# kewei/gnss-sdr-rs

Hardware: AMD Instinct MI355X
Metric: acq PRN×Doppler cells/s + tracking ch×Msps at 1/2/4/8 GPU; % HBM roofline (higher is better)
Workload: dtype f32

## Files before the change

gnss-sdr-rs_amd/_lib.py:

```python
import ctypes as C
import os

_HERE = os.path.dirname(os.path.abspath(__file__))
_LIB_PATH = os.environ.get("GM_LIB_PATH") or os.path.join(_HERE, "lib", "libgnss_mi355x.so")


class GmError(RuntimeError):
    def __init__(self, status, where, detail=""):
        self.status = status
        super().__init__(f"{where}: gm_status {status} ({detail})")


class c32(C.Structure):
    _fields_ = [("re", C.c_float), ("im", C.c_float)]


class AcqResult(C.Structure):
    _fields_ = [("prn", C.c_uint8), ("code_phase_samples", C.c_uint64), ("code_phase_chips", C.c_float),
                ("carrier_freq", C.c_float), ("fs", C.c_float), ("mag_relative", C.c_float),
                ("sample_global_index", C.c_uint64), ("doppler_bin", C.c_int32)]

    def as_dict(self):
        return {k: getattr(self, k) for k, _ in self._fields_}


class AcqCfg(C.Structure):
    _fields_ = [("fs", C.c_float), ("f_if", C.c_float), ("fft_size", C.c_uint32), ("n_integrations", C.c_uint32),
                ("n_bins", C.c_uint32), ("doppler_hz", C.c_void_p), ("tables", C.c_void_p),
                ("table_freq", C.c_void_p), ("n_prn", C.c_uint32), ("prn_ids", C.c_void_p), ("codes", C.c_void_p),
                ("code_len", C.c_uint32), ("code_rate", C.c_float), ("threshold", C.c_float),
                ("decision_mode", C.c_int32), ("strict_sum_order", C.c_int32), ("reference_products", C.c_int32),
                ("any_length", C.c_int32), ("coherent_periods", C.c_uint32)]


class AcqPlan(C.Structure):
    _fields_ = [("form", C.c_int32), ("base", C.c_uint32), ("q", C.c_uint32), ("transform_len", C.c_uint32)]


ACQ_FORM_LDS, ACQ_FORM_COMPOSITE, ACQ_FORM_LONG, ACQ_FORM_LONG_PADDED = 0, 1, 2, 3


class TrkState(C.Structure):
    _fields_ = [("prn", C.c_uint8), ("active", C.c_uint8), ("reserved", C.c_uint8 * 2), ("lost_counter", C.c_uint32),
                ("next_sample_index", C.c_uint64), ("num_samples_per_code", C.c_uint64),
                ("carrier_freq", C.c_float), ("carrier_phase", C.c_float), ("carrier_error", C.c_float),
                ("carrier_nco", C.c_float), ("code_phase", C.c_float), ("code_error", C.c_float),
                ("code_nco", C.c_float), ("code_rate", C.c_float), ("i_prompt", C.c_float), ("q_prompt", C.c_float)]


class TrkOut(C.Structure):
    _fields_ = [(k, C.c_float) for k in ("ip", "qp", "ie", "qe", "il", "ql", "ive", "qve", "ivl", "qvl")]


class NavStatus(C.Structure):
    _fields_ = [("flag_bit_sync", C.c_uint8), ("flag_frame_sync", C.c_uint8), ("sync_sw", C.c_uint8), ("bit", C.c_int8),
                ("polarity", C.c_int8), ("frame_sync_ind", C.c_uint32), ("n_frame_bits", C.c_uint64), ("i_p", C.c_float),
                ("sf_cnt", C.c_uint64), ("sf_start_biti", C.c_uint64), ("tow_expected_ind", C.c_uint64)]


class TrkCfg(C.Structure):
    _fields_ = [("fs", C.c_float), ("n_channels", C.c_uint32), ("n_arms", C.c_uint32),
                ("early_late_space", C.c_float), ("very_early_late_space", C.c_float),
                ("code_index_mode", C.c_int32), ("boc11", C.c_int32), ("codes", C.c_void_p),
                ("n_codes", C.c_uint32), ("code_len", C.c_uint32), ("nominal_code_rate", C.c_float),
                ("pll_bw", C.c_float), ("pll_zeta", C.c_float), ("pll_gain", C.c_float), ("dll_bw", C.c_float),
                ("dll_zeta", C.c_float), ("dll_gain", C.c_float), ("pll_dt", C.c_float), ("dll_dt", C.c_float),
                ("lock_threshold", C.c_float), ("max_lost_epochs", C.c_uint32), ("strict_libm", C.c_int32), ("strict_sum_order", C.c_int32),
                ("share_device", C.c_int32)]


FMT_C32, FMT_I8_IQ, FMT_I8_REAL = 0, 1, 2
CODE_INDEX_FAITHFUL, CODE_INDEX_FIXED = 0, 1

_vp, _f, _u64, _u32, _sz, _i = C.c_void_p, C.c_float, C.c_uint64, C.c_uint32, C.c_size_t, C.c_int
SIGNATURES = {
    "gm_abi_version": (_i, []),
    "gm_init": (_i, [_i]),
    "gm_device_count": (_i, [C.POINTER(_i)]),
    "gm_last_error": (C.c_char_p, []),
    "gm_status_string": (C.c_char_p, [_i]),
    "gm_ca_code_row": (_i, [_i, _vp]),
    "gm_b1i_code": (_i, [C.c_uint32, _vp, C.c_uint32]),
    "gm_generate_ca_code_samples": (_i, [C.c_uint8, _f, _f, _vp, _sz, C.POINTER(_sz)]),
    "gm_doppler_table_new": (_i, [_f, _f, _f, _sz, C.POINTER(_f), _vp]),
    "gm_apply_doppler_shift": (_i, [_vp, _vp, _vp, _sz]),
    "gm_fft_c2c_f32": (_i, [_sz, _i, _vp, _sz]),
    "gm_fft_power_spectrum_f32": (_i, [_sz, _vp, _vp]),
    "gm_rfft_f32": (_i, [_sz, _vp, _vp]),
    "gm_fft_supported_sizes": (_i, [_vp, _i]),
    "gm_acq_plan_info": (_i, [C.c_uint32, C.c_int32, C.POINTER(AcqPlan)]),
    "gm_acq_create": (_i, [C.POINTER(AcqCfg), C.POINTER(_vp)]),
    "gm_acq_destroy": (_i, [_vp]),
    "gm_acq_search": (_i, [_vp, _vp, _sz, _i, _u64, _u64, _vp, _vp]),
    "gm_acq_search_c32": (_i, [_vp, _vp, _sz, _u64, _u64, _vp, _vp]),
    "gm_acq_search_i8": (_i, [_vp, _vp, _sz, _u64, _u64, _vp, _vp]),
    "gm_acq_search_ring": (_i, [_vp, _vp, _u64, _vp, _vp, C.POINTER(_u64)]),
    "gm_acq_search_dev": (_i, [_vp, _vp, _i, _vp]),
    "gm_acq_set_prn_mask": (_i, [_vp, _u64]),
    "gm_acq_decide_dev": (_i, [_vp, _vp, _u32, _vp, _u64]),
    "gm_acq_finer_doppler": (_i, [_vp, _vp, _vp, _u32, _vp, _vp, _vp, _vp]),
    "gm_comm_get_unique_id": (_i, [_vp]),
    "gm_comm_init": (_i, [_i, _i, _vp, _vp]),
    "gm_comm_destroy": (_i, [_vp]),
    "gm_comm_info": (_i, [_vp, _vp, _vp]),
    "gm_acq_allgather_metrics": (_i, [_vp, _vp, _vp, _vp]),
    "gm_acq_allgather_metrics_async": (_i, [_vp, _vp, _vp, _vp]),
    "gm_comm_wait": (_i, [_vp, _vp]),
    "gm_comm_allgather_words": (_i, [_vp, _vp, _vp, _sz, _vp]),
    "gm_grid_assemble_dev": (_i, [_vp, _u32, _u32, _u32, _vp, _u32, _vp, _vp]),
    "gm_acq_decide_planes_dev": (_i, [_vp, _vp, _vp, _u32, _u32, _vp, _vp, _u32, _f, _f, _f, _i, _u64, _vp, _vp, _vp]),
    "gm_acq_fetch_results": (_i, [_vp, _u32, _vp, _vp]),
    "gm_acq_decide_host": (_i, [_vp, _vp, _vp, _vp, _u32, _u32, _vp, _u32, _f, _f, _f, _u64, _vp, _vp]),
    "gm_acq_synchronize": (_i, [_vp]),
    "gm_acq_set_deferred_decision": (_i, [_vp, _i]),
    "gm_acq_prepare_dev": (_i, [_vp, _vp, _i, _vp, C.POINTER(C.c_uint64)]),
    "gm_acq_search_prepared_dev": (_i, [_vp, C.c_uint64, _vp]),
    "gm_acq_drop_prepared": (_i, [_vp]),
    "gm_acq_set_stream": (_i, [_vp, _vp]),
    "gm_acq_metrics": (_i, [_vp, _vp, _vp, _vp]),
    "gm_acq_code_fft": (_i, [_vp, _u32, _vp]),
    "gm_acq_tables": (_i, [_vp, _vp, _vp]),
    "gm_acq_coherent_phasors": (_i, [_vp, _vp]),
    "gm_acq_edge_dwell_periods": (_i, [_u32, _u32, _u32, _vp, _vp, C.POINTER(_u64)]),
    "gm_acq_set_edge_search": (_i, [_vp, _u32, _vp, _vp]),
    "gm_acq_edge_metrics": (_i, [_vp, _vp, _vp, _vp]),
    "gm_acq_edge_choice": (_i, [_vp, _vp]),
    "gm_acq_result_offsets": (_i, [_vp, _vp, _vp, _u32, _vp]),
    "gm_acq_enable_timing": (_i, [_vp, _i]),
    "gm_acq_last_timing": (_i, [_vp, C.POINTER(_f), C.POINTER(_f), C.POINTER(_f)]),
    "gm_acq_timing_summary": (_i, [_vp, C.POINTER(_u32), C.POINTER(_f), C.POINTER(_f)]),
    "gm_acq_debug_stamps": (_i, [_vp, _vp]),
    "gm_acq_manager_mode_for": (_i, [_sz]),
    "gm_acq_manager_pacing_and_list": (_i, [_i, _u32, C.POINTER(_u64), C.POINTER(_u32)]),
    "gm_ring_create": (_i, [_sz, C.POINTER(_vp)]),
    "gm_ring_destroy": (_i, [_vp]),
    "gm_ring_write_samples": (_i, [_vp, _vp, _sz]),
    "gm_ring_get_head": (_i, [_vp, C.POINTER(_u64)]),
    "gm_ring_copy_to_slice": (_i, [_vp, _u64, _vp, _sz]),
    "gm_ring_write_samples_async": (_i, [_vp, _vp, _sz]),
    "gm_ring_flush": (_i, [_vp]),
    "gm_ring_get_enqueued_head": (_i, [_vp, C.POINTER(_u64)]),
    "gm_ring_wait_head": (_i, [_vp, _u64, _u32, _vp]),
    "gm_nav_sync_create": (_i, [_i, _vp]),
    "gm_nav_sync_destroy": (_i, [_vp]),
    "gm_nav_sync_update": (_i, [_vp, _f, _f, _u64, _u64, _vp]),
    "gm_nav_sync_update_many": (_i, [_vp, _f, _vp, _sz, _sz, _u64, _u64, _vp, _vp, _vp]),
    "gm_nav_sync_frame_bits": (_i, [_vp, _vp, _sz, _vp]),
    "gm_nav_sync_histogram": (_i, [_vp, _vp]),
    "gm_nav_parity_check": (_i, [_vp, _vp, _vp]),
    "gm_frontend_create": (_i, [_f, _f, _f, _vp]),
    "gm_frontend_destroy": (_i, [_vp]),
    "gm_frontend_lut": (_i, [_vp, _vp, _vp, _vp]),
    "gm_frontend_get_state": (_i, [_vp, _vp, _vp, _vp]),
    "gm_frontend_set_state": (_i, [_vp, _f, _vp, _vp]),
    "gm_frontend_process_block": (_i, [_vp, _vp, _sz]),
    "gm_frontend_process_dev": (_i, [_vp, _vp, _i, _vp, _sz, _vp]),
    "gm_frontend_process_dev_batch": (_i, [_vp, _u32, _vp, _i, _vp, _sz, _vp]),
    "gm_frontend_synchronize": (_i, [_vp]),
    "gm_frontend_write_ring": (_i, [_vp, _vp, _vp, _sz, _i]),
    "gm_frontend_debug_repairs": (_i, [_vp, C.POINTER(_u32)]),
    "gm_trk_create": (_i, [C.POINTER(TrkCfg), C.POINTER(_vp)]),
    "gm_trk_destroy": (_i, [_vp]),
    "gm_trk_start": (_i, [_vp, _u32, C.POINTER(AcqResult)]),
    "gm_trk_reset": (_i, [_vp, _u32]),
    "gm_trk_get_state": (_i, [_vp, _u32, C.POINTER(TrkState)]),
    "gm_trk_set_state": (_i, [_vp, _u32, C.POINTER(TrkState)]),
    "gm_trk_get_ca_chip": (_i, [_vp, _u32, _f, C.POINTER(_f)]),
    "gm_loop_filter_new": (_i, [_f, _f, _f, C.POINTER(_f), C.POINTER(_f)]),
    "gm_loop_filter_update": (_f, [_f, _f, _f, _f, _f]),
    "gm_trk_correlate": (_i, [_vp, _u32, _vp, _sz, C.POINTER(TrkOut)]),
    "gm_trk_do_work": (_i, [_vp, _u32, _vp, _sz, C.POINTER(TrkOut), C.POINTER(C.c_uint8), C.POINTER(C.c_uint8)]),
    "gm_trk_update_all": (_i, [_vp, _vp, _u32, _vp, _vp, _vp, C.POINTER(_u32)]),
    "gm_trk_update_all_dev": (_i, [_vp, _vp, _u32]),
    "gm_trk_update_all_async": (_i, [_vp, _vp, _u32, C.POINTER(C.c_uint64)]),
    "gm_trk_collect": (_i, [_vp, C.c_uint64, _i, _vp, _vp, _vp, _vp, C.POINTER(_u32), C.POINTER(_i)]),
    "gm_trk_get_states": (_i, [_vp, _vp]),
    "gm_trk_set_states": (_i, [_vp, _vp, _vp]),
    "gm_trk_synchronize": (_i, [_vp]),
    "gm_trk_set_stream": (_i, [_vp, _vp]),
    "gm_trk_debug_stamps": (_i, [_vp, _u32, _vp]),
    "gm_trk_enable_timing": (_i, [_vp, _i]),
    "gm_trk_last_timing": (_i, [_vp, C.POINTER(_f), C.POINTER(_u32)]),
}

_lib = None


def library_path():
    return _LIB_PATH


def lib():
    global _lib
    if _lib is not None:
        return _lib
    if not os.path.exists(_LIB_PATH):
        raise ImportError(f"{_LIB_PATH} is missing: run `python __graft_entry__.py build` (hipcc, gfx950). "
                          "There is no CPU fallback for the HIP path.")
    L = C.CDLL(_LIB_PATH)
    for name, (res, args) in SIGNATURES.items():
        fn = getattr(L, name)
        fn.restype, fn.argtypes = res, args
    _lib = L
    return L


def check(status, where):
    if status != 0:
        L = lib()
        raise GmError(status, where, (L.gm_status_string(status) or b"").decode() + "; " +
                      (L.gm_last_error() or b"").decode())


_initialised = None


def init(device=0):
    global _initialised
    if _initialised != device:
        check(lib().gm_init(device), "gm_init")
        _initialised = device
```

gnss-sdr-rs_amd/build.py:

```python
import os
import subprocess
import sys
from concurrent.futures import ThreadPoolExecutor

HERE = os.path.dirname(os.path.abspath(__file__))
CSRC = os.path.join(HERE, "csrc")
LIBDIR = os.path.join(HERE, "lib")
LIB = os.path.join(LIBDIR, "libgnss_mi355x.so")
SOURCES = ["acq_kernels.hip", "acq_composite.hip", "acq_long.hip", "acq_coherent.hip", "acq_edge.hip", "trk_kernels.hip", "fe_kernels.hip", "nav_host.hip", "gm_api.hip"]
HEADERS = ["fft_core.h", "fft_plans.h", "acq_corr_plans.h", "gm_internal.h", "gm_libm.h", "acq_device.h", "acq_corr_ws31.h", "ws31_core.h", "acq_comp_ws.h", os.path.join("..", "..", "include", "gnss_mi355x.h")]
FLAGS = ["--offload-arch=gfx950", "-O3", "-std=c++17", "-ffp-contract=off", "-fno-slp-vectorize", "-fhip-fp32-correctly-rounded-divide-sqrt", "-fPIC",
         "-Wall", "-Wno-unused-function"]


def _stale(target, deps):
    if not os.path.exists(target):
        return True
    t = os.path.getmtime(target)
    return any(os.path.getmtime(d) > t for d in deps)


def build(force=False, verbose=False):
    global LIB
    extra = os.environ.get("GM_EXTRA_FLAGS", "").split()
    suffix = os.environ.get("GM_LIB_SUFFIX", "")
    if suffix:
        LIB = os.path.join(LIBDIR, "libgnss_mi355x%s.so" % suffix)
    os.makedirs(LIBDIR, exist_ok=True)
    objdir = os.path.join(HERE, "build" + suffix)
    os.makedirs(objdir, exist_ok=True)
    hdrs = [os.path.join(CSRC, h) for h in HEADERS]
    jobs = []
    for src in SOURCES:
        s = os.path.join(CSRC, src)
        o = os.path.join(objdir, src + ".o")
        if force or _stale(o, [s] + hdrs):
            jobs.append(["hipcc", *FLAGS, *extra, "-c", s, "-o", o])
    def run(cmd):
        if verbose:
            print(" ".join(cmd), flush=True)
        r = subprocess.run(cmd, stdout=subprocess.PIPE, stderr=subprocess.STDOUT, text=True)
        if r.returncode:
            raise RuntimeError("hipcc failed:\n" + " ".join(cmd) + "\n" + r.stdout)
        return r.stdout
    with ThreadPoolExecutor(max_workers=6) as ex:
        list(ex.map(run, jobs))
    objs = [os.path.join(objdir, s + ".o") for s in SOURCES]
    if force or jobs or _stale(LIB, objs):
        run(["hipcc", "--offload-arch=gfx950", "-shared", "-fPIC", "-o", LIB, *objs,
             "-Wl,--version-script=" + os.path.join(CSRC, "exports.map")])
    build_synth(force)
    build_receiver_harness(force)
    return LIB


def build_receiver_harness(force=False):
    src = os.path.join(HERE, "host", "receiver_harness.cpp")
    lib = os.path.join(LIBDIR, "libgm_receiver.so")
    deps = [src, os.path.join(HERE, "host", "gnss_sdr.hpp"), os.path.join(HERE, "..", "include", "gnss_mi355x.h")]
    product = os.path.join(LIBDIR, "libgnss_mi355x.so")
    if force or _stale(lib, deps) or (os.path.exists(product) and os.path.getmtime(product) > os.path.getmtime(lib)):
        r = subprocess.run(["g++", "-O2", "-std=c++17", "-fPIC", "-shared", "-ffp-contract=off", "-Wall", "-o", lib, src,
                            "-L", LIBDIR, "-lgnss_mi355x", "-Wl,-rpath,$ORIGIN", "-Wl,-rpath,/opt/rocm/lib", "-pthread"],
                           stdout=subprocess.PIPE, stderr=subprocess.STDOUT, text=True)
        if r.returncode:
            raise RuntimeError("g++ failed:\n" + r.stdout)
    return lib


def build_synth(force=False):
    src = os.path.join(HERE, "synthgen", "synth_xoshiro.cpp")
    lib = os.path.join(LIBDIR, "libgm_synth.so")
    if force or _stale(lib, [src]):
        r = subprocess.run(["g++", "-O2", "-std=c++17", "-fPIC", "-shared", "-fopenmp", "-ffp-contract=off", "-fno-builtin", "-o", lib, src],
                           stdout=subprocess.PIPE, stderr=subprocess.STDOUT, text=True)
        if r.returncode:
            raise RuntimeError("g++ failed:\n" + r.stdout)
    return lib


if __name__ == "__main__":
    print(build(force="--force" in sys.argv, verbose=True))
```

gnss-sdr-rs_amd/csrc/acq_kernels.hip:

```cpp
#include "acq_device.h"

namespace gm {

template <bool WG>
__device__ __forceinline__ void decide_body(const DecideArgs& a, int p, int lane, float* dsm) {
    const int D = a.n_bins;
    float* smax = dsm;
    float* ssum = dsm + D;
    uint32_t* sarg = reinterpret_cast<uint32_t*>(dsm + 2 * D);
    for (int d = lane; d < D; d += 64) {
        const size_t o = size_t(p) * D + d;
        smax[d] = a.mmax[o]; ssum[d] = a.msum[o]; sarg[d] = a.margmax[o];
    }
    if constexpr (WG) __syncthreads();
    else { __builtin_amdgcn_fence(__ATOMIC_RELEASE, "workgroup"); __builtin_amdgcn_wave_barrier(); __builtin_amdgcn_fence(__ATOMIC_ACQUIRE, "workgroup"); }
    const bool searched = (p >= 64) || ((a.mask_lo >> p) & 1ull);
    float gmax = 0.0f, bsum = 0.0f;
    uint32_t bphase = 0;
    int bbin = -1;
    bool pass = false;
    float carry_v = 0.0f;
    int carry_b = -1;
    for (int d0 = 0; d0 < D; d0 += 64) {
        const int d = d0 + lane;
        if (d0 > 0) { gmax = 0.0f; bsum = 0.0f; bphase = 0; bbin = -1; }
#ifdef GM_DECIDE_SERIAL_SCAN
        if (d < D && searched) {
            for (int q = 0; q <= d; ++q) {
                const float lm = smax[q];
                if (lm > gmax) { gmax = lm; bphase = sarg[q]; bsum = ssum[q]; bbin = q; }
            }
        }
#else
        {
            const float own = (d < D) ? smax[d] : 0.0f;
            gmax = own > 0.0f ? own : 0.0f;
            bbin = own > 0.0f ? d : -1;
#pragma unroll
            for (int off = 1; off < 64; off <<= 1) {
                const float ev = __shfl_up(gmax, off, 64);
                const int eb = __shfl_up(bbin, off, 64);
                if (lane >= off && !(gmax > ev)) { gmax = ev; bbin = eb; }
            }
            if (d0 > 0 && !(gmax > carry_v)) { gmax = carry_v; bbin = carry_b; }
            carry_v = __shfl(gmax, 63, 64); carry_b = __shfl(bbin, 63, 64);
            bphase = bbin >= 0 ? sarg[bbin] : 0u;
            bsum = bbin >= 0 ? ssum[bbin] : 0.0f;
        }
#endif
        if (d < D && searched) {
            if (!a.best_bin_mode || d + 1 == D) {
                const float avg = __fdiv_rn(bsum - gmax, float(a.fft_size - 1));
                pass = __fdiv_rn(gmax, avg) > a.threshold;
            }
        }
        const unsigned long long votes = __ballot(pass);
        if (votes) {
            if (lane == __ffsll((long long)votes) - 1) {
                gm_acq_result r;
                r.prn = a.prn_ids[p];
                r.code_phase_samples = bphase;
                r.code_phase_chips = __fdiv_rn(float(bphase) * a.code_rate, a.fs);
                r.carrier_freq = a.table_freq[bbin]; r.fs = a.fs; r.mag_relative = gmax;
                r.sample_global_index = a.local_tail + bphase; r.doppler_bin = bbin;
                a.results[p] = r;
                a.found[p] = 1;
            }
            return;
        }
    }
    if (lane == 0) {
        gm_acq_result r;
        r.prn = a.prn_ids[p]; r.code_phase_samples = 0; r.code_phase_chips = 0.f; r.carrier_freq = 0.f;
        r.fs = 0.f; r.mag_relative = 0.f; r.sample_global_index = 0; r.doppler_bin = -1;
        a.results[p] = r;
        a.found[p] = 0;
    }
}
__global__ __launch_bounds__(64) void decide_kernel(DecideArgs a) {
    extern __shared__ float dsm[];
    decide_body<true>(a, blockIdx.x, threadIdx.x, dsm);
}

template <class PLX>
__global__ __launch_bounds__(MixPlanOf<PLX>::type::T) void acq_mix_fft_kernel(const void* __restrict__ samples, int fmt,
                                                            const cf* __restrict__ tables,
                                                            const cf* __restrict__ tw_fwd,
                                                            cf* __restrict__ spectra, int n_int,
                                                            uint32_t* __restrict__ clear_tickets,
                                                            const uint16_t* __restrict__ order, int n_items, DecideArgs dec) {
    using PL = typename MixPlanOf<PLX>::type;
    using CP = typename CorrPlanOf<PLX>::type;
    static_assert(PL::N == PLX::N, "the mix plan keeps the size");
    constexpr bool PERMUTED = CorrMode<CP>::PERMUTED;
    constexpr int STAGE = PERMUTED ? PL::N + PL::N / 32 + 1 : 0;
    constexpr int LDS_N = PL::LDS_ELEMS + PL::TW_TOTAL > STAGE ? PL::LDS_ELEMS + PL::TW_TOTAL : STAGE;
    __shared__ cf lds[LDS_N];
    if (int(blockIdx.x) >= n_items) {
        static_assert(LDS_N * 8 >= 3 * 64 * 4, "room for the decision's staging");
        if (threadIdx.x < 64) decide_body<false>(dec, int(blockIdx.x) - n_items, threadIdx.x, reinterpret_cast<float*>(lds));
        return;
    }
    cf* tw = lds + PL::LDS_ELEMS;
    const int tid = threadIdx.x;
    const int d = blockIdx.x / n_int, m = blockIdx.x % n_int;
    if (clear_tickets && blockIdx.x == 0)
        for (int i = tid; i < GM_CORR_SPLIT_MAX_ITEMS; i += PL::T) clear_tickets[i] = 0u;
    load_twiddles<PL>(tw, tw_fwd, tid);
    const size_t sbase = size_t(m) * PL::N;
    const cf* tab = tables + size_t(d) * PL::N;
    cf* dst = spectra + size_t(blockIdx.x) * PL::N;
    constexpr int NB0 = PL::NB(0);
    auto in = [&](int it, int r) {
        const int idx = (tid + it * PL::T) + r * NB0;
        const cf s = load_sample(samples, fmt, sbase + idx);
        const cf t = tab[idx];
        return cf_make(s.x * t.x - s.y * t.y, s.x * t.y + s.y * t.x);
    };
    if constexpr (!PERMUTED) {
        constexpr int NBL = PL::NB(PL::NP - 1);
        lds_transform<PL, false>(in, [&](int it, int r, cf val) { dst[PairLayout<CP>::pos((tid + it * PL::T) + r * NBL)] = val; }, lds, tw, tid);
    } else {
        constexpr int NBL = PL::NB(PL::NP - 1);
        {
            cf v0[PL::IT0][PL::R0];
            Fft<PL, false>::pass0_stage1(v0, in, tid);
            __syncthreads();
            Fft<PL, false>::pass0_stage2(v0, lds, tid);
        }
        __syncthreads();
        MiddlePasses<PL, false, 1>::run(lds, tw, tid);
        cf vl[PL::ITL][PL::RL];
        Fft<PL, false>::last_stage1(vl, lds, tw, tid);
        __syncthreads();
        Fft<PL, false>::last_stage2(vl, [&](int it, int r, cf val) {
            const int k = (tid + it * PL::T) + r * NBL;
            lds[k + (k >> 5)] = val; }, tid);
        __syncthreads();
        static_assert(PL::N % 2 == 0, "N must be even");
        for (int g = tid; g < PL::N / 2; g += PL::T) {
            const uint32_t o = reinterpret_cast<const uint32_t*>(order)[g];
            const int k0 = int(o & 0xffffu), k1 = int(o >> 16);
            const cf v0 = lds[k0 + (k0 >> 5)], v1 = lds[k1 + (k1 >> 5)];
            reinterpret_cast<float4*>(dst)[g] = make_float4(v0.x, v0.y, v1.x, v1.y);
        }
    }
}

__device__ long long* g_corr_stamps = nullptr;
__device__ __forceinline__ void corr_stamp(long long* base, int m, int wave, int phase) {
    if (base) {
        unsigned long long t;
        __builtin_amdgcn_sched_barrier(0);
        asm volatile("s_memtime %0\n\ts_waitcnt lgkmcnt(0)" : "=s"(t) :: "memory");
        __builtin_amdgcn_sched_barrier(0);
        base[(size_t(m) * 8 + wave) * 8 + phase] = (long long)t;
    }
}
#ifdef GM_DIAG_STAMPS
static bool g_corr_stamps_armed = false;
bool corr_stamps_built() { return true; }
void set_corr_stamps(long long* d_ptr) {
    (void)hipMemcpyToSymbol(HIP_SYMBOL(g_corr_stamps), &d_ptr, sizeof(d_ptr));
    g_corr_stamps_armed = d_ptr != nullptr;
}
#else
static constexpr bool g_corr_stamps_armed = false;
bool corr_stamps_built() { return false; }
void set_corr_stamps(long long*) {}
#endif

template <class PLX, bool KEEP_CODE, bool STAMPS, bool REF_MUL>
__global__ __launch_bounds__(CorrPlanOf<PLX>::type::T, CorrPlanOf<PLX>::type::WAVES_PER_EU) void acq_corr_kernel(
    const cf* __restrict__ spectra, const cf* __restrict__ code_fft, const cf* __restrict__ tw_inv,
    float* __restrict__ mmax, uint32_t* __restrict__ margmax, float* __restrict__ msum,
    const uint32_t* __restrict__ worker_list, int n_workers, int n_bins, int n_int, int map_mode,
    int split_from, int split_k, int split_items, float* __restrict__ split_scratch, uint32_t* __restrict__ split_counter,
    int strict_sum) {
    const int xcd = blockIdx.x & 7, wslot = blockIdx.x >> 3;
    int slot = wslot, part = 0, parts = 1;
    if (wslot >= split_from) {
        const int h = wslot - split_from;
        slot = split_from + h / split_k;
        part = h % split_k;
        parts = split_k;
    }
    int d, p;
    if (map_mode == 0) {
        const int items = n_bins * n_workers, share = (items + 7) >> 3;
        const int item = xcd * share + slot;
        if (slot >= share || item >= items) return;
        d = item / n_workers;
        p = int(worker_list[item - d * n_workers]);
    } else if (map_mode >= 16) {
        const int cb = map_mode >> 4, rows_max = map_mode & 15;
        const int items = n_bins * n_workers, share = (items + 7) >> 3;
        const int it_lo = xcd * share, it_hi = it_lo + share < items ? it_lo + share : items;
        const int d_lo = it_lo / n_workers, per_blk = rows_max * cb;
        const int blk = slot / per_blk, rem = slot - blk * per_blk, dr = rem / cb, w = blk * cb + (rem - dr * cb);
        const int item = (d_lo + dr) * n_workers + w;
        if (w >= n_workers || item < it_lo || item >= it_hi) return;
        d = d_lo + dr;
        p = int(worker_list[w]);
    } else if (map_mode == 1) {
        d = xcd + 8 * (slot / n_workers);
        if (d >= n_bins) return;
        p = int(worker_list[slot % n_workers]);
    } else {
        const int q = n_bins >> 3, whole = q * n_workers;
        if (slot < whole) {
            d = xcd + 8 * (slot / n_workers);
            p = int(worker_list[slot % n_workers]);
        } else {
            const int left = (n_bins - 8 * q) * n_workers, each = (left + 7) >> 3;
            const int j = slot - whole, item = xcd * each + j;
            if (j >= each || item >= left) return;
            d = 8 * q + item / n_workers;
            p = int(worker_list[item % n_workers]);
        }
    }

    using PL = typename CorrPlanOf<PLX>::type;
    constexpr bool PFA = CorrMode<PL>::PFA, HYB = CorrMode<PL>::HYBRID;
    __shared__ cf lds[PL::LDS_ELEMS + ((PFA || HYB) ? 0 : PL::TW_TOTAL)];
    cf* tw = lds + PL::LDS_ELEMS;
    const int tid = threadIdx.x;
    if constexpr (!PFA && !HYB) load_twiddles<PL>(tw, tw_inv, tid);
    constexpr int NB0 = PL::NB(0), NBL = PL::NB(PL::NP - 1);
    auto last_active = [&](int it) { if constexpr (HYB) return PL::last_active(tid); else return tid + it * PL::T < NBL; };
    auto out_index = [&](int it, int r) {
        if constexpr (HYB) return PL::out_index(tid, r);
        else if constexpr (PFA) return Pfa<PL>::out_index(tid + it * PL::T, r);
        else return (tid + it * PL::T) + r * NBL;
    };

    const __amdgpu_buffer_rsrc_t xrs = make_rsrc(spectra + size_t(d) * n_int * PL::N, unsigned(n_int) * PL::N * 8u);
    const __amdgpu_buffer_rsrc_t crs = make_rsrc(code_fft + size_t(p) * PL::N, PL::N * 8u);

    using PLd = PairLoad<PL>;
    constexpr bool CODE_PAIRED = CorrLayout<PL>::CODE_PAIRED;
    cf cc[KEEP_CODE ? PL::IT0 : 1][KEEP_CODE ? PL::R0 : 1];
    if constexpr (KEEP_CODE) {
#pragma unroll
        for (int it = 0; it < PL::IT0; ++it) {
            const int b = tid + it * PL::T;
            if (b < NB0) {
                PLd q;
                if constexpr (CODE_PAIRED) q.load(crs, b, 0);
#pragma unroll
                for (int r = 0; r < PL::R0; ++r) {
                    const cf c = CODE_PAIRED ? q.get(r) : buf_load_cf(crs, b * 8, r * NB0 * 8);
                    cc[it][r] = cf_make(c.x, -c.y);
                }
            }
        }
    }
    float acc[PL::ITL][PL::RL];
#pragma unroll
    for (int it = 0; it < PL::ITL; ++it)
#pragma unroll
        for (int r = 0; r < PL::RL; ++r) acc[it][r] = 0.0f;

    long long* stbase = nullptr;
    if constexpr (STAMPS) stbase = (blockIdx.x == 0 && (tid & 63) == 0 && PL::T / 64 <= 8) ? g_corr_stamps : nullptr;
    const int wv = tid >> 6;
    const int m_per = n_int / parts, m_begin = part * m_per, m_end = m_begin + m_per;
    constexpr bool CAN_SPLIT = !STAMPS;
    constexpr int RL4 = (PL::RL + 3) / 4;
    auto acc_or_zero = [&](int it, int r) { return r < PL::RL ? acc[it][r < PL::RL ? r : 0] : 0.0f; };
#ifndef GM_CORR_PREFETCH_PAIRS
#define GM_CORR_PREFETCH_PAIRS 4
#endif
    constexpr int NPF = (HYB && CODE_PAIRED && !STAMPS && !KEEP_CODE) ? (GM_CORR_PREFETCH_PAIRS < PLd::NPAIR ? GM_CORR_PREFETCH_PAIRS : PLd::NPAIR) : 0;
    PLd xq[PL::IT0];
    auto load_x_ahead = [&](int m_) {
#pragma unroll
        for (int it = 0; it < PL::IT0; ++it) xq[it].template load_range<0, NPF, false>(xrs, tid + it * PL::T, m_ * PL::N);
    };
    if constexpr (NPF > 0) load_x_ahead(m_begin);
    for (int m = m_begin; m < m_end; ++m) {
        PLd cq[(KEEP_CODE || !CODE_PAIRED) ? 1 : PL::IT0];
#pragma unroll
        for (int it = 0; it < PL::IT0; ++it) {
            const int b = tid + it * PL::T;
            if constexpr (CODE_PAIRED) xq[it].template load_range<NPF, PLd::NPAIR, true>(xrs, b, m * PL::N);
            if constexpr (!KEEP_CODE && CODE_PAIRED) cq[it].load(crs, b, 0);
        }
        auto in = [&](int it, int r) {
            const cf a = CODE_PAIRED ? xq[it].get(r) : buf_load_cf(xrs, (tid + it * PL::T) * 8, (m * PL::N + r * NB0) * 8);
            cf c;
            if constexpr (KEEP_CODE) c = cc[it][r];
            else if constexpr (CODE_PAIRED) { const cf g = cq[it].get(r); c = cf_make(g.x, -g.y); }
            else { const cf g = buf_load_cf(crs, (tid + it * PL::T) * 8, r * NB0 * 8); c = cf_make(g.x, -g.y); }
            if constexpr (REF_MUL) return cf_make(a.x * c.x - a.y * c.y, a.x * c.y + a.y * c.x);
            else return cf_make(__builtin_fmaf(a.x, c.x, -(a.y * c.y)), __builtin_fmaf(a.x, c.y, a.y * c.x));
        };
        auto out = [&](int it, int r, cf v) {
            if constexpr (REF_MUL) acc[it][r] = acc[it][r] + (v.x * v.x + v.y * v.y);
            else acc[it][r] = acc[it][r] + __builtin_fmaf(v.y, v.y, v.x * v.x);
        };
        if constexpr (NPF > 0) {
            lds_transform<PL, true, PFA>(in, out, lds, tw, tid, [&](int k) {
                if (k == 1) {
                    __builtin_amdgcn_sched_barrier(0);
                    load_x_ahead(m + 1 < m_end ? m + 1 : n_int);
                    __builtin_amdgcn_sched_barrier(0);
                }
            });
        } else if constexpr (!STAMPS) {
            lds_transform<PL, true, PFA>(in, out, lds, tw, tid);
        } else {
            auto st = [&](int k) { corr_stamp(stbase, m, wv, k); };
            st(0);
            {
                cf v0[PL::IT0][PL::R0];
                Fft<PL, true, PFA>::pass0_stage1(v0, in, tid);
                st(1);
                __syncthreads();
                st(2);
                Fft<PL, true, PFA>::pass0_stage2(v0, lds, tid);
            }
            st(3);
            __syncthreads();
            MiddlePasses<PL, true, 1, PFA>::run(lds, tw, tid, st);
            cf vl[PL::ITL][PL::RL];
            Fft<PL, true, PFA>::last_stage1(vl, lds, tw, tid);
            Fft<PL, true, PFA>::last_stage2(vl, out, tid);
        }
    }

    if constexpr (CAN_SPLIT) {
        if (parts > 1) {
            constexpr int SLAB = PL::ITL * RL4 * 4 * PL::T;
            const size_t item_plane0 = (size_t(xcd) * split_items + (slot - split_from)) * size_t(n_int);
            const __amdgpu_buffer_rsrc_t srs = make_rsrc(split_scratch + item_plane0 * SLAB, unsigned(n_int) * SLAB * 4u);
            const int voff = tid * 16 + part * SLAB * 4;
#pragma unroll
            for (int it = 0; it < PL::ITL; ++it)
#pragma unroll
                for (int r4 = 0; r4 < RL4; ++r4) {
                    u32x4 v;
                    v.x = __float_as_uint(acc_or_zero(it, 4 * r4 + 0)); v.y = __float_as_uint(acc_or_zero(it, 4 * r4 + 1));
                    v.z = __float_as_uint(acc_or_zero(it, 4 * r4 + 2)); v.w = __float_as_uint(acc_or_zero(it, 4 * r4 + 3));
                    __builtin_amdgcn_raw_buffer_store_b128(v, srs, voff + (it * RL4 + r4) * PL::T * 16, 0, 16);
                    asm volatile("s_nop 1" ::: "memory");
                }
            asm volatile("s_waitcnt vmcnt(0)" ::: "memory");
            __syncthreads();
            __shared__ int s_last;
            if (tid == 0) {
                uint32_t* cnt = split_counter + size_t(xcd) * split_items + (slot - split_from);
                const uint32_t old = __hip_atomic_fetch_add(cnt, 1u, __ATOMIC_RELAXED, __HIP_MEMORY_SCOPE_AGENT);
                s_last = (old == uint32_t(parts - 1)) ? 1 : 0;
            }
            __syncthreads();
            if (!s_last) return;
#pragma unroll
            for (int it = 0; it < PL::ITL; ++it)
#pragma unroll
                for (int r = 0; r < PL::RL; ++r) acc[it][r] = 0.0f;
            for (int q = 0; q < n_int; ++q) {
#pragma unroll
                for (int it = 0; it < PL::ITL; ++it)
#pragma unroll
                    for (int r4 = 0; r4 < RL4; ++r4) {
                        const u32x4 v = __builtin_amdgcn_raw_buffer_load_b128(srs, tid * 16, (q * SLAB + (it * RL4 + r4) * PL::T * 4) * 4, 16);
                        if (4 * r4 + 0 < PL::RL) acc[it][4 * r4 + 0] += __uint_as_float(v.x);
                        if (4 * r4 + 1 < PL::RL) acc[it][4 * r4 + 1 < PL::RL ? 4 * r4 + 1 : 0] += __uint_as_float(v.y);
                        if (4 * r4 + 2 < PL::RL) acc[it][4 * r4 + 2 < PL::RL ? 4 * r4 + 2 : 0] += __uint_as_float(v.z);
                        if (4 * r4 + 3 < PL::RL) acc[it][4 * r4 + 3 < PL::RL ? 4 * r4 + 3 : 0] += __uint_as_float(v.w);
                    }
            }
        }
    }

    float strict_total = 0.0f;
    if (strict_sum) {
        __syncthreads();
        float* pl = reinterpret_cast<float*>(lds);
#pragma unroll
        for (int it = 0; it < PL::ITL; ++it) {
            if (last_active(it)) {
#pragma unroll
                for (int r = 0; r < PL::RL; ++r) pl[out_index(it, r)] = acc[it][r];
            }
        }
        __syncthreads();
        if (tid < 64) {
            float ls = 0.0f;
            if (tid < 8) {
                constexpr int CHUNKS = PL::N / 8;
#pragma unroll 8
                for (int c = 0; c < CHUNKS; ++c) ls = ls + pl[c * 8 + tid];
            }
            float t = -0.0f;
#pragma unroll
            for (int l = 0; l < 8; ++l) t = t + __uint_as_float(__builtin_amdgcn_readlane(__float_as_uint(ls), l));
            strict_total = t;
        }
    }

    float bv = 0.0f, sum = 0.0f;
    uint32_t bi = 0xffffffffu;
    if constexpr (!PFA) {
#pragma unroll
        for (int it = 0; it < PL::ITL; ++it) {
            if (last_active(it)) {
#pragma unroll
                for (int r = 0; r < PL::RL; ++r) {
                    take_better(bv, bi, acc[it][r], uint32_t(out_index(it, r)));
                    sum += acc[it][r];
                }
            }
        }
    } else {
        int bs = -1, ties = 0;
#pragma unroll
        for (int it = 0; it < PL::ITL; ++it) {
            if (tid + it * PL::T < NBL) {
#pragma unroll
                for (int r = 0; r < PL::RL; ++r) {
                    const float v = acc[it][r];
                    if (v > bv) { bv = v; bs = it * PL::RL + r; }
                    sum += v;
                }
            }
        }
#pragma unroll
        for (int it = 0; it < PL::ITL; ++it) {
            if (tid + it * PL::T < NBL) {
#pragma unroll
                for (int r = 0; r < PL::RL; ++r) ties += acc[it][r] == bv ? 1 : 0;
            }
        }
        if (ties == 1 && bs >= 0) {
            bi = uint32_t(Pfa<PL>::out_index(tid + (bs / PL::RL) * PL::T, bs % PL::RL));
        } else if (ties >= 1) {
#pragma unroll
            for (int it = 0; it < PL::ITL; ++it) {
                const int b = tid + it * PL::T;
                if (b < NBL) {
#pragma unroll
                    for (int r = 0; r < PL::RL; ++r)
                        if (acc[it][r] == bv) {
                            const uint32_t i = uint32_t(Pfa<PL>::out_index(b, r));
                            bi = i < bi ? i : bi;
                        }
                }
            }
        }
    }
#pragma unroll
    for (int off = 32; off >= 1; off >>= 1) {
        const float ov = __shfl_xor(bv, off, 64);
        const uint32_t oi = uint32_t(__shfl_xor(int(bi), off, 64));
        const float os = __shfl_xor(sum, off, 64);
        take_better(bv, bi, ov, oi);
        sum += os;
    }
    __syncthreads();
    float* sv = reinterpret_cast<float*>(lds);
    uint32_t* si = reinterpret_cast<uint32_t*>(lds) + 64;
    float* ss = reinterpret_cast<float*>(lds) + 128;
    const int wave = tid >> 6, lane = tid & 63;
    constexpr int NW = PL::T / 64;
    if (lane == 0) { sv[wave] = bv; si[wave] = bi; ss[wave] = sum; }
    __syncthreads();
    if (tid == 0) {
        float fv = sv[0], fs = ss[0];
        uint32_t fi = si[0];
        for (int w = 1; w < NW; ++w) { take_better(fv, fi, sv[w], si[w]); fs += ss[w]; }
        if (fi == 0xffffffffu) fi = 0;
        const size_t o = size_t(p) * n_bins + d;
        mmax[o] = fv; margmax[o] = fi; msum[o] = strict_sum ? strict_total : fs;
    }
}

}
#include "acq_corr_ws31.h"
namespace gm {

template <class PL>
__global__ __launch_bounds__(PL::T) void acq_code_fft_kernel(const int8_t* __restrict__ code_samples,
                                                             const cf* __restrict__ tw_fwd,
                                                             cf* __restrict__ code_fft) {
    __shared__ cf lds[PL::LDS_ELEMS + PL::TW_TOTAL];
    cf* tw = lds + PL::LDS_ELEMS;
    const int tid = threadIdx.x;
    load_twiddles<PL>(tw, tw_fwd, tid);
    const int8_t* src = code_samples + size_t(blockIdx.x) * PL::N;
    cf* dst = code_fft + size_t(blockIdx.x) * PL::N;
    constexpr int NB0 = PL::NB(0), NBL = PL::NB(PL::NP - 1);
    lds_transform<PL, false>([&](int it, int r) { return cf_make(float(src[(tid + it * PL::T) + r * NB0]), 0.0f); },
                             [&](int it, int r, cf val) { dst[(tid + it * PL::T) + r * NBL] = val; }, lds, tw, tid);
}

template <class PL, bool INV>
__global__ __launch_bounds__(PL::T) void fft_batch_kernel(cf* __restrict__ data, const cf* __restrict__ tw_g) {
    __shared__ cf lds[PL::LDS_ELEMS + PL::TW_TOTAL];
    cf* tw = lds + PL::LDS_ELEMS;
    const int tid = threadIdx.x;
    load_twiddles<PL>(tw, tw_g, tid);
    cf* x = data + size_t(blockIdx.x) * PL::N;
    constexpr int NB0 = PL::NB(0), NBL = PL::NB(PL::NP - 1);
    lds_transform<PL, INV>([&](int it, int r) { return x[(tid + it * PL::T) + r * NB0]; },
                           [&](int it, int r, cf val) { x[(tid + it * PL::T) + r * NBL] = val; }, lds, tw, tid);
}

template <class PL, bool INV>
__global__ __launch_bounds__(PL::T) void big_cols_kernel(const cf* __restrict__ x, cf* __restrict__ B, const cf* __restrict__ tw_g, uint32_t N2) {
    __shared__ cf lds[PL::LDS_ELEMS + PL::TW_TOTAL];
    cf* tw = lds + PL::LDS_ELEMS;
    const int tid = threadIdx.x;
    const uint32_t n2 = blockIdx.x, L = uint32_t(PL::N) * N2;
    load_twiddles<PL>(tw, tw_g, tid);
    cf* dst = B + size_t(n2) * PL::N;
    constexpr int NB0 = PL::NB(0), NBL = PL::NB(PL::NP - 1);
    const float inv_l = 2.0f / float(L);
    lds_transform<PL, INV>(
        [&](int it, int r) { return x[size_t(N2) * uint32_t((tid + it * PL::T) + r * NB0) + n2]; },
        [&](int it, int r, cf v) {
            const uint32_t k1 = uint32_t((tid + it * PL::T) + r * NBL);
            const uint32_t t = (n2 * k1) & (L - 1u);
            float sn, cs;
            sincospif(float(t) * inv_l, &sn, &cs);
            if (INV) sn = -sn;
            dst[k1] = cf_make(__builtin_fmaf(v.x, cs, v.y * sn), __builtin_fmaf(v.y, cs, -(v.x * sn)));
        },
        lds, tw, tid);
}
template <class PL, bool INV>
__global__ __launch_bounds__(PL::T) void big_rows_kernel(const cf* __restrict__ B, cf* __restrict__ X, const cf* __restrict__ tw_g, uint32_t N1) {
    __shared__ cf lds[PL::LDS_ELEMS + PL::TW_TOTAL];
    cf* tw = lds + PL::LDS_ELEMS;
    const int tid = threadIdx.x;
    const uint32_t k1 = blockIdx.x;
    load_twiddles<PL>(tw, tw_g, tid);
    constexpr int NB0 = PL::NB(0), NBL = PL::NB(PL::NP - 1);
    lds_transform<PL, INV>(
        [&](int it, int r) { return B[size_t(uint32_t((tid + it * PL::T) + r * NB0)) * N1 + k1]; },
        [&](int it, int r, cf v) { X[size_t(N1) * uint32_t((tid + it * PL::T) + r * NBL) + k1] = v; },
        lds, tw, tid);
}

template <class PL>
__global__ __launch_bounds__(PL::T) void fine_cols_kernel(FineArgs a) {
    __shared__ cf lds[PL::LDS_ELEMS + PL::TW_TOTAL];
    cf* tw = lds + PL::LDS_ELEMS;
    const int tid = threadIdx.x;
    const uint32_t n2 = blockIdx.x, sat = blockIdx.y;
    load_twiddles<PL>(tw, a.tw1, tid);
    const uint32_t cp = a.sat_code_phase[sat];
    const int8_t* chips = a.chips + size_t(a.sat_worker[sat]) * a.code_len;
    const float mre = a.mean[0], mim = a.mean[1];
    cf* dst = a.B + (size_t(sat) * a.N2 + n2) * PL::N;
    constexpr int NB0 = PL::NB(0), NBL = PL::NB(PL::NP - 1);
    const float inv_n = 2.0f / float(a.N1 * a.N2);
    lds_transform<PL, false>(
        [&](int it, int r) {
            const uint32_t n1 = uint32_t((tid + it * PL::T) + r * NB0);
            const uint32_t n = a.N2 * n1 + n2;
            if (n >= a.size_use) return cf_make(0.0f, 0.0f);
            const cf s = load_sample(a.samples, a.fmt, size_t(cp) + n);
            const uint32_t ind = uint32_t(floorf((float(n) * a.code_rate) / a.fs)) % a.code_len;
            const float c = float(chips[ind]);
            return cf_make((s.x - mre) * c, (s.y - mim) * c);
        },
        [&](int it, int r, cf v) {
            const uint32_t k1 = uint32_t((tid + it * PL::T) + r * NBL);
            const uint32_t t = (n2 * k1) & (a.N1 * a.N2 - 1u);
            float sn, cs;
            sincospif(float(t) * inv_n, &sn, &cs);
            dst[k1] = cf_make(__builtin_fmaf(v.x, cs, v.y * sn), __builtin_fmaf(v.y, cs, -(v.x * sn)));
        },
        lds, tw, tid);
}

template <class PL> struct FineRows {
    static constexpr int PER = PL::IT0 * PL::R0;
    static constexpr int RT = PL::T >= 1024 ? 1 : (PER <= 8 ? 8 : (PER <= 16 ? 4 : (PER <= 32 ? 2 : 1)));
};

template <class PL>
__global__ __launch_bounds__(PL::T) void fine_rows_kernel(FineArgs a) {
    constexpr int RT = FineRows<PL>::RT;
    __shared__ cf lds[PL::LDS_ELEMS + PL::TW_TOTAL];
    __shared__ float s_p[PL::T / 64];
    __shared__ uint32_t s_k[PL::T / 64];
    cf* tw = lds + PL::LDS_ELEMS;
    const int tid = threadIdx.x;
    const uint32_t k1_0 = blockIdx.x * RT, sat = blockIdx.y;
    load_twiddles<PL>(tw, a.tw2, tid);
    const cf* src = a.B + size_t(sat) * a.N2 * a.N1 + k1_0;
    constexpr int NB0 = PL::NB(0), NBL = PL::NB(PL::NP - 1);
    cf tile[RT][PL::IT0][PL::R0];
#pragma unroll
    for (int it = 0; it < PL::IT0; ++it) {
        const int b = tid + it * PL::T;
        if (b < NB0) {
#pragma unroll
            for (int r = 0; r < PL::R0; ++r) {
                const cf* p = src + size_t(b + r * NB0) * a.N1;
#pragma unroll
                for (int j = 0; j < RT; ++j) tile[j][it][r] = p[j];
            }
        }
    }
    float best = -1.0f;
    uint32_t bestk = 0xFFFFFFFFu;
#pragma unroll
    for (int j = 0; j < RT; ++j) {
        lds_transform<PL, false>(
            [&](int it, int r) { return tile[j][it][r]; },
            [&](int it, int r, cf v) {
                const uint32_t k = (k1_0 + j) + a.N1 * uint32_t((tid + it * PL::T) + r * NBL);
                const float p = __builtin_fmaf(v.x, v.x, v.y * v.y);
                if (p > best || (p == best && k < bestk)) { best = p; bestk = k; }
            },
            lds, tw, tid);
    }
    for (int off = 32; off > 0; off >>= 1) {
        const float op = __shfl_xor(best, off);
        const uint32_t ok = __shfl_xor(bestk, off);
        if (op > best || (op == best && ok < bestk)) { best = op; bestk = ok; }
    }
    if ((tid & 63) == 0) { s_p[tid >> 6] = best; s_k[tid >> 6] = bestk; }
    __syncthreads();
    if (tid == 0) {
        for (int w = 1; w < PL::T / 64; ++w)
            if (s_p[w] > best || (s_p[w] == best && s_k[w] < bestk)) { best = s_p[w]; bestk = s_k[w]; }
        a.rowmax[size_t(sat) * (a.N1 / RT) + blockIdx.x] = best;
        a.rowarg[size_t(sat) * (a.N1 / RT) + blockIdx.x] = bestk;
    }
}

__global__ __launch_bounds__(256) void fine_final_kernel(const float* __restrict__ rowmax, const uint32_t* __restrict__ rowarg,
                                                         uint32_t n_rows, float* __restrict__ peak_pow,
                                                         uint32_t* __restrict__ peak_idx) {
    __shared__ float s_p[4];
    __shared__ uint32_t s_k[4];
    const int tid = threadIdx.x;
    const uint32_t sat = blockIdx.x;
    float best = -1.0f;
    uint32_t bestk = 0xFFFFFFFFu;
    for (uint32_t i = tid; i < n_rows; i += 256) {
        const float p = rowmax[size_t(sat) * n_rows + i];
        const uint32_t k = rowarg[size_t(sat) * n_rows + i];
        if (p > best || (p == best && k < bestk)) { best = p; bestk = k; }
    }
    for (int off = 32; off > 0; off >>= 1) {
        const float op = __shfl_xor(best, off);
        const uint32_t ok = __shfl_xor(bestk, off);
        if (op > best || (op == best && ok < bestk)) { best = op; bestk = ok; }
    }
    if ((tid & 63) == 0) { s_p[tid >> 6] = best; s_k[tid >> 6] = bestk; }
    __syncthreads();
    if (tid == 0) {
        for (int w = 1; w < 4; ++w)
            if (s_p[w] > best || (s_p[w] == best && s_k[w] < bestk)) { best = s_p[w]; bestk = s_k[w]; }
        peak_pow[sat] = best;
        peak_idx[sat] = bestk;
    }
}
void launch_fine_final(hipStream_t st, const float* rowmax, const uint32_t* rowarg, uint32_t n_rows, int n_sats,
                       float* peak_pow, uint32_t* peak_idx) {
    hipLaunchKernelGGL(fine_final_kernel, dim3(n_sats), dim3(256), 0, st, rowmax, rowarg, n_rows, peak_pow, peak_idx);
}

__global__ __launch_bounds__(1024) void fine_mean_kernel(const void* __restrict__ samples, int fmt, uint32_t n, float* __restrict__ mean) {
    __shared__ float s_re[16], s_im[16];
    const int tid = threadIdx.x;
    float re = 0.0f, im = 0.0f;
    for (uint32_t i = tid; i < n; i += 1024) {
        const cf v = load_sample(samples, fmt, i);
        re += v.x; im += v.y;
    }
    for (int off = 32; off > 0; off >>= 1) { re += __shfl_xor(re, off); im += __shfl_xor(im, off); }
    if ((tid & 63) == 0) { s_re[tid >> 6] = re; s_im[tid >> 6] = im; }
    __syncthreads();
    if (tid == 0) {
        for (int w = 1; w < 16; ++w) { re += s_re[w]; im += s_im[w]; }
        mean[0] = re / float(n);
        mean[1] = im / float(n);
    }
}
void launch_fine_mean(hipStream_t st, const void* samples, int fmt, uint32_t n, float* d_mean) {
    hipLaunchKernelGGL(fine_mean_kernel, dim3(1), dim3(1024), 0, st, samples, fmt, n, d_mean);
}

template <class PL> struct Launch {
    static void fill_tw(cf* tw, bool inverse) {
        fill_twiddles<PL>(tw, inverse, [](double a) { return ::cos(a); }, [](double a) { return ::sin(a); });
    }
    using CP = typename CorrPlanOf<PL>::type;
    static constexpr bool CORR_TW = !CorrMode<CP>::PFA && !CorrMode<CP>::HYBRID;
    static constexpr int corr_tw_total() { if constexpr (CORR_TW) return CP::TW_TOTAL; else return 0; }
    static void fill_tw_corr(cf* tw) {
        if constexpr (CORR_TW) fill_twiddles<CP>(tw, true, [](double a) { return ::cos(a); }, [](double a) { return ::sin(a); });
    }
    static_assert(CP::T == PL::T && CP::N == PL::N, "the correlation plan keeps the size and the workgroup");
    using MP = typename MixPlanOf<PL>::type;
    static void fill_tw_mix(cf* tw, bool inverse) {
        fill_twiddles<MP>(tw, inverse, [](double a) { return ::cos(a); }, [](double a) { return ::sin(a); });
    }
    static void mix_fft(hipStream_t st, const void* samples, int fmt, const cf* tables, const cf* tw_fwd,
                        cf* spectra, int n_bins, int n_int, uint32_t* clear_tickets, const uint16_t* order, const DecideArgs* dec) {
        const int n_items = n_bins * n_int, n_dec = dec ? dec->n_prn : 0;
        DecideArgs none{};
        hipLaunchKernelGGL(acq_mix_fft_kernel<PL>, dim3(n_items + n_dec), dim3(MP::T), 0, st, samples, fmt,
                           tables, tw_fwd, spectra, n_int, clear_tickets, order, n_items, dec ? *dec : none);
    }
    static int fill_order(uint16_t* order) { return fill_order_table<CP>(order); }
    static constexpr bool WS31 = Ws31<CP>::USE && CorrMode<CP>::PFA;
    static constexpr int slab() {
        constexpr int generic = CP::ITL * ((CP::RL + 3) / 4) * 4 * CP::T;
        if constexpr (WS31) return ws31_split_slab<CP>() > generic ? ws31_split_slab<CP>() : generic;
        else return generic;
    }
    static constexpr int SPLIT_SLAB = slab();
    static void corr(hipStream_t st, const cf* spectra, const cf* code_fft, const cf* tw_inv, float* mmax,
                     uint32_t* margmax, float* msum, const uint32_t* worker_list, int n_workers, int n_bins,
                     int n_int, float* split_scratch, int split_planes, uint32_t* split_counter, int strict_sum, int tickets_cleared,
                     int ref_mul) {
        if (n_workers <= 0) return;
        static const int forced = diag_int("GM_CORR_MAP", -1);
        const int per_xcd_bins = ((n_bins + 7) / 8) * n_workers, per_xcd_even = (n_bins * n_workers + 7) / 8;
        const int slots = 32 * CP::WG_PER_CU;
        const int q = n_bins / 8, left = (n_bins - 8 * q) * n_workers;
        const int per_xcd_mixed = q * n_workers + (left + 7) / 8;
        int map_mode = ((per_xcd_bins + slots - 1) / slots > (per_xcd_even + slots - 1) / slots) ? 0 : 1;
        if (map_mode == 1 && per_xcd_mixed < per_xcd_bins) map_mode = 2;
        if (forced >= 0) map_mode = forced;
        static const int cb_env = diag_int("GM_CORR_CB", -1);
        int cb = cb_env >= 0 ? cb_env : 0;
        int share = map_mode == 0 ? per_xcd_even : (map_mode == 1 ? per_xcd_bins : per_xcd_mixed);
        if (cb > 0) {
            const int rows_max = (per_xcd_even + n_workers - 2) / n_workers + 1;
            if (rows_max <= 15 && cb <= 1000) {
                map_mode = (cb << 4) | rows_max;
                share = ((n_workers + cb - 1) / cb) * rows_max * cb;
            }
        }
        static const int split_env = diag_int("GM_CORR_SPLIT", -1);
        static const int items_env = diag_int("GM_CORR_SPLIT_ITEMS", -1);
        int split_from = share, split_k = 1, split_items = 0;
        if (SPLIT_SLAB && split_scratch && split_counter && split_env != 0 && !g_corr_stamps_armed && !strict_sum &&
            (share > slots || share <= GM_CORR_SPLIT_MAX_ITEMS / 8)) {
            const bool all = share <= slots;
            if (n_int >= 2 && n_int <= GM_CORR_SPLIT_MAX_K && (!all || share * n_int <= split_planes / 8)) split_k = n_int;
            if (CP::WG_PER_CU == 1 && !all && split_env < 0) split_k = 1;
            if (split_env == 1) split_k = 1;
            if (split_k > 1) {
                split_items = items_env > 0 ? items_env : (all ? share : (slots + split_k - 1) / split_k);
                if (split_items > share) split_items = share;
                if (split_items > GM_CORR_SPLIT_MAX_ITEMS / 8) split_items = GM_CORR_SPLIT_MAX_ITEMS / 8;
                if (split_items * n_int > split_planes / 8) split_items = split_planes / 8 / n_int;
                if (split_items <= 0) { split_items = 0; split_k = 1; }
                split_from = share - split_items;
            }
        }
        const int grid = 8 * (split_from + split_items * split_k);
        if (split_k > 1 && !tickets_cleared) (void)hipMemsetAsync(split_counter, 0, size_t(GM_CORR_SPLIT_MAX_ITEMS) * sizeof(uint32_t), st);
        if constexpr (WS31) {
            if (!g_corr_stamps_armed) {
                if (ref_mul)
                    hipLaunchKernelGGL((acq_corr_ws31_kernel<CP, true>), dim3(grid), dim3(1024), 0, st, spectra, code_fft, mmax, margmax, msum,
                                       worker_list, n_workers, n_bins, n_int, map_mode, split_from, split_k, split_items, split_scratch, split_counter, strict_sum);
                else
                    hipLaunchKernelGGL((acq_corr_ws31_kernel<CP, false>), dim3(grid), dim3(1024), 0, st, spectra, code_fft, mmax, margmax, msum,
                                       worker_list, n_workers, n_bins, n_int, map_mode, split_from, split_k, split_items, split_scratch, split_counter, strict_sum);
                return;
            }
        }
#ifdef GM_DIAG_STAMPS
        if (g_corr_stamps_armed) {
            hipLaunchKernelGGL((acq_corr_kernel<PL, CP::KEEP_CODE, true, false>), dim3(grid), dim3(PL::T), 0, st,
                               spectra, code_fft, tw_inv, mmax, margmax, msum, worker_list, n_workers, n_bins, n_int, map_mode,
                               split_from, split_k, split_items, split_scratch, split_counter, strict_sum);
            return;
        }
#endif
#ifdef GM_DIAG_STAMPS
        constexpr bool GENERIC = true;
#else
        constexpr bool GENERIC = !WS31;
#endif
        if constexpr (GENERIC) {
            if (ref_mul)
                hipLaunchKernelGGL((acq_corr_kernel<PL, CP::KEEP_CODE, false, true>), dim3(grid), dim3(PL::T), 0, st,
                                   spectra, code_fft, tw_inv, mmax, margmax, msum, worker_list, n_workers, n_bins, n_int, map_mode,
                                   split_from, split_k, split_items, split_scratch, split_counter, strict_sum);
            else
                hipLaunchKernelGGL((acq_corr_kernel<PL, CP::KEEP_CODE, false, false>), dim3(grid), dim3(PL::T), 0, st,
                                   spectra, code_fft, tw_inv, mmax, margmax, msum, worker_list, n_workers, n_bins, n_int, map_mode,
                                   split_from, split_k, split_items, split_scratch, split_counter, strict_sum);
        }
    }
    static void code_fft(hipStream_t st, const int8_t* code_samples, const cf* tw_fwd, cf* out, int n_codes) {
        hipLaunchKernelGGL(acq_code_fft_kernel<PL>, dim3(n_codes), dim3(PL::T), 0, st, code_samples, tw_fwd, out);
    }
    static void pair_codes(hipStream_t st, const cf* nat, cf* paired, int n_codes) {
        hipLaunchKernelGGL(relayout_kernel<CP>, dim3(n_codes * 4 < 1024 ? n_codes * 4 : 1024), dim3(256), 0, st, nat, paired, n_codes);
    }
    static void fft_batch(hipStream_t st, cf* data, const cf* tw, int inverse, int batch) {
        if (inverse) hipLaunchKernelGGL((fft_batch_kernel<PL, true>), dim3(batch), dim3(PL::T), 0, st, data, tw);
        else hipLaunchKernelGGL((fft_batch_kernel<PL, false>), dim3(batch), dim3(PL::T), 0, st, data, tw);
    }
    static constexpr bool POW2 = (PL::N & (PL::N - 1)) == 0;
    static void big_cols(hipStream_t st, const cf* x, cf* B, const cf* tw, uint32_t n2, int inverse) {
        if constexpr (POW2) {
            if (inverse) hipLaunchKernelGGL((big_cols_kernel<PL, true>), dim3(n2), dim3(PL::T), 0, st, x, B, tw, n2);
            else hipLaunchKernelGGL((big_cols_kernel<PL, false>), dim3(n2), dim3(PL::T), 0, st, x, B, tw, n2);
        }
    }
    static void big_rows(hipStream_t st, const cf* B, cf* X, const cf* tw, uint32_t n1, int inverse) {
        if constexpr (POW2) {
            if (inverse) hipLaunchKernelGGL((big_rows_kernel<PL, true>), dim3(n1), dim3(PL::T), 0, st, B, X, tw, n1);
            else hipLaunchKernelGGL((big_rows_kernel<PL, false>), dim3(n1), dim3(PL::T), 0, st, B, X, tw, n1);
        }
    }
    static void fine_cols(hipStream_t st, const FineArgs& a, int n_sats) {
        if constexpr (POW2) hipLaunchKernelGGL(fine_cols_kernel<PL>, dim3(a.N2, n_sats), dim3(PL::T), 0, st, a);
    }
    static void fine_rows(hipStream_t st, const FineArgs& a, int n_sats) {
        if constexpr (POW2) hipLaunchKernelGGL(fine_rows_kernel<PL>, dim3(a.N1 / FineRows<PL>::RT, n_sats), dim3(PL::T), 0, st, a);
    }
    static constexpr PlanOps ops() {
        return PlanOps{PL::N, PL::T, PL::TW_TOTAL, int(sizeof(cf)) * (CP::LDS_ELEMS + corr_tw_total()), SPLIT_SLAB,
                       CorrLayout<CP>::RELAYOUT ? 1 : 0,
                       &fill_tw, &fill_order, &mix_fft, &corr, &code_fft, &pair_codes, &fft_batch,
                       POW2 ? &fine_cols : nullptr, POW2 ? &fine_rows : nullptr, FineRows<PL>::RT,
                       POW2 ? &big_cols : nullptr, POW2 ? &big_rows : nullptr, MP::TW_TOTAL, &fill_tw_mix, corr_tw_total(), &fill_tw_corr,
                       &launch_mix_fft_coh<PL>};
    }
};

#define GM_PLAN_ENTRY(PL) Launch<PL>::ops(),
static const PlanOps g_plans[] = {GM_FOR_EACH_PLAN(GM_PLAN_ENTRY)};

const PlanOps* find_plan(int n) {
    for (const PlanOps& p : g_plans)
        if (p.n == n) return &p;
    return nullptr;
}
int list_plans(uint32_t* sizes, int cap) {
    int k = 0;
    for (const PlanOps& p : g_plans) {
        if (k < cap && sizes) sizes[k] = uint32_t(p.n);
        ++k;
    }
    return k;
}

__global__ void apply_doppler_kernel(const cf* __restrict__ s, const cf* __restrict__ t, cf* __restrict__ out,
                                     size_t n4) {
    for (size_t i = size_t(blockIdx.x) * blockDim.x + threadIdx.x; i < n4; i += size_t(gridDim.x) * blockDim.x) {
        const cf a = s[i], b = t[i];
        out[i] = cf_make(a.x * b.x - a.y * b.y, a.x * b.y + a.y * b.x);
    }
}
void launch_apply_doppler(hipStream_t st, const cf* s, const cf* t, cf* out, size_t n) {
    const size_t n4 = (n / 4) * 4;
    if (!n4) return;
    const int blocks = int((n4 + 255) / 256 < 2048 ? (n4 + 255) / 256 : 2048);
    hipLaunchKernelGGL(apply_doppler_kernel, dim3(blocks), dim3(256), 0, st, s, t, out, n4);
}

__global__ void power_kernel(const cf* __restrict__ x, float* __restrict__ p, size_t n) {
    for (size_t i = size_t(blockIdx.x) * blockDim.x + threadIdx.x; i < n; i += size_t(gridDim.x) * blockDim.x) {
        const cf v = x[i];
        p[i] = v.x * v.x + v.y * v.y;
    }
}
void launch_power(hipStream_t st, const cf* x, float* p, size_t n) {
    if (!n) return;
    const int blocks = int((n + 255) / 256 < 2048 ? (n + 255) / 256 : 2048);
    hipLaunchKernelGGL(power_kernel, dim3(blocks), dim3(256), 0, st, x, p, n);
}

void launch_decide(hipStream_t st, const DecideArgs& a) {
    if (a.n_prn <= 0) return;
    hipLaunchKernelGGL(decide_kernel, dim3(a.n_prn), dim3(64), size_t(a.n_bins) * 12, st, a);
}

}
```

gnss-sdr-rs_amd/csrc/gm_api.hip:

```cpp
#include <dlfcn.h>
#include <math.h>
#include <stdio.h>
#include <stdlib.h>
#include <string.h>

#include <algorithm>
#include <atomic>
#include <chrono>
#include <condition_variable>
#include <mutex>
#include <string>
#include <vector>

#include "gm_internal.h"

using gm::cf;

extern char** environ;
namespace gm {
static const char* env_lookup(const char* name) {
    const size_t n = strlen(name);
    for (char** e = environ; e && *e; ++e)
        if (!strncmp(*e, name, n) && (*e)[n] == '=') return *e + n + 1;
    return nullptr;
}
int diag_int(const char* name, int dflt) {
    static const bool on = [] { const char* v = env_lookup("GM_DIAGNOSTICS"); return v && !strcmp(v, "1"); }();
    if (!on) return dflt;
    const char* v = env_lookup(name);
    return (v && *v) ? atoi(v) : dflt;
}
}

namespace {

thread_local std::string g_last_error;
int g_device = -1;

int set_err(int code, const char* what) {
    g_last_error = what ? what : "";
    return code;
}
int hip_fail(hipError_t e, const char* where) {
    char buf[256];
    snprintf(buf, sizeof(buf), "%s: %s", where, hipGetErrorString(e));
    g_last_error = buf;
    return GM_ERR_HIP;
}
#define HIPC(expr)                                         \
    do {                                                   \
        hipError_t _e = (expr);                            \
        if (_e != hipSuccess) return hip_fail(_e, #expr);  \
    } while (0)

int ensure_device(int dev) {
    if (dev < 0) return set_err(GM_ERR_NO_DEVICE, "gm_init() has not selected a HIP device");
    HIPC(hipSetDevice(dev));
    return GM_OK;
}

#define PI_F 3.14159265358979323846f
const float CA_RATE = 1.023e6f, CA_LEN = 1023.0f;

const uint16_t kG2Delay[32] = {5,   6,   7,   8,   17,  18,  139, 140, 141, 251, 252, 254, 255, 256, 257, 258,
                               469, 470, 471, 472, 473, 474, 509, 512, 513, 514, 515, 516, 859, 860, 861, 862};
struct CaTable {
    int8_t rows[32][1023];
    CaTable() {
        uint8_t g1[1023], g2[1023];
        uint16_t r1 = 0x3ff, r2 = 0x3ff;
        for (int i = 0; i < 1023; ++i) {
            g1[i] = (r1 >> 9) & 1;
            g2[i] = (r2 >> 9) & 1;
            const uint16_t f1 = ((r1 >> 2) ^ (r1 >> 9)) & 1;
            const uint16_t f2 = ((r2 >> 1) ^ (r2 >> 2) ^ (r2 >> 5) ^ (r2 >> 7) ^ (r2 >> 8) ^ (r2 >> 9)) & 1;
            r1 = uint16_t(((r1 << 1) | f1) & 0x3ff);
            r2 = uint16_t(((r2 << 1) | f2) & 0x3ff);
        }
        for (int p = 0; p < 32; ++p)
            for (int i = 0; i < 1023; ++i)
                rows[p][i] = (g1[i] ^ g2[(i + 1023 - kG2Delay[p]) % 1023]) ? 1 : -1;
    }
};
const CaTable& ca_table() {
    static const CaTable t;
    return t;
}

const uint8_t kB1iPhase[37][2] = {{1, 3}, {1, 4}, {1, 5}, {1, 6}, {1, 8}, {1, 9}, {1, 10}, {1, 11}, {2, 7}, {3, 4}, {3, 5}, {3, 6},
                                  {3, 8}, {3, 9}, {3, 10}, {3, 11}, {4, 5}, {4, 6}, {4, 8}, {4, 9}, {4, 10}, {4, 11}, {5, 6}, {5, 8},
                                  {5, 9}, {5, 10}, {5, 11}, {6, 8}, {6, 9}, {6, 10}, {6, 11}, {8, 9}, {8, 10}, {8, 11}, {9, 10},
                                  {9, 11}, {10, 11}};
int b1i_code(uint32_t prn, int8_t* out, uint32_t n_chips) {
    if (prn < 1 || prn > 37 || n_chips > 2047) return GM_ERR_OUT_OF_RANGE;
    uint8_t g1[11], g2[11];
    for (int k = 0; k < 11; ++k) g1[k] = g2[k] = uint8_t(k & 1);
    const int a = kB1iPhase[prn - 1][0] - 1, b = kB1iPhase[prn - 1][1] - 1;
    for (uint32_t i = 0; i < n_chips; ++i) {
        const uint8_t chip = g1[10] ^ g2[a] ^ g2[b];
        out[i] = chip ? -1 : 1;
        const uint8_t f1 = g1[0] ^ g1[6] ^ g1[7] ^ g1[8] ^ g1[9] ^ g1[10];
        const uint8_t f2 = g2[0] ^ g2[1] ^ g2[2] ^ g2[3] ^ g2[4] ^ g2[7] ^ g2[8] ^ g2[10];
        for (int k = 10; k > 0; --k) { g1[k] = g1[k - 1]; g2[k] = g2[k - 1]; }
        g1[0] = f1; g2[0] = f2;
    }
    return GM_OK;
}

size_t num_samples_per_code(float code_rate, float fs, float len) {
    const float v = roundf(fs / (code_rate / len));
    return v > 0.0f ? size_t(v) : 0;
}

int resample_code(const int8_t* chips, size_t code_len, bool wrap, float code_rate, float fs, size_t n, int8_t* out) {
    for (size_t i = 0; i < n; ++i) {
        const float f = floorf((float(i) * code_rate) / fs);
        size_t ind = f > 0.0f ? size_t(f) : 0;
        if (ind >= code_len) {
            if (!wrap) return GM_ERR_OUT_OF_RANGE;
            ind %= code_len;
        }
        out[i] = chips[ind];
    }
    return GM_OK;
}

void loop_filter_new(float bw, float zeta, float gain, float* tau1, float* tau2) {
    const float w = bw * 8.0f * zeta / (4.0f * (zeta * zeta) + 1.0f);
    *tau1 = gain / (w * w);
    *tau2 = (2.0f * zeta) / w;
}

struct Timing {
    static constexpr int CAP = 512;
    std::vector<hipEvent_t> ev;
    bool on = false;
    int stride = 1;
    int calls = 0;
    bool this_call = false;
    int count = 0;
    bool decide_valid = false;
};

}

struct gm_ring {
    int device = -1;
    cf* d_buf = nullptr;
    size_t size = 0, mask = 0;
    std::atomic<uint64_t> head{0};
    std::mutex notifier;
    std::condition_variable condvar;
    static constexpr int SLOTS = 4;
    static constexpr size_t SLOT_SAMPLES_MAX = size_t(1) << 19;
    size_t slot_samples = 0;
    cf* staging[SLOTS] = {nullptr, nullptr, nullptr, nullptr};
    hipEvent_t slot_done[SLOTS] = {nullptr, nullptr, nullptr, nullptr};
    bool slot_used[SLOTS] = {false, false, false, false};
    hipStream_t copy_stream = nullptr;
    hipStream_t fe_stream = nullptr;
    hipEvent_t h2d_done[SLOTS] = {nullptr, nullptr, nullptr, nullptr};
    hipStream_t last_enq_stream = nullptr;
    uint64_t write_pos = 0;
    uint64_t slot_seq = 0;
    struct Pending { int slot; uint64_t new_head; };
    std::mutex pend_mu;
    std::vector<Pending> pending;
    std::mutex enq_mu;
    hipEvent_t ev_enq = nullptr;
    uint64_t enqueued = 0;
    bool ev_enq_armed = false;
};

static hipError_t wait_event_polling(hipEvent_t ev) {
    const auto t0 = std::chrono::steady_clock::now();
    for (;;) {
        const hipError_t q = hipEventQuery(ev);
        if (q != hipErrorNotReady) return q;
        (void)hipGetLastError();
        if (std::chrono::steady_clock::now() - t0 > std::chrono::milliseconds(2)) return hipEventSynchronize(ev);
    }
}

static void ring_publish(gm_ring* r, uint64_t new_head) {
    uint64_t cur = r->head.load(std::memory_order_relaxed);
    bool moved = false;
    while (int64_t(new_head - cur) > 0) {
        if (r->head.compare_exchange_weak(cur, new_head, std::memory_order_release, std::memory_order_relaxed)) { moved = true; break; }
    }
    if (!moved) return;
    std::lock_guard<std::mutex> g(r->notifier);
    r->condvar.notify_all();
}
static void ring_refresh_head(gm_ring* r, bool all = false) {
    if (!r->copy_stream) return;
    uint64_t newest = 0;
    bool any = false;
    {
        std::lock_guard<std::mutex> g(r->pend_mu);
        size_t done = 0;
        while (done < r->pending.size()) {
            if (!all) {
                const hipError_t q = hipEventQuery(r->slot_done[r->pending[done].slot]);
                if (q != hipSuccess) { (void)hipGetLastError(); break; }
            }
            newest = r->pending[done].new_head; any = true; ++done;
        }
        if (done) r->pending.erase(r->pending.begin(), r->pending.begin() + done);
    }
    if (any) ring_publish(r, newest);
}
static int ring_async_init(gm_ring* r) {
    if (r->copy_stream) return GM_OK;
    {
        int least = 0, greatest = 0;
        HIPC(hipDeviceGetStreamPriorityRange(&least, &greatest));
        const int pr = gm::diag_int("GM_RING_COPY_PRIORITY", 99);
        HIPC(hipStreamCreateWithPriority(&r->copy_stream, hipStreamNonBlocking, pr == 99 ? least : pr));
    }
    for (int i = 0; i < gm_ring::SLOTS; ++i) {
        HIPC(hipHostMalloc(reinterpret_cast<void**>(&r->staging[i]), r->slot_samples * 8, hipHostMallocDefault));
        HIPC(hipEventCreateWithFlags(&r->slot_done[i], hipEventDisableTiming));
    }
    r->write_pos = r->head.load(std::memory_order_relaxed);
    return GM_OK;
}
static int ring_enqueue_publish(gm_ring* r, int slot, hipStream_t st) {
    {
        std::lock_guard<std::mutex> g(r->pend_mu);
        r->pending.push_back(gm_ring::Pending{slot, r->write_pos});
    }
    {
        std::lock_guard<std::mutex> g(r->enq_mu);
        if (!r->ev_enq) HIPC(hipEventCreateWithFlags(&r->ev_enq, hipEventDisableTiming));
        if (r->ev_enq_armed && r->last_enq_stream != st) HIPC(hipStreamWaitEvent(st, r->ev_enq, 0));
        r->last_enq_stream = st;
        HIPC(hipEventRecord(r->ev_enq, st));
        r->enqueued = r->write_pos;
        r->ev_enq_armed = true;
    }
    return GM_OK;
}
static int ring_reclaim_slot(gm_ring* r, int slot) {
    if (!r->slot_used[slot]) return GM_OK;
    HIPC(wait_event_polling(r->slot_done[slot]));
    ring_refresh_head(r);
    return GM_OK;
}

struct gm_acq {
    int device = -1;
    gm_acq_cfg cfg{};
    const gm::PlanOps* plan = nullptr;
    hipStream_t stream = nullptr;
    bool own_stream = false;
    uint32_t N = 0, D = 0, M = 0, P = 0;
    uint32_t K = 1;
    cf* d_rho = nullptr;
    struct Edge {
        uint32_t H = 0;
        std::vector<uint32_t> offsets;
        uint32_t o_max = 0, neg = 0;
        uint32_t* d_offsets = nullptr;
        cf* d_spectra = nullptr;
        cf* d_tmp = nullptr;
        uint32_t* d_full = nullptr;
        uint32_t* d_choice = nullptr;
        float* d_long_part = nullptr;
        float* d_planes = nullptr;
        gm::EdgeLaunch fwd = nullptr;
    } edge;
    float code_rate = CA_RATE;
    std::vector<float> table_freq;
    std::vector<uint8_t> prn_ids, dev_prn_ids;
    cf* d_tw_mix = nullptr;
    cf *d_tables = nullptr, *d_tw_fwd = nullptr, *d_tw_inv = nullptr, *d_code_fft = nullptr, *d_spectra = nullptr;
    cf* d_code_fft_paired = nullptr;
    uint16_t* d_order = nullptr;
    float* d_table_freq = nullptr;
    int8_t* d_code_samples = nullptr;
    void* d_samples = nullptr;
    size_t samples_cap = 0;
    uint32_t* d_metrics = nullptr;
    uint32_t* d_worker_list = nullptr;
    std::vector<uint32_t> worker_list;
    uint64_t mask = ~0ull;
    uint32_t n_workers = 0;
    gm_acq_result* d_results = nullptr;
    uint8_t *d_found = nullptr, *d_prn_ids = nullptr;
    uint32_t results_cap = 0;
    const void* last_metrics = nullptr;
    Timing tm;
    float* d_split_scratch = nullptr;
    int split_planes = 0;
    uint32_t* d_split_counter = nullptr;
    uint32_t Q = 1, Nb = 0;
    const gm::CompOps* comp = nullptr;
    cf* d_comp_tmp = nullptr;
    cf* d_comp_twn = nullptr;
    float* d_planes = nullptr;
    cf* d_code_comb = nullptr;
    const gm::LongOps* lng = nullptr;
    uint32_t L = 0, long_lim = 0, long_slab = 0;
    float long_scale = 1.0f;
    cf* d_long_code = nullptr;
    cf* d_long_z = nullptr;
    float* d_long_part = nullptr;
    struct Ahead {
        cf* d_spectra_alt = nullptr;
        hipStream_t side = nullptr;
        hipEvent_t ev_s = nullptr, ev_f = nullptr, ev_in = nullptr;
        bool valid = false;
        uint64_t token = 0, next_token = 1;
        const void* samples = nullptr;
        int fmt = 0;
        bool comp_wait = false;
    } ahead;
    bool defer_decisions = false;
    bool dec_deferred = false;
    gm::DecideArgs dec_args{};
    bool comp_post_folded = false;
    std::vector<int8_t> chips;
    uint32_t code_len = 1023;
    const void* last_samples = nullptr;
    int last_fmt = GM_FMT_C32;
    struct Fine {
        const gm::PlanOps *p1 = nullptr, *p2 = nullptr;
        uint32_t size_use = 0, sats_cap = 0;
        int8_t* d_chips = nullptr;
        cf *d_tw1 = nullptr, *d_tw2 = nullptr, *d_B = nullptr;
        float *d_mean = nullptr, *d_rowmax = nullptr, *d_peak_pow = nullptr;
        uint32_t *d_rowarg = nullptr, *d_sat_worker = nullptr, *d_sat_cp = nullptr, *d_peak_idx = nullptr;
    } fine;
};

static bool acq_fused(const gm_acq* a) { return a->Q == 1 && !a->lng; }

static size_t acq_dwell_periods(const gm_acq* a) { return size_t(a->K) * a->M + (a->edge.H ? a->edge.o_max : 0u); }
static void acq_edge_free(gm_acq::Edge& e) {
    hipFree(e.d_offsets); hipFree(e.d_spectra); hipFree(e.d_tmp); hipFree(e.d_full); hipFree(e.d_choice); hipFree(e.d_long_part);
    hipFree(e.d_planes);
    e = gm_acq::Edge{};
}

static int acq_set_mask(gm_acq* a, uint64_t mask) {
    std::vector<uint32_t> wl;
    for (uint32_t i = 0; i < a->P; ++i)
        if (i >= 64 || ((mask >> i) & 1ull)) wl.push_back(i);
    a->mask = mask;
    if (wl != a->worker_list || a->n_workers != wl.size()) {
        a->worker_list = wl;
        a->n_workers = uint32_t(wl.size());
        if (!wl.empty())
            HIPC(hipMemcpyAsync(a->d_worker_list, a->worker_list.data(), wl.size() * sizeof(uint32_t),
                                hipMemcpyHostToDevice, a->stream));
        HIPC(hipStreamSynchronize(a->stream));
    }
    return GM_OK;
}

static int acq_flush_decision(gm_acq* a) {
    if (a->dec_deferred) {
        a->dec_deferred = false;
        gm::launch_decide(a->stream, a->dec_args);
        HIPC(hipGetLastError());
    }
    return GM_OK;
}

static int acq_reserve_results(gm_acq* a, uint32_t n) {
    if (n <= a->results_cap) return GM_OK;
    if (int rc = acq_flush_decision(a)) return rc;
    void* blk = nullptr;
    uint8_t* ids = nullptr;
    HIPC(hipHostMalloc(&blk, (sizeof(gm_acq_result) + 1) * size_t(n), hipHostMallocDefault));
    if (hipError_t e = hipMalloc(&ids, n); e != hipSuccess) { hipHostFree(blk); return hip_fail(e, "hipMalloc(prn ids)"); }
    if (a->d_results) {
        if (hipError_t e = hipStreamSynchronize(a->stream); e != hipSuccess) { hipHostFree(blk); hipFree(ids); return hip_fail(e, "hipStreamSynchronize"); }
        hipHostFree(a->d_results);
        hipFree(a->d_prn_ids);
    }
    a->dev_prn_ids.clear();
    a->d_results = static_cast<gm_acq_result*>(blk);
    a->d_found = reinterpret_cast<uint8_t*>(a->d_results + n);
    a->d_prn_ids = ids;
    a->results_cap = n;
    return GM_OK;
}

extern "C" {

int gm_abi_version(void) { return GM_ABI_VERSION; }

int gm_device_count(int* count) {
    if (!count) return set_err(GM_ERR_INVALID_ARG, "count is null");
    int n = 0;
    hipError_t e = hipGetDeviceCount(&n);
    if (e != hipSuccess) { *count = 0; return hip_fail(e, "hipGetDeviceCount"); }
    *count = n;
    return GM_OK;
}

int gm_init(int device) {
    int n = 0;
    hipError_t e = hipGetDeviceCount(&n);
    if (e != hipSuccess || n <= 0) return set_err(GM_ERR_NO_DEVICE, "no HIP device visible");
    if (device < 0 || device >= n) return set_err(GM_ERR_INVALID_ARG, "device index out of range");
    HIPC(hipSetDevice(device));
    g_device = device;
    return GM_OK;
}

const char* gm_last_error(void) { return g_last_error.c_str(); }

const char* gm_status_string(int s) {
    switch (s) {
        case GM_OK: return "ok";
        case GM_ERR_INVALID_ARG: return "invalid argument";
        case GM_ERR_UNSUPPORTED_N: return "no FFT plan for this fft_size";
        case GM_ERR_NO_DEVICE: return "no HIP device";
        case GM_ERR_HIP: return "HIP runtime error";
        case GM_ERR_OUT_OF_RANGE: return "index out of range";
        case GM_ERR_ALIGNMENT: return "fft_size must be a multiple of 8";
        case GM_ERR_NOMEM: return "out of memory";
        default: return "unknown status";
    }
}

int gm_b1i_code(uint32_t prn, int8_t* out_chips, uint32_t n_chips) {
    if (!out_chips) return set_err(GM_ERR_INVALID_ARG, "null out");
    if (int rc = b1i_code(prn, out_chips, n_chips)) return set_err(rc, "B1I PRN 1..37, at most 2047 chips");
    return GM_OK;
}

int gm_ca_code_row(int row, int8_t out[1023]) {
    if (row < 0 || row > 31 || !out) return set_err(GM_ERR_OUT_OF_RANGE, "row must be 0..31");
    memcpy(out, ca_table().rows[row], 1023);
    return GM_OK;
}

int gm_generate_ca_code_samples(uint8_t prn, float code_rate, float fs, int8_t* out, size_t cap, size_t* n_out) {
    if (prn < 1 || prn > 32) return set_err(GM_ERR_OUT_OF_RANGE, "prn must be 1..=32");
    const size_t n = num_samples_per_code(code_rate, fs, CA_LEN);
    if (n_out) *n_out = n;
    std::vector<int8_t> tmp(n);
    const int rc = resample_code(ca_table().rows[prn - 1], 1023, false, code_rate, fs, n, tmp.data());
    if (rc) return set_err(rc, "chip index reached 1023 (the reference panics)");
    if (out) memcpy(out, tmp.data(), n < cap ? n : cap);
// ... 30 lines not shown
}

int gm_fft_supported_sizes(uint32_t* sizes, int cap) { return gm::list_plans(sizes, cap); }

static bool pow2_split(size_t n, const gm::PlanOps** p1, const gm::PlanOps** p2) {
    if (n < 2 || (n & (n - 1)) || n > (size_t(1) << 28)) return false;
    for (size_t n2 = 256; n2 * n2 <= n || n2 <= 16384; n2 *= 2) {
        if (n % n2) continue;
        const size_t n1 = n / n2;
        if (n1 < n2) break;
        const gm::PlanOps *a = n1 <= 16384 ? gm::find_plan(int(n1)) : nullptr, *b = gm::find_plan(int(n2));
        if (a && b && a->big_cols && b->big_rows) { *p1 = a; *p2 = b; return true; }
    }
    return false;
}
static int fft_run_big(size_t n, int dir, cf* d_data, size_t batch, hipStream_t st) {
    const gm::PlanOps *p1 = nullptr, *p2 = nullptr;
    if (!pow2_split(n, &p1, &p2)) return set_err(GM_ERR_UNSUPPORTED_N, "no in-LDS FFT plan for this length");
    std::vector<cf> t1(size_t(p1->tw_total) + 1), t2(size_t(p2->tw_total) + 1);
    p1->fill_tw(t1.data(), dir != 0);
    p2->fill_tw(t2.data(), dir != 0);
    cf *d_t1 = nullptr, *d_t2 = nullptr, *d_b = nullptr;
    auto done = [&](int code) { hipFree(d_t1); hipFree(d_t2); hipFree(d_b); return code; };
    if (hipMalloc(&d_t1, t1.size() * 8) != hipSuccess || hipMalloc(&d_t2, t2.size() * 8) != hipSuccess || hipMalloc(&d_b, n * 8) != hipSuccess)
        return done(set_err(GM_ERR_NOMEM, "hipMalloc (long FFT)"));
    if (hipMemcpy(d_t1, t1.data(), t1.size() * 8, hipMemcpyHostToDevice) != hipSuccess ||
        hipMemcpy(d_t2, t2.data(), t2.size() * 8, hipMemcpyHostToDevice) != hipSuccess) return done(set_err(GM_ERR_HIP, "hipMemcpy"));
    for (size_t it = 0; it < batch; ++it) {
        cf* x = d_data + it * n;
        p1->big_cols(st, x, d_b, d_t1, uint32_t(p2->n), dir != 0);
        p2->big_rows(st, d_b, x, d_t2, uint32_t(p1->n), dir != 0);
    }
    if (hipGetLastError() != hipSuccess || hipStreamSynchronize(st) != hipSuccess) return done(set_err(GM_ERR_HIP, "long FFT kernels"));
    return done(GM_OK);
}

static int fft_run(size_t n, int dir, cf* d_data, size_t batch, hipStream_t st) {
    const gm::PlanOps* pl = gm::find_plan(int(n));
    if (!pl) return fft_run_big(n, dir, d_data, batch, st);
    std::vector<cf> tw(size_t(pl->tw_total) + 1);
    pl->fill_tw(tw.data(), dir != 0);
    cf* d_tw = nullptr;
    HIPC(hipMalloc(&d_tw, tw.size() * sizeof(cf)));
    HIPC(hipMemcpy(d_tw, tw.data(), tw.size() * sizeof(cf), hipMemcpyHostToDevice));
    pl->fft_batch(st, d_data, d_tw, dir != 0, int(batch));
    HIPC(hipGetLastError());
    HIPC(hipStreamSynchronize(st));
    hipFree(d_tw);
    return GM_OK;
}

static int fft_bluestein(size_t n, int dir, gm_c32* inout, size_t batch) {
    size_t L = 256;
    while (L < 2 * n - 1) L *= 2;
    {
        const gm::PlanOps *p1 = nullptr, *p2 = nullptr;
        while (L <= (size_t(1) << 24) && !gm::find_plan(int(L)) && !pow2_split(L, &p1, &p2)) L *= 2;
        if (L > (size_t(1) << 24))
            return set_err(GM_ERR_UNSUPPORTED_N, "length above 2^23: no FFT plan (Bluestein needs a power of two >= 2N - 1, at most 2^24)");
    }
    std::vector<cf> c(n), b(L, gm::cf_make(0.f, 0.f));
    for (size_t i = 0; i < n; ++i) {
        const double a = M_PI * double((uint64_t(i) * i) % (2 * n)) / double(n);
        c[i] = gm::cf_make(float(cos(a)), float(-sin(a)));
    }
    b[0] = gm::cf_make(1.f, 0.f);
    for (size_t i = 1; i < n; ++i) b[i] = b[L - i] = gm::cf_make(c[i].x, -c[i].y);
    cf *d_b = nullptr, *d_a = nullptr, *d_y = nullptr;
    int rc = GM_OK;
    auto done = [&](int code) { hipFree(d_b); hipFree(d_a); hipFree(d_y); return code; };
    if (hipMalloc(&d_b, L * 8) != hipSuccess || hipMalloc(&d_a, L * 8) != hipSuccess || hipMalloc(&d_y, L * 8) != hipSuccess)
        return done(set_err(GM_ERR_HIP, "hipMalloc"));
    if (hipMemcpy(d_b, b.data(), L * 8, hipMemcpyHostToDevice) != hipSuccess) return done(set_err(GM_ERR_HIP, "hipMemcpy"));
    if ((rc = fft_run(L, 0, d_b, 1, nullptr))) return done(rc);
    std::vector<cf> a(L), y(L);
    const float inv_l = 1.0f / float(L);
    for (size_t it = 0; it < batch; ++it) {
        gm_c32* x = inout + it * n;
        for (size_t i = 0; i < L; ++i) a[i] = gm::cf_make(0.f, 0.f);
        for (size_t i = 0; i < n; ++i) {
            const cf xi = gm::cf_make(x[i].re, dir ? -x[i].im : x[i].im);
            a[i] = gm::cf_make(xi.x * c[i].x - xi.y * c[i].y, xi.x * c[i].y + xi.y * c[i].x);
        }
        if (hipMemcpy(d_a, a.data(), L * 8, hipMemcpyHostToDevice) != hipSuccess) return done(set_err(GM_ERR_HIP, "hipMemcpy"));
        if ((rc = fft_run(L, 0, d_a, 1, nullptr))) return done(rc);
        gm::launch_apply_doppler(nullptr, d_a, d_b, d_y, L);
        if (hipGetLastError() != hipSuccess) return done(set_err(GM_ERR_HIP, "product kernel"));
        if ((rc = fft_run(L, 1, d_y, 1, nullptr))) return done(rc);
        if (hipMemcpy(y.data(), d_y, L * 8, hipMemcpyDeviceToHost) != hipSuccess) return done(set_err(GM_ERR_HIP, "hipMemcpy"));
        for (size_t k = 0; k < n; ++k) {
            const float yr = y[k].x * inv_l, yi = y[k].y * inv_l;
            const float re = yr * c[k].x - yi * c[k].y, im = yr * c[k].y + yi * c[k].x;
            x[k].re = re; x[k].im = dir ? -im : im;
        }
    }
    return done(GM_OK);
}

int gm_fft_c2c_f32(size_t n, int dir, gm_c32* inout, size_t batch) {
    if (!inout || !n || !batch) return set_err(GM_ERR_INVALID_ARG, "null or empty");
    if (int rc = ensure_device(g_device)) return rc;
    {
        const gm::PlanOps *p1 = nullptr, *p2 = nullptr;
        if (!gm::find_plan(int(n)) && !pow2_split(n, &p1, &p2)) return fft_bluestein(n, dir, inout, batch);
    }
    cf* d = nullptr;
    HIPC(hipMalloc(&d, n * batch * 8));
    HIPC(hipMemcpy(d, inout, n * batch * 8, hipMemcpyHostToDevice));
    const int rc = fft_run(n, dir, d, batch, nullptr);
    if (!rc) HIPC(hipMemcpy(inout, d, n * batch * 8, hipMemcpyDeviceToHost));
    hipFree(d);
    return rc;
}

int gm_fft_power_spectrum_f32(size_t n, gm_c32* inout, float* power) {
    if (!inout || !power || !n) return set_err(GM_ERR_INVALID_ARG, "null or empty");
    if (int rc = ensure_device(g_device)) return rc;
    const gm::PlanOps *pp1 = nullptr, *pp2 = nullptr;
    if (!gm::find_plan(int(n)) && !pow2_split(n, &pp1, &pp2)) {
        if (int rc = fft_bluestein(n, 0, inout, 1)) return rc;
        for (size_t i = 0; i < n; ++i) power[i] = inout[i].re * inout[i].re + inout[i].im * inout[i].im;
        return GM_OK;
    }
    cf* d = nullptr; float* dp = nullptr;
    HIPC(hipMalloc(&d, n * 8)); HIPC(hipMalloc(&dp, n * 4));
    HIPC(hipMemcpy(d, inout, n * 8, hipMemcpyHostToDevice));
    int rc = fft_run(n, 0, d, 1, nullptr);
    if (!rc) {
        gm::launch_power(nullptr, d, dp, n);
        HIPC(hipGetLastError());
        HIPC(hipMemcpy(inout, d, n * 8, hipMemcpyDeviceToHost));
        HIPC(hipMemcpy(power, dp, n * 4, hipMemcpyDeviceToHost));
    }
    hipFree(d); hipFree(dp);
    return rc;
}

int gm_rfft_f32(size_t n, const float* in, gm_c32* out) {
    if (!in || !out || !n) return set_err(GM_ERR_INVALID_ARG, "null or empty");
    std::vector<gm_c32> buf(n);
    for (size_t i = 0; i < n; ++i) { buf[i].re = in[i]; buf[i].im = 0.0f; }
    const int rc = gm_fft_c2c_f32(n, 0, buf.data(), 1);
    if (!rc) memcpy(out, buf.data(), (n / 2 + 1) * sizeof(gm_c32));
    return rc;
}

int gm_acq_destroy(gm_acq* a) {
    if (!a) return GM_OK;
    if (a->device >= 0) hipSetDevice(a->device);
    acq_edge_free(a->edge);
    hipFree(a->d_planes);
    if (a->d_long_code != a->d_code_fft) hipFree(a->d_long_code);
    hipFree(a->d_long_z); hipFree(a->d_long_part);
    hipFree(a->d_comp_tmp); hipFree(a->d_comp_twn); hipFree(a->d_code_comb); hipFree(a->d_split_scratch); hipFree(a->d_split_counter);
    hipFree(a->fine.d_chips); hipFree(a->fine.d_tw1); hipFree(a->fine.d_tw2); hipFree(a->fine.d_B); hipFree(a->fine.d_mean);
    hipFree(a->fine.d_rowmax); hipFree(a->fine.d_rowarg); hipFree(a->fine.d_sat_worker); hipFree(a->fine.d_sat_cp);
    hipFree(a->fine.d_peak_pow); hipFree(a->fine.d_peak_idx);
    if (a->device >= 0) hipSetDevice(a->device);
    hipFree(a->d_tw_mix);
    hipFree(a->d_tables); hipFree(a->d_tw_fwd); hipFree(a->d_tw_inv); hipFree(a->d_code_fft); hipFree(a->d_code_fft_paired); hipFree(a->d_order);
    hipFree(a->d_spectra); hipFree(a->d_rho); hipFree(a->d_table_freq); hipFree(a->d_code_samples); hipFree(a->d_samples);
    hipFree(a->d_metrics); hipFree(a->d_worker_list); if (a->d_results) hipHostFree(a->d_results);
    hipFree(a->d_prn_ids);
    for (auto& e : a->tm.ev) if (e) hipEventDestroy(e);
    if (a->ahead.side) { hipStreamSynchronize(a->ahead.side); hipStreamDestroy(a->ahead.side); }
    if (a->ahead.ev_s) hipEventDestroy(a->ahead.ev_s);
    if (a->ahead.ev_f) hipEventDestroy(a->ahead.ev_f);
    if (a->ahead.ev_in) hipEventDestroy(a->ahead.ev_in);
    hipFree(a->ahead.d_spectra_alt);
    if (a->own_stream && a->stream) hipStreamDestroy(a->stream);
    delete a;
    return GM_OK;
}

static int acq_choose(uint32_t n, int32_t any_length, gm_acq_plan* info, const gm::PlanOps** pl, const gm::CompOps** comp,
                      const gm::LongOps** lng) {
    gm_acq_plan o{GM_ACQ_FORM_LDS, n, 1, n};
    const gm::PlanOps* p = nullptr;
    const gm::CompOps* c = nullptr;
    const gm::LongOps* l = nullptr;
    if (!n) return GM_ERR_INVALID_ARG;
    if (n % 8) return GM_ERR_ALIGNMENT;
    if ((p = gm::find_plan(int(n)))) {
    } else if ((c = gm::find_comp(n))) {
        p = gm::find_plan(c->nb);
        o = gm_acq_plan{GM_ACQ_FORM_COMPOSITE, uint32_t(c->nb), uint32_t(c->q), n};
    } else if (any_length && n >= 1024 && n <= 262144) {
        int nl = 0;
        const gm::LongOps* bases = gm::long_bases(&nl);
        for (int i = 0; i < nl && !l; ++i)
            if (n % uint32_t(bases[i].nb) == 0 && n / uint32_t(bases[i].nb) <= 32) {
                l = &bases[i];
                o = gm_acq_plan{GM_ACQ_FORM_LONG, uint32_t(l->nb), n / uint32_t(l->nb), n};
            }
        if (!l) {
            uint64_t best = 0;
            for (int i = 0; i < nl; ++i) {
                const uint64_t nb = uint64_t(bases[i].nb), q = (2 * uint64_t(n) + nb - 1) / nb;
                if (q <= 32 && (!best || q * nb < best)) { best = q * nb; l = &bases[i]; }
            }
            if (l) o = gm_acq_plan{GM_ACQ_FORM_LONG_PADDED, uint32_t(l->nb), uint32_t(best / uint64_t(l->nb)), uint32_t(best)};
        }
        if (l) p = gm::find_plan(l->nb);
    }
    if (!p) return GM_ERR_UNSUPPORTED_N;
    if (info) *info = o;
    if (pl) *pl = p;
    if (comp) *comp = c;
    if (lng) *lng = l;
    return GM_OK;
}

int gm_acq_plan_info(uint32_t fft_size, int32_t any_length, gm_acq_plan* out) {
    const int rc = acq_choose(fft_size, any_length, out, nullptr, nullptr, nullptr);
    if (rc == GM_ERR_ALIGNMENT) return set_err(rc, "fft_size % 8 != 0");
    if (rc == GM_ERR_UNSUPPORTED_N) return set_err(rc, "no acquisition path for this fft_size (gm_acq_cfg.any_length: multiples of 8 in [1024, 262144])");
    if (rc) return set_err(rc, "fft_size is required");
    return GM_OK;
}

int gm_acq_create(const gm_acq_cfg* cfg, gm_acq** out) {
    if (!cfg || !out) return set_err(GM_ERR_INVALID_ARG, "null cfg/out");
    *out = nullptr;
    if (!cfg->fft_size || !cfg->n_integrations || !cfg->n_bins || !cfg->n_prn || !cfg->prn_ids)
        return set_err(GM_ERR_INVALID_ARG, "fft_size, n_integrations, n_bins, n_prn, prn_ids are required");
    if (!cfg->tables && !cfg->doppler_hz) return set_err(GM_ERR_INVALID_ARG, "doppler_hz or tables required");
    if (cfg->tables && !cfg->table_freq) return set_err(GM_ERR_INVALID_ARG, "table_freq required with tables");
    if (cfg->fft_size % 8) return set_err(GM_ERR_ALIGNMENT, "fft_size % 8 != 0");
    if (cfg->coherent_periods > uint32_t(gm::GM_COHERENT_MAX)) return set_err(GM_ERR_INVALID_ARG, "coherent_periods > 32");
    const gm::PlanOps* pl = nullptr;
    const gm::CompOps* comp = nullptr;
    const gm::LongOps* lng = nullptr;
    gm_acq_plan form{};
    if (acq_choose(cfg->fft_size, cfg->any_length, &form, &pl, &comp, &lng) != GM_OK) pl = nullptr;
    uint32_t comp_q = comp ? uint32_t(comp->q) : 1;
    if (pl && !comp && !lng && !cfg->strict_sum_order && !cfg->reference_products && gm::diag_int("GM_COMP_BASE", 0) > 0) {
        const gm::CompOps* c = gm::find_comp(cfg->fft_size);
        if (c && c->nb == gm::diag_int("GM_COMP_BASE", 0)) { comp = c; pl = gm::find_plan(c->nb); comp_q = uint32_t(c->q); }
    }
    if (!pl) return set_err(GM_ERR_UNSUPPORTED_N, cfg->any_length ? "no acquisition path for this fft_size (any_length: multiples of 8 in [1024, 262144])"
                                                                 : "no in-LDS FFT plan for this fft_size, nor Q x {16384, 16368, 16000, 8192, 8184, 8000, 6000, 5000, 4000} with Q in {2,3,4,5,6,8}");
    if (cfg->reference_products && (comp_q > 1 || lng))
        return set_err(GM_ERR_INVALID_ARG, "reference_products needs an fft_size with an in-LDS plan (gm_fft_supported_sizes)");
    if (int rc = ensure_device(g_device)) return rc;

    gm_acq* a = new gm_acq();
    a->device = g_device;
    a->cfg = *cfg;
    a->plan = pl;
    a->N = cfg->fft_size; a->D = cfg->n_bins; a->M = cfg->n_integrations; a->P = cfg->n_prn;
    a->K = cfg->coherent_periods > 1 ? cfg->coherent_periods : 1;
    a->Q = lng ? form.q : comp_q; a->Nb = uint32_t(pl->n); a->comp = comp;
    a->lng = lng;
    if (lng) {
        a->L = form.transform_len;
        a->long_lim = form.form == GM_ACQ_FORM_LONG_PADDED ? 2 * cfg->fft_size : cfg->fft_size;
        const double r = double(cfg->fft_size) / double(a->L);
        a->long_scale = float(r * r);
    }
    if (cfg->threshold == 0.0f) a->cfg.threshold = 7.0f;
    a->code_rate = cfg->codes ? (cfg->code_rate > 0 ? cfg->code_rate : CA_RATE) : CA_RATE;
    a->prn_ids.assign(cfg->prn_ids, cfg->prn_ids + a->P);
    const size_t N = a->N, D = a->D, M = a->M, P = a->P, K = a->K;
    int rc = GM_OK;
    auto fail = [&](int code) { gm_acq_destroy(a); return code; };

    std::vector<gm_c32> tables(D * N);
    a->table_freq.resize(D);
    if (cfg->tables) {
        memcpy(tables.data(), cfg->tables, D * N * sizeof(gm_c32));
        memcpy(a->table_freq.data(), cfg->table_freq, D * sizeof(float));
    } else {
        for (size_t d = 0; d < D; ++d)
            gm_doppler_table_new(cfg->f_if, cfg->doppler_hz[d], cfg->fs, N, &a->table_freq[d], &tables[d * N]);
    }
    std::vector<gm_c32> rho(D * K);
    for (size_t d = 0; d < D; ++d)
        for (size_t k = 0; k < K; ++k) {
            const double cyc = double(a->table_freq[d]) * double(k * N) / double(cfg->fs);
            const double ang = 2.0 * 3.14159265358979323846 * (cyc - ::floor(cyc));
            rho[d * K + k] = gm_c32{float(::cos(ang)), float(0.0 - ::sin(ang))};
        }
    std::vector<int8_t> code_samples(P * N);
    a->code_len = cfg->codes ? cfg->code_len : 1023u;
    a->chips.resize(P * size_t(a->code_len));
    for (size_t p = 0; p < P; ++p) {
        if (cfg->codes) {
            if (!cfg->code_len) return fail(set_err(GM_ERR_INVALID_ARG, "code_len required with codes"));
            memcpy(&a->chips[p * a->code_len], cfg->codes + p * cfg->code_len, cfg->code_len);
            rc = resample_code(cfg->codes + p * cfg->code_len, cfg->code_len, true, a->code_rate, cfg->fs, N,
                               &code_samples[p * N]);
        } else {
            const uint8_t prn = a->prn_ids[p];
            if (prn < 1 || prn > 32) return fail(set_err(GM_ERR_OUT_OF_RANGE, "prn must be 1..=32"));
            if (num_samples_per_code(CA_RATE, cfg->fs, CA_LEN) != N)
                return fail(set_err(GM_ERR_INVALID_ARG, "fft_size != round(fs / 1 kHz)"));
            memcpy(&a->chips[p * 1023], ca_table().rows[prn - 1], 1023);
            rc = resample_code(ca_table().rows[prn - 1], 1023, false, CA_RATE, cfg->fs, N, &code_samples[p * N]);
        }
        if (rc) return fail(set_err(rc, "code resampling index out of range"));
    }
    const bool twi_corr = acq_fused(a);
    std::vector<cf> twf(size_t(pl->tw_total) + 1), twi(size_t(twi_corr ? pl->tw_total_corr : pl->tw_total) + 1);
    pl->fill_tw(twf.data(), false);
    if (twi_corr) pl->fill_tw_corr(twi.data());
    else pl->fill_tw(twi.data(), true);
    std::vector<cf> twm(size_t(pl->tw_total_mix) + 1);
    pl->fill_tw_mix(twm.data(), false);

#define HIPA(expr)                                                     \
    do {                                                               \
        hipError_t _e = (expr);                                        \
        if (_e != hipSuccess) return fail(hip_fail(_e, #expr));        \
    } while (0)
    HIPA(hipStreamCreateWithFlags(&a->stream, hipStreamNonBlocking));
    a->own_stream = true;
    HIPA(hipMalloc(&a->d_tables, D * N * 8));
    HIPA(hipMalloc(&a->d_table_freq, D * 4));
    HIPA(hipMalloc(&a->d_tw_fwd, twf.size() * 8));
    HIPA(hipMalloc(&a->d_tw_inv, twi.size() * 8));
    HIPA(hipMalloc(&a->d_tw_mix, twm.size() * 8));
    HIPA(hipMalloc(&a->d_code_samples, P * N));
    HIPA(hipMalloc(&a->d_code_fft, P * N * 8));
    HIPA(hipMalloc(&a->d_spectra, D * M * (a->lng ? size_t(a->L) : N) * 8));
    a->samples_cap = K * M * N * 8;
    HIPA(hipMalloc(&a->d_samples, a->samples_cap));
    HIPA(hipMalloc(&a->d_metrics, 3 * P * D * 4));
    HIPA(hipMemsetAsync(a->d_metrics, 0, 3 * P * D * 4, a->stream));
    HIPA(hipMalloc(&a->d_worker_list, P * 4));
    HIPA(hipMalloc(&a->d_rho, D * K * 8));
    HIPA(hipMemcpy(a->d_rho, rho.data(), D * K * 8, hipMemcpyHostToDevice));
    if (acq_fused(a) && pl->split_slab && M >= 2) {
        size_t planes = size_t(8) * ((P * D + 7) / 8) * M;
        const size_t tail = size_t(8) * (64 + M);
        if (planes < tail) planes = tail;
        if (planes > size_t(gm::GM_CORR_SPLIT_MAX_SLABS)) planes = size_t(gm::GM_CORR_SPLIT_MAX_SLABS);
        a->split_planes = int(planes);
        HIPA(hipMalloc(&a->d_split_scratch, planes * pl->split_slab * sizeof(float)));
        HIPA(hipMalloc(&a->d_split_counter, gm::GM_CORR_SPLIT_MAX_ITEMS * sizeof(uint32_t)));
        HIPA(hipMemsetAsync(a->d_split_counter, 0, gm::GM_CORR_SPLIT_MAX_ITEMS * sizeof(uint32_t), a->stream));
    }
    HIPA(hipMemcpy(a->d_tables, tables.data(), D * N * 8, hipMemcpyHostToDevice));
    HIPA(hipMemcpy(a->d_table_freq, a->table_freq.data(), D * 4, hipMemcpyHostToDevice));
    HIPA(hipMemcpy(a->d_tw_fwd, twf.data(), twf.size() * 8, hipMemcpyHostToDevice));
    HIPA(hipMemcpy(a->d_tw_inv, twi.data(), twi.size() * 8, hipMemcpyHostToDevice));
    HIPA(hipMemcpy(a->d_tw_mix, twm.data(), twm.size() * 8, hipMemcpyHostToDevice));
    HIPA(hipMemcpy(a->d_code_samples, code_samples.data(), P * N, hipMemcpyHostToDevice));
    if ((rc = acq_reserve_results(a, uint32_t(P)))) return fail(rc);
    HIPA(hipMemcpy(a->d_prn_ids, a->prn_ids.data(), P, hipMemcpyHostToDevice));
    a->dev_prn_ids = a->prn_ids;
    int (*fill_order)(uint16_t*) = a->lng ? nullptr : (a->Q == 1 ? pl->fill_order : comp->fill_order);
    if (const int n_order = fill_order ? fill_order(nullptr) : 0) {
        std::vector<uint16_t> order(static_cast<size_t>(n_order), 0);
        fill_order(order.data());
        HIPA(hipMalloc(&a->d_order, order.size() * sizeof(uint16_t)));
        HIPA(hipMemcpy(a->d_order, order.data(), order.size() * sizeof(uint16_t), hipMemcpyHostToDevice));
    }
    if (a->lng) {
        const size_t L = a->L;
        if (L == N) a->d_long_code = a->d_code_fft;
        else HIPA(hipMalloc(&a->d_long_code, P * L * 8));
        a->lng->fwd_sub(a->stream, nullptr, GM_FMT_C32, nullptr, a->d_code_samples, a->d_tw_fwd, a->d_long_code, uint32_t(P), a->Q,
                        uint32_t(N), uint32_t(N), 1);
        gm::launch_long_fwd_post(a->stream, a->d_long_code, uint32_t(P), a->Q, a->Nb);
        size_t slab = (size_t(128) << 20) / (M * L * 8);
        if (slab < 1) slab = 1;
        if (slab > P * D) slab = P * D;
        if (slab * M > 65535) slab = 65535 / M;
        a->long_slab = uint32_t(slab);
        HIPA(hipMalloc(&a->d_long_z, slab * M * L * 8));
        HIPA(hipMalloc(&a->d_long_part, 3 * P * D * a->Q * 4));
        if (cfg->strict_sum_order) HIPA(hipMalloc(&a->d_planes, P * D * N * sizeof(float)));
        if (L != N) {
            std::vector<gm_c32> cb(P * N);
            for (size_t i = 0; i < P * N; ++i) { cb[i].re = float(code_samples[i]); cb[i].im = 0.0f; }
            HIPA(hipStreamSynchronize(a->stream));
            if ((rc = gm_fft_c2c_f32(N, 0, cb.data(), P))) return fail(rc);
            HIPA(hipMemcpy(a->d_code_fft, cb.data(), P * N * 8, hipMemcpyHostToDevice));
        }
    } else if (a->Q == 1) {
        pl->code_fft(a->stream, a->d_code_samples, a->d_tw_fwd, a->d_code_fft, int(P));
        HIPA(hipMalloc(&a->d_code_fft_paired, P * N * 8));
        pl->pair_codes(a->stream, a->d_code_fft, a->d_code_fft_paired, int(P));
    } else {
        const size_t tmp_items = D * M > P ? D * M : P;
        HIPA(hipMalloc(&a->d_comp_tmp, tmp_items * N * 8));
        if (cfg->strict_sum_order) HIPA(hipMalloc(&a->d_planes, P * D * N * sizeof(float)));
        HIPA(hipMalloc(&a->d_comp_twn, N * 8));
        HIPA(hipMalloc(&a->d_code_fft_paired, P * N * 8));
        std::vector<gm::cf> twn(N);
        comp->fill_twn(twn.data());
        HIPA(hipMemcpy(a->d_comp_twn, twn.data(), N * 8, hipMemcpyHostToDevice));
        comp->fwd_sub(a->stream, nullptr, GM_FMT_C32, nullptr, a->d_code_samples, a->d_tw_mix, a->d_comp_tmp, uint32_t(P), 1, nullptr);
        comp->fwd_post(a->stream, a->d_comp_tmp, a->d_code_fft, uint32_t(P), 0, nullptr);
        comp->relayout(a->stream, a->d_code_fft, a->d_code_fft_paired, int(P * a->Q));
        HIPA(hipMalloc(&a->d_code_comb, P * a->Q * N * 8));
        comp->comb(a->stream, a->d_code_fft_paired, a->d_comp_twn, a->d_code_comb, uint32_t(P));
        if (a->d_order) {
            gm::cf* comb2 = nullptr;
            HIPA(hipMalloc(&comb2, P * a->Q * N * 8));
            comp->fold_post(a->stream, a->d_code_comb, a->d_order, comb2, uint32_t(P));
            HIPA(hipStreamSynchronize(a->stream));
            hipFree(a->d_code_comb);
            a->d_code_comb = comb2;
            a->comp_post_folded = true;
        }
    }
    HIPA(hipGetLastError());
    HIPA(hipStreamSynchronize(a->stream));
    a->worker_list.clear();
    a->n_workers = 0xffffffffu;
    if ((rc = acq_set_mask(a, ~0ull))) return fail(rc);
#undef HIPA
    *out = a;
    return GM_OK;
}

int gm_acq_set_stream(gm_acq* a, void* s) {
    if (!a) return set_err(GM_ERR_INVALID_ARG, "null handle");
    if (a->dec_deferred) { if (int rc = ensure_device(a->device)) return rc; if (int rc = acq_flush_decision(a)) return rc; }
    if (a->own_stream && a->stream) { hipStreamSynchronize(a->stream); hipStreamDestroy(a->stream); }
    a->stream = reinterpret_cast<hipStream_t>(s);
    a->own_stream = false;
    return GM_OK;
}

int gm_acq_set_prn_mask(gm_acq* a, uint64_t mask) {
    if (!a) return set_err(GM_ERR_INVALID_ARG, "null handle");
    if (int rc = ensure_device(a->device)) return rc;
    return acq_set_mask(a, mask);
}

static gm::CohArgs acq_coh_args(const gm_acq* a, const void* d_samples, int fmt, const cf* tw_fwd, cf* out, uint32_t* clear_tickets) {
    gm::CohArgs c{};
    c.samples = d_samples; c.fmt = fmt; c.rho = a->d_rho; c.K = a->K; c.tables = a->d_tables; c.tw_fwd = tw_fwd; c.out = out;
    c.n_bins = a->D; c.n_int = a->M; c.Q = a->Q; c.N = a->N; c.lim = a->long_lim; c.clear_tickets = clear_tickets;
    c.order = a->lng ? nullptr : a->d_order;
    return c;
}

static int acq_search_common(gm_acq* a, const void* d_samples, int fmt, void* d_metrics, bool prepared) {
    uint32_t* const met_out = d_metrics ? static_cast<uint32_t*>(d_metrics) : a->d_metrics;
    const gm_acq::Edge& eg = a->edge;
    const bool edge = eg.H > 0;
    const uint32_t Dv = edge ? eg.H * a->D : a->D;
    uint32_t* met = edge ? eg.d_full : met_out;
    float* const planes = edge ? eg.d_planes : a->d_planes;
    const size_t PD = size_t(a->P) * Dv;
    const bool t = a->tm.on && (a->tm.calls++ % a->tm.stride == 0);
    a->tm.this_call = t;
    if (t) { if (int rc = acq_flush_decision(a)) return rc; }
    hipEvent_t* ev = t ? &a->tm.ev[size_t(a->tm.count % Timing::CAP) * 4] : nullptr;
    if (t) HIPC(hipEventRecord(ev[0], a->stream));
    gm_acq::Ahead& ah = a->ahead;
    bool tickets_cleared = a->d_split_counter != nullptr;
    if (prepared) {
        if (int rc = acq_flush_decision(a)) return rc;
        ah.valid = false;
        std::swap(a->d_spectra, ah.d_spectra_alt);
        HIPC(hipStreamWaitEvent(a->stream, ah.ev_f, 0));
        tickets_cleared = false;
    } else if (edge) {
        gm::EdgeArgs c{};
        c.samples = d_samples; c.fmt = fmt; c.rho = a->d_rho; c.K = a->K; c.offsets = eg.d_offsets; c.H = eg.H; c.neg = eg.neg;
        c.tables = a->d_tables; c.n_bins = a->D; c.n_int = a->M; c.Q = a->Q; c.N = a->N; c.lim = a->long_lim;
        c.order = a->lng ? nullptr : a->d_order;
        const uint32_t items = Dv * a->M;
        cf* const spectra = eg.d_spectra;
        if (a->lng) {
            c.tw_fwd = a->d_tw_fwd; c.out = spectra;
            eg.fwd(a->stream, c);
            for (uint32_t i0 = 0; i0 < items; i0 += 65535u)
                gm::launch_long_fwd_post(a->stream, spectra + size_t(i0) * a->L, items - i0 < 65535u ? items - i0 : 65535u, a->Q, a->Nb);
        } else if (a->Q == 1) {
            c.tw_fwd = a->d_tw_mix; c.out = spectra; c.clear_tickets = a->d_split_counter;
            eg.fwd(a->stream, c);
            a->dec_deferred = false;
        } else {
            c.tw_fwd = a->d_tw_mix; c.out = a->comp_post_folded ? spectra : eg.d_tmp;
            eg.fwd(a->stream, c);
            if (!a->comp_post_folded)
                for (uint32_t i0 = 0; i0 < items; i0 += 65535u)
                    a->comp->fwd_post(a->stream, eg.d_tmp + size_t(i0) * a->N, spectra + size_t(i0) * a->N,
                                      items - i0 < 65535u ? items - i0 : 65535u, 1, a->d_order);
        }
    } else if (a->lng) {
        if (a->K > 1)
            a->lng->fwd_sub_coh(a->stream, acq_coh_args(a, d_samples, fmt, a->d_tw_fwd, a->d_spectra, nullptr));
        else
            a->lng->fwd_sub(a->stream, d_samples, fmt, a->d_tables, nullptr, a->d_tw_fwd, a->d_spectra, a->D * a->M, a->Q, a->N, a->long_lim, a->M);
        gm::launch_long_fwd_post(a->stream, a->d_spectra, a->D * a->M, a->Q, a->Nb);
    } else if (a->Q == 1) {
        if (a->K > 1)
            a->plan->mix_fft_coh(a->stream, acq_coh_args(a, d_samples, fmt, a->d_tw_mix, a->d_spectra, a->d_split_counter));
        else
            a->plan->mix_fft(a->stream, d_samples, fmt, a->d_tables, a->d_tw_mix, a->d_spectra, int(a->D), int(a->M), a->d_split_counter, a->d_order,
                             a->dec_deferred ? &a->dec_args : nullptr);
        a->dec_deferred = false;
    } else {
        cf* sub = a->comp_post_folded ? a->d_spectra : a->d_comp_tmp;
        if (a->K > 1)
            a->comp->fwd_sub_coh(a->stream, acq_coh_args(a, d_samples, fmt, a->d_tw_mix, sub, nullptr));
        else
            a->comp->fwd_sub(a->stream, d_samples, fmt, a->d_tables, nullptr, a->d_tw_mix, sub, a->D * a->M, a->M, a->d_order);
        if (!a->comp_post_folded) {
            a->comp->fwd_post(a->stream, a->d_comp_tmp, a->d_spectra, a->D * a->M, 1, a->d_order);
        }
    }
    if (t) HIPC(hipEventRecord(ev[1], a->stream));
    if (ah.side) HIPC(hipEventRecord(ah.ev_s, a->stream));
    cf* const spectra = edge ? eg.d_spectra : a->d_spectra;
    if (a->lng) {
        if (a->n_workers) {
            const size_t part = size_t(a->P) * Dv * a->Q;
            float* const lp = edge ? eg.d_long_part : a->d_long_part;
            gm::LongCorrArgs la{};
            la.spectra = spectra; la.code_fft = a->d_long_code; la.tw_inv = a->d_tw_inv; la.Z = a->d_long_z;
            la.pmax = lp; la.parg = reinterpret_cast<uint32_t*>(lp + part); la.psum = lp + 2 * part;
            la.mmax = reinterpret_cast<float*>(met); la.margmax = met + PD; la.msum = reinterpret_cast<float*>(met + 2 * PD);
            la.planes = planes; la.worker_list = a->d_worker_list;
            la.n_workers = a->n_workers; la.n_bins = Dv; la.n_int = a->M; la.Q = a->Q; la.Nb = a->Nb; la.N = a->N;
            la.slab_items = a->long_slab; la.scale = a->long_scale;
            gm::launch_long_corr(a->stream, a->lng, la);
            if (planes)
                gm::launch_plane_strict_sum(a->stream, planes, reinterpret_cast<float*>(met + 2 * PD), a->d_worker_list, int(a->n_workers), int(Dv), uint32_t(a->N));
        }
    } else if (a->Q == 1) {
        a->plan->corr(a->stream, spectra, a->plan->code_paired ? a->d_code_fft_paired : a->d_code_fft, a->d_tw_inv, reinterpret_cast<float*>(met), met + PD,
                      reinterpret_cast<float*>(met + 2 * PD), a->d_worker_list, int(a->n_workers), int(Dv), int(a->M),
                      a->d_split_scratch, a->split_planes, a->d_split_counter, a->cfg.strict_sum_order ? 1 : 0, tickets_cleared ? 1 : 0,
                      a->cfg.reference_products ? 1 : 0);
    } else if (a->n_workers) {
        a->comp->corr(a->stream, spectra, a->d_code_comb, a->d_comp_twn, a->d_tw_inv, reinterpret_cast<float*>(met),
                      met + PD, reinterpret_cast<float*>(met + 2 * PD), a->d_worker_list, int(a->n_workers), int(Dv), int(a->M), planes);
        if (planes)
            gm::launch_plane_strict_sum(a->stream, planes, reinterpret_cast<float*>(met + 2 * PD), a->d_worker_list, int(a->n_workers), int(Dv), uint32_t(a->N));
    }
    if (edge) {
        gm::launch_edge_reduce(a->stream, eg.d_full, met_out, eg.d_choice, a->d_worker_list, a->n_workers, a->P, eg.H, a->D);
        met = met_out;
    }
    if (t) { HIPC(hipEventRecord(ev[2], a->stream)); a->tm.count++; a->tm.decide_valid = false; }
    HIPC(hipGetLastError());
    a->last_metrics = met;
    a->last_samples = d_samples; a->last_fmt = fmt;
    return GM_OK;
}

int gm_acq_search_dev(gm_acq* a, const void* d_samples, int fmt, void* d_metrics) {
    if (!a || !d_samples) return set_err(GM_ERR_INVALID_ARG, "null handle/samples");
    if (fmt < GM_FMT_C32 || fmt > GM_FMT_I8_REAL) return set_err(GM_ERR_INVALID_ARG, "bad sample format");
    if (int rc = ensure_device(a->device)) return rc;
    return acq_search_common(a, d_samples, fmt, d_metrics, false);
}

int gm_acq_search_prepared_dev(gm_acq* a, uint64_t token, void* d_metrics) {
    if (!a) return set_err(GM_ERR_INVALID_ARG, "null handle");
    gm_acq::Ahead& ah = a->ahead;
    if (!token || !ah.valid || ah.token != token)
        return set_err(GM_ERR_INVALID_ARG, "no such preparation (token stale, consumed, replaced or dropped)");
    if (int rc = ensure_device(a->device)) return rc;
    if (!acq_fused(a) || a->edge.H) {
        ah.valid = false;
        if (ah.comp_wait) { HIPC(hipStreamWaitEvent(a->stream, ah.ev_in, 0)); ah.comp_wait = false; }
        return acq_search_common(a, ah.samples, ah.fmt, d_metrics, false);
    }
    return acq_search_common(a, ah.samples, ah.fmt, d_metrics, true);
}

int gm_acq_drop_prepared(gm_acq* a) {
    if (!a) return set_err(GM_ERR_INVALID_ARG, "null handle");
    a->ahead.valid = false;
    return GM_OK;
}

int gm_acq_prepare_dev(gm_acq* a, const void* d_samples, int fmt, void* ready_stream, uint64_t* token) {
    if (!a || !d_samples || !token) return set_err(GM_ERR_INVALID_ARG, "null handle/samples/token");
    if (fmt < GM_FMT_C32 || fmt > GM_FMT_I8_REAL) return set_err(GM_ERR_INVALID_ARG, "bad sample format");
    *token = 0;
    gm_acq::Ahead& ah = a->ahead;
    if (int rc = ensure_device(a->device)) return rc;
    if (!acq_fused(a) || a->edge.H) {
        ah.valid = false; ah.comp_wait = false;
        if (ready_stream) {
            if (!ah.ev_in) HIPC(hipEventCreateWithFlags(&ah.ev_in, hipEventDisableTiming));
            HIPC(hipEventRecord(ah.ev_in, reinterpret_cast<hipStream_t>(ready_stream)));
            ah.comp_wait = true;
        }
        ah.valid = true; ah.samples = d_samples; ah.fmt = fmt; ah.token = *token = ah.next_token++;
        return GM_OK;
    }
    if (!ah.side) {
        cf* buf = nullptr; hipStream_t side = nullptr; hipEvent_t e[3] = {nullptr, nullptr, nullptr};
        int least = 0, greatest = 0;
        hipError_t er = hipMalloc(&buf, size_t(a->D) * a->M * a->N * 8);
        if (er == hipSuccess) er = hipDeviceGetStreamPriorityRange(&least, &greatest);
        if (er == hipSuccess) er = hipStreamCreateWithPriority(&side, hipStreamNonBlocking, gm::diag_int("GM_PREPARE_PRIORITY", least));
        for (int i = 0; i < 3 && er == hipSuccess; ++i) er = hipEventCreateWithFlags(&e[i], hipEventDisableTiming);
        if (er == hipSuccess) er = hipEventRecord(e[0], a->stream);
        if (er != hipSuccess) {
            for (hipEvent_t x : e) if (x) (void)hipEventDestroy(x);
            if (side) (void)hipStreamDestroy(side);
            if (buf) (void)hipFree(buf);
            return set_err(GM_ERR_HIP, hipGetErrorString(er));
        }
        ah.d_spectra_alt = buf; ah.side = side; ah.ev_s = e[0]; ah.ev_f = e[1]; ah.ev_in = e[2];
    }
    HIPC(hipStreamWaitEvent(ah.side, ah.ev_s, 0));
    if (ready_stream) {
        HIPC(hipEventRecord(ah.ev_in, reinterpret_cast<hipStream_t>(ready_stream)));
        HIPC(hipStreamWaitEvent(ah.side, ah.ev_in, 0));
    }
    ah.valid = false;
    if (a->K > 1)
        a->plan->mix_fft_coh(ah.side, acq_coh_args(a, d_samples, fmt, a->d_tw_mix, ah.d_spectra_alt, nullptr));
    else
        a->plan->mix_fft(ah.side, d_samples, fmt, a->d_tables, a->d_tw_mix, ah.d_spectra_alt, int(a->D), int(a->M), nullptr, a->d_order, nullptr);
    HIPC(hipEventRecord(ah.ev_f, ah.side));
    HIPC(hipGetLastError());
    ah.valid = true; ah.samples = d_samples; ah.fmt = fmt; ah.token = *token = ah.next_token++;
    return GM_OK;
}

int gm_acq_decide_dev(gm_acq* a, const void* d_metrics, uint32_t n_prn, const uint8_t* prn_ids, uint64_t local_tail) {
    if (!a || !n_prn) return set_err(GM_ERR_INVALID_ARG, "null handle / n_prn == 0");
    if (int rc = ensure_device(a->device)) return rc;
    if (int rc = acq_flush_decision(a)) return rc;
    if (int rc = acq_reserve_results(a, n_prn)) return rc;
    const uint32_t* met = d_metrics ? static_cast<const uint32_t*>(d_metrics) : a->d_metrics;
    const uint8_t* ids = prn_ids ? prn_ids : (n_prn == a->P ? a->prn_ids.data() : nullptr);
    if (!ids) return set_err(GM_ERR_INVALID_ARG, "prn_ids required when n_prn differs from the handle's");
    if (a->dev_prn_ids.size() != n_prn || memcmp(a->dev_prn_ids.data(), ids, n_prn) != 0) {
        a->dev_prn_ids.assign(ids, ids + n_prn);
        HIPC(hipMemcpyAsync(a->d_prn_ids, a->dev_prn_ids.data(), n_prn, hipMemcpyHostToDevice, a->stream));
        HIPC(hipStreamSynchronize(a->stream));
    }
    const size_t PD = size_t(n_prn) * a->D;
    gm::DecideArgs da;
    da.mmax = reinterpret_cast<const float*>(met);
    da.margmax = met + PD;
    da.msum = reinterpret_cast<const float*>(met + 2 * PD);
    da.table_freq = a->d_table_freq;
    da.prn_ids = a->d_prn_ids;
    da.mask_lo = (d_metrics && n_prn != a->P) ? ~0ull : a->mask;
    da.n_prn = int(n_prn); da.n_bins = int(a->D); da.fft_size = int(a->N);
    da.fs = a->cfg.fs; da.threshold = a->cfg.threshold; da.code_rate = a->code_rate;
    da.best_bin_mode = a->cfg.decision_mode == GM_DECIDE_BEST_BIN ? 1 : 0;
    da.local_tail = local_tail;
    da.results = a->d_results; da.found = a->d_found;
    if (a->defer_decisions && acq_fused(a) && a->K == 1 && !(a->tm.on && a->tm.this_call) && met == a->last_metrics && a->D <= 64) {
        a->dec_args = da;
        a->dec_deferred = true;
        return GM_OK;
    }
    gm::launch_decide(a->stream, da);
    if (a->tm.on && a->tm.this_call && a->tm.count > 0) {
        a->tm.this_call = false;
        HIPC(hipEventRecord(a->tm.ev[size_t((a->tm.count - 1) % Timing::CAP) * 4 + 3], a->stream));
        a->tm.decide_valid = true;
    }
    HIPC(hipGetLastError());
    return GM_OK;
}

int gm_acq_synchronize(gm_acq* a) {
    if (!a) return set_err(GM_ERR_INVALID_ARG, "null handle");
    if (int rc = ensure_device(a->device)) return rc;
    if (int rc = acq_flush_decision(a)) return rc;
    HIPC(hipStreamSynchronize(a->stream));
    return GM_OK;
}

int gm_acq_set_deferred_decision(gm_acq* a, int on) {
    if (!a) return set_err(GM_ERR_INVALID_ARG, "null handle");
    if (!on && a->dec_deferred) { if (int rc = ensure_device(a->device)) return rc; if (int rc = acq_flush_decision(a)) return rc; }
    a->defer_decisions = on != 0;
    return GM_OK;
}

int gm_acq_fetch_results(gm_acq* a, uint32_t n_prn, gm_acq_result* results, uint8_t* found) {
    if (!a || !results || !found) return set_err(GM_ERR_INVALID_ARG, "null pointer");
    if (n_prn > a->results_cap) return set_err(GM_ERR_INVALID_ARG, "n_prn exceeds the last decide call");
    if (int rc = ensure_device(a->device)) return rc;
    if (int rc = acq_flush_decision(a)) return rc;
// ... 136 lines not shown
    HIPC(hipMemcpyAsync(pw.data(), f.d_peak_pow, S * 4, hipMemcpyDeviceToHost, a->stream));
    HIPC(hipMemcpyAsync(pi.data(), f.d_peak_idx, S * 4, hipMemcpyDeviceToHost, a->stream));
    HIPC(hipStreamSynchronize(a->stream));
    const uint64_t fft_size = uint64_t(N1) * N2;
    const uint64_t one_side = uint64_t(ceilf((float(fft_size) + 1.0f) / 2.0f));
    for (uint32_t p = 0; p < n_prn; ++p) {
        if (slot[p] == 0xFFFFFFFFu) continue;
        const uint64_t idx = pi[slot[p]];
        if (peak_index) peak_index[p] = idx;
        if (peak_mag) peak_mag[p] = sqrtf(pw[slot[p]]);
        if (fine_freq_hz)
            fine_freq_hz[p] = idx > one_side ? -((float(fft_size - idx) * a->cfg.fs) / float(fft_size))
                                             : (float(idx) * a->cfg.fs) / float(fft_size);
    }
    }
    return GM_OK;
}

int gm_acq_search_c32(gm_acq* a, const gm_c32* s, size_t n, uint64_t tail, uint64_t mask, gm_acq_result* r, uint8_t* f) {
    return gm_acq_search(a, s, n, GM_FMT_C32, tail, mask, r, f);
}
int gm_acq_search_i8(gm_acq* a, const int8_t* s, size_t n, uint64_t tail, uint64_t mask, gm_acq_result* r, uint8_t* f) {
    return gm_acq_search(a, s, n, GM_FMT_I8_IQ, tail, mask, r, f);
}

int gm_acq_metrics(gm_acq* a, float* mx, uint32_t* am, float* sm) {
    if (!a) return set_err(GM_ERR_INVALID_ARG, "null handle");
    if (int rc = ensure_device(a->device)) return rc;
    HIPC(hipStreamSynchronize(a->stream));
    const size_t PD = size_t(a->P) * a->D;
    const uint32_t* met = a->last_metrics ? static_cast<const uint32_t*>(a->last_metrics) : a->d_metrics;
    if (mx) HIPC(hipMemcpy(mx, met, PD * 4, hipMemcpyDeviceToHost));
    if (am) HIPC(hipMemcpy(am, met + PD, PD * 4, hipMemcpyDeviceToHost));
    if (sm) HIPC(hipMemcpy(sm, met + 2 * PD, PD * 4, hipMemcpyDeviceToHost));
    return GM_OK;
}

int gm_acq_code_fft(gm_acq* a, uint32_t worker, gm_c32* out) {
    if (!a || !out || worker >= a->P) return set_err(GM_ERR_INVALID_ARG, "bad worker index");
    if (int rc = ensure_device(a->device)) return rc;
    HIPC(hipMemcpy(out, a->d_code_fft + size_t(worker) * a->N, size_t(a->N) * 8, hipMemcpyDeviceToHost));
    return GM_OK;
}

int gm_acq_tables(gm_acq* a, gm_c32* tables, float* freq) {
    if (!a) return set_err(GM_ERR_INVALID_ARG, "null handle");
    if (int rc = ensure_device(a->device)) return rc;
    if (tables) HIPC(hipMemcpy(tables, a->d_tables, size_t(a->D) * a->N * 8, hipMemcpyDeviceToHost));
    if (freq) memcpy(freq, a->table_freq.data(), a->D * sizeof(float));
    return GM_OK;
}

int gm_acq_coherent_phasors(gm_acq* a, gm_c32* out) {
    if (!a || !out) return set_err(GM_ERR_INVALID_ARG, "null handle/out");
    if (int rc = ensure_device(a->device)) return rc;
    HIPC(hipMemcpy(out, a->d_rho, size_t(a->D) * a->K * 8, hipMemcpyDeviceToHost));
    return GM_OK;
}

static int edge_check(uint32_t K, uint32_t n, const uint32_t* offsets, const int8_t* secondary, uint32_t* neg) {
    if (K < 2) return set_err(GM_ERR_INVALID_ARG, "the edge search needs a coherent handle (coherent_periods >= 2)");
    if (K > uint32_t(gm::GM_COHERENT_MAX)) return set_err(GM_ERR_INVALID_ARG, "coherent_periods > 32");
    if (n > 32) return set_err(GM_ERR_INVALID_ARG, "more than 32 edge offsets");
    if (!offsets) return set_err(GM_ERR_INVALID_ARG, "null offsets");
    for (uint32_t h = 0; h < n; ++h) {
        if (offsets[h] > 63) return set_err(GM_ERR_INVALID_ARG, "edge offset above 63 periods");
        if (h && offsets[h] <= offsets[h - 1]) return set_err(GM_ERR_INVALID_ARG, "edge offsets must ascend strictly");
    }
    *neg = 0;
    if (secondary)
        for (uint32_t k = 0; k < K; ++k) {
            if (secondary[k] != 1 && secondary[k] != -1) return set_err(GM_ERR_INVALID_ARG, "secondary row entries must be +1 or -1");
            if (secondary[k] < 0) *neg |= 1u << k;
        }
    return GM_OK;
}

int gm_acq_edge_dwell_periods(uint32_t coherent_periods, uint32_t n_integrations, uint32_t n_offsets, const uint32_t* offsets,
                              const int8_t* secondary, uint64_t* dwell_periods) {
    if (!dwell_periods || !n_integrations) return set_err(GM_ERR_INVALID_ARG, "null dwell_periods / n_integrations == 0");
    const uint32_t K = coherent_periods > 1 ? coherent_periods : 1;
    if (!n_offsets) {
        if (K > uint32_t(gm::GM_COHERENT_MAX)) return set_err(GM_ERR_INVALID_ARG, "coherent_periods > 32");
        *dwell_periods = uint64_t(K) * n_integrations;
        return GM_OK;
    }
    uint32_t neg = 0;
    if (int rc = edge_check(K, n_offsets, offsets, secondary, &neg)) return rc;
    *dwell_periods = uint64_t(K) * n_integrations + offsets[n_offsets - 1];
    return GM_OK;
}

int gm_acq_set_edge_search(gm_acq* a, uint32_t n_offsets, const uint32_t* offsets, const int8_t* secondary) {
    if (!a) return set_err(GM_ERR_INVALID_ARG, "null handle");
    uint32_t neg = 0;
    if (n_offsets)
        if (int rc = edge_check(a->K, n_offsets, offsets, secondary, &neg)) return rc;
    if (int rc = ensure_device(a->device)) return rc;
    if (int rc = acq_flush_decision(a)) return rc;
    a->ahead.valid = false;
    a->ahead.comp_wait = false;
    HIPC(hipStreamSynchronize(a->stream));
    if (!n_offsets) {
        if (a->edge.H) a->last_samples = nullptr;
        acq_edge_free(a->edge);
        return GM_OK;
    }
    gm_acq::Edge e;
    e.H = n_offsets; e.offsets.assign(offsets, offsets + n_offsets); e.o_max = offsets[n_offsets - 1]; e.neg = neg;
    e.fwd = a->lng ? gm::find_edge_long_fwd_sub(a->lng->nb) : (a->Q == 1 ? gm::find_edge_mix_fft(a->plan->n) : gm::find_edge_comp_fwd_sub(a->comp->nb));
    if (!e.fwd) return set_err(GM_ERR_UNSUPPORTED_N, "no edge-search stage F for this handle's base plan");
    const size_t H = n_offsets, D = a->D, M = a->M, P = a->P, N = a->N, T = a->lng ? size_t(a->L) : N;
    void* smp = nullptr;
    const size_t smp_bytes = (size_t(a->K) * M + e.o_max) * N * 8;
    bool ok = hipMalloc(&e.d_offsets, H * 4) == hipSuccess && hipMalloc(&e.d_spectra, H * D * M * T * 8) == hipSuccess &&
              hipMalloc(&e.d_full, 3 * P * H * D * 4) == hipSuccess && hipMalloc(&e.d_choice, P * D * 4) == hipSuccess;
    if (ok && a->Q > 1 && !a->lng && !a->comp_post_folded) ok = hipMalloc(&e.d_tmp, H * D * M * N * 8) == hipSuccess;
    if (ok && a->lng) ok = hipMalloc(&e.d_long_part, 3 * P * H * D * a->Q * 4) == hipSuccess;
    if (ok && a->d_planes) ok = hipMalloc(&e.d_planes, P * H * D * N * sizeof(float)) == hipSuccess;
    if (ok && smp_bytes > a->samples_cap) ok = hipMalloc(&smp, smp_bytes) == hipSuccess;
    if (ok) ok = hipMemset(e.d_full, 0, 3 * P * H * D * 4) == hipSuccess && hipMemset(e.d_choice, 0, P * D * 4) == hipSuccess &&
                 hipMemcpy(e.d_offsets, e.offsets.data(), H * 4, hipMemcpyHostToDevice) == hipSuccess;
    if (!ok) {
        (void)hipGetLastError();
        hipFree(smp);
        acq_edge_free(e);
        return set_err(GM_ERR_NOMEM, "the edge search's buffers do not fit (gnss_mi355x.h states the formula); the handle is as it was");
    }
    if (smp) { hipFree(a->d_samples); a->d_samples = smp; a->samples_cap = smp_bytes; }
    acq_edge_free(a->edge);
    a->edge = std::move(e);
    a->last_samples = nullptr;
    return GM_OK;
}

int gm_acq_edge_metrics(gm_acq* a, float* mx, uint32_t* am, float* sm) {
    if (!a) return set_err(GM_ERR_INVALID_ARG, "null handle");
    if (!a->edge.H) return set_err(GM_ERR_INVALID_ARG, "the edge search is off (gm_acq_set_edge_search)");
    if (int rc = ensure_device(a->device)) return rc;
    HIPC(hipStreamSynchronize(a->stream));
    const size_t n = size_t(a->P) * a->edge.H * a->D;
    if (mx) HIPC(hipMemcpy(mx, a->edge.d_full, n * 4, hipMemcpyDeviceToHost));
    if (am) HIPC(hipMemcpy(am, a->edge.d_full + n, n * 4, hipMemcpyDeviceToHost));
    if (sm) HIPC(hipMemcpy(sm, a->edge.d_full + 2 * n, n * 4, hipMemcpyDeviceToHost));
    return GM_OK;
}

int gm_acq_edge_choice(gm_acq* a, uint32_t* hypothesis) {
    if (!a || !hypothesis) return set_err(GM_ERR_INVALID_ARG, "null handle/out");
    if (!a->edge.H) return set_err(GM_ERR_INVALID_ARG, "the edge search is off (gm_acq_set_edge_search)");
    if (int rc = ensure_device(a->device)) return rc;
    HIPC(hipStreamSynchronize(a->stream));
    HIPC(hipMemcpy(hypothesis, a->edge.d_choice, size_t(a->P) * a->D * 4, hipMemcpyDeviceToHost));
    return GM_OK;
}

int gm_acq_result_offsets(gm_acq* a, const gm_acq_result* results, const uint8_t* found, uint32_t n_prn, uint32_t* offset_periods) {
    if (!a || !results || !found || !offset_periods) return set_err(GM_ERR_INVALID_ARG, "null pointer");
    if (!a->edge.H) return set_err(GM_ERR_INVALID_ARG, "the edge search is off (gm_acq_set_edge_search)");
    if (n_prn > a->P) return set_err(GM_ERR_INVALID_ARG, "n_prn exceeds the handle's workers");
    std::vector<uint32_t> choice(size_t(a->P) * a->D);
    if (int rc = gm_acq_edge_choice(a, choice.data())) return rc;
    for (uint32_t p = 0; p < n_prn; ++p) {
        if (!found[p]) continue;
        const int32_t d = results[p].doppler_bin;
        if (d < 0 || uint32_t(d) >= a->D) return set_err(GM_ERR_OUT_OF_RANGE, "result.doppler_bin outside the handle's bins");
        const uint32_t h = choice[size_t(p) * a->D + uint32_t(d)];
        offset_periods[p] = a->edge.offsets[h < a->edge.H ? h : 0];
    }
    return GM_OK;
}

int gm_acq_enable_timing(gm_acq* a, int on) {
    if (!a) return set_err(GM_ERR_INVALID_ARG, "null handle");
    if (int rc = ensure_device(a->device)) return rc;
    if (on && a->tm.ev.empty()) {
        a->tm.ev.assign(size_t(Timing::CAP) * 4, nullptr);
        for (auto& e : a->tm.ev) HIPC(hipEventCreate(&e));
    }
    a->tm.on = on != 0;
    a->tm.stride = on > 1 ? on : 1;
    a->tm.calls = 0;
    a->tm.this_call = false;
    a->tm.count = 0;
    a->tm.decide_valid = false;
    return GM_OK;
}

int gm_acq_last_timing(gm_acq* a, float* ms_mix, float* ms_corr, float* ms_decide) {
    if (!a || !a->tm.on || a->tm.count == 0) return set_err(GM_ERR_INVALID_ARG, "timing not enabled / nothing recorded");
    if (int rc = ensure_device(a->device)) return rc;
    HIPC(hipStreamSynchronize(a->stream));
    hipEvent_t* ev = &a->tm.ev[size_t((a->tm.count - 1) % Timing::CAP) * 4];
    float t = 0;
    if (ms_mix) { HIPC(hipEventElapsedTime(&t, ev[0], ev[1])); *ms_mix = t; }
    if (ms_corr) { HIPC(hipEventElapsedTime(&t, ev[1], ev[2])); *ms_corr = t; }
    if (ms_decide) {
        *ms_decide = 0;
        if (a->tm.decide_valid) { HIPC(hipEventElapsedTime(&t, ev[2], ev[3])); *ms_decide = t; }
    }
    return GM_OK;
}

int gm_acq_timing_summary(gm_acq* a, uint32_t* launches, float* avg_ms_mix, float* avg_ms_corr) {
    if (!a || !a->tm.on) return set_err(GM_ERR_INVALID_ARG, "timing not enabled");
    if (int rc = ensure_device(a->device)) return rc;
    HIPC(hipStreamSynchronize(a->stream));
    const int n = a->tm.count < Timing::CAP ? a->tm.count : Timing::CAP;
    double sm = 0, sc = 0;
    for (int i = 0; i < n; ++i) {
        hipEvent_t* ev = &a->tm.ev[size_t(i) * 4];
        float t = 0;
        HIPC(hipEventElapsedTime(&t, ev[0], ev[1])); sm += t;
        HIPC(hipEventElapsedTime(&t, ev[1], ev[2])); sc += t;
    }
    if (launches) *launches = uint32_t(n);
    if (avg_ms_mix) *avg_ms_mix = n ? float(sm / n) : 0.f;
    if (avg_ms_corr) *avg_ms_corr = n ? float(sc / n) : 0.f;
    return GM_OK;
}

int gm_acq_decide_host(const float* mmax, const uint32_t* margmax, const float* msum, const float* table_freq,
                       uint32_t n_prn, uint32_t n_bins, const uint8_t* prn_ids, uint32_t fft_size, float fs,
                       float code_rate, float threshold, uint64_t local_tail, gm_acq_result* results, uint8_t* found) {
    if (!mmax || !margmax || !msum || !table_freq || !prn_ids || !results || !found || fft_size < 2)
        return set_err(GM_ERR_INVALID_ARG, "null pointer");
    if (threshold == 0.0f) threshold = 7.0f;
    if (!(code_rate > 0.0f)) code_rate = CA_RATE;
    const float nm1 = float(fft_size - 1);
    for (uint32_t p = 0; p < n_prn; ++p) {
        gm_acq_result r;
        memset(&r, 0, sizeof(r));
        r.prn = prn_ids[p]; r.doppler_bin = -1;
        found[p] = 0;
        float gmax = 0.0f, bfreq = 0.0f, bsum = 0.0f;
        uint32_t bphase = 0;
        int bbin = -1;
        for (uint32_t d = 0; d < n_bins; ++d) {
            const size_t o = size_t(p) * n_bins + d;
            if (mmax[o] > gmax) { gmax = mmax[o]; bfreq = table_freq[d]; bphase = margmax[o]; bsum = msum[o]; bbin = int(d); }
            const float avg = (bsum - gmax) / nm1;
            if (gmax / avg > threshold) {
                r.code_phase_samples = bphase;
                r.code_phase_chips = float(bphase) * code_rate / fs;
                r.carrier_freq = bfreq; r.fs = fs; r.mag_relative = gmax;
                r.sample_global_index = local_tail + bphase; r.doppler_bin = bbin;
                found[p] = 1;
                break;
            }
        }
        results[p] = r;
    }
    return GM_OK;
}

int gm_acq_debug_stamps(gm_acq* a, long long* out) {
    if (!a) return set_err(GM_ERR_INVALID_ARG, "null handle");
    if (!gm::corr_stamps_built())
        return set_err(GM_ERR_UNSUPPORTED, "the stamped correlation kernels are in a diagnostic build only (GM_EXTRA_FLAGS=-DGM_DIAG_STAMPS, tools/README.md)");
    if (int rc = ensure_device(a->device)) return rc;
    static long long* d_st = nullptr;
    const size_t bytes = size_t(a->M) * 64 * sizeof(long long);
    if (!out) {
        if (d_st) { gm::set_corr_stamps(nullptr); hipFree(d_st); d_st = nullptr; }
        HIPC(hipMalloc(&d_st, bytes));
        HIPC(hipMemset(d_st, 0, bytes));
        HIPC(hipStreamSynchronize(nullptr));
        gm::set_corr_stamps(d_st);
        return GM_OK;
    }
    if (!d_st) return set_err(GM_ERR_INVALID_ARG, "stamps not armed");
    HIPC(hipStreamSynchronize(a->stream));
    HIPC(hipMemcpy(out, d_st, bytes, hipMemcpyDeviceToHost));
    gm::set_corr_stamps(nullptr);
    hipFree(d_st); d_st = nullptr;
    return GM_OK;
}

int gm_acq_manager_mode_for(size_t n) { return n == 0 ? 0 : (n <= 4 ? 1 : 2); }

int gm_acq_manager_pacing_and_list(int mode, uint32_t active, uint64_t* interval_ms, uint32_t* mask) {
    if (!interval_ms || !mask) return set_err(GM_ERR_INVALID_ARG, "null pointer");
    uint64_t interval; uint32_t size;
    switch (mode) {
        case 0: interval = 500; size = 32; break;
        case 1: interval = 1000; size = 8; break;
        case 2: interval = 2000; size = 5; break;
        default: return set_err(GM_ERR_INVALID_ARG, "mode must be 0..2");
    }
    uint32_t m = 0, taken = 0;
    for (uint32_t prn = 1; prn <= 32 && taken < size; ++prn)
        if (!((active >> (prn - 1)) & 1u)) { m |= 1u << (prn - 1); ++taken; }
    *interval_ms = interval; *mask = m;
    return GM_OK;
}

}


extern "C" {

int gm_ring_create(size_t buf_size, gm_ring** out) {
    if (!out) return set_err(GM_ERR_INVALID_ARG, "null out");
    *out = nullptr;
    if (!buf_size || (buf_size & (buf_size - 1))) return set_err(GM_ERR_INVALID_ARG, "Buffer size must be a power of two");
    if (int rc = ensure_device(g_device)) return rc;
// ... 1249 lines not shown
```

gnss-sdr-rs_amd/csrc/gm_internal.h:

```cpp
#pragma once
#include <hip/hip_runtime.h>
#include <stdint.h>

#include "../../include/gnss_mi355x.h"
#include "fft_core.h"

namespace gm {

struct FineArgs {
    const void* samples; int fmt;
    const float* mean;
    const int8_t* chips; uint32_t code_len; float code_rate, fs;
    const uint32_t* sat_worker;
    const uint32_t* sat_code_phase;
    uint32_t size_use, N1, N2;
    cf* B;
    const cf *tw1, *tw2;
    float* rowmax; uint32_t* rowarg;
};

constexpr int GM_COHERENT_MAX = 32;

struct CohArgs {
    const void* samples; int fmt;
    const cf* rho; uint32_t K;
    const cf* tables; const cf* tw_fwd;
    cf* out;
    uint32_t n_bins, n_int;
    uint32_t Q, N, lim;
    uint32_t* clear_tickets;
    const uint16_t* order;
};
template <class PL> void launch_mix_fft_coh(hipStream_t, const CohArgs&);
template <class PL> void launch_comp_fwd_sub_coh(hipStream_t, const CohArgs&);
template <class PL> void launch_long_fwd_sub_coh(hipStream_t, const CohArgs&);

struct EdgeArgs {
    const void* samples; int fmt;
    const cf* rho; uint32_t K;
    const uint32_t* offsets; uint32_t H;
    uint32_t neg;
    const cf* tables; const cf* tw_fwd;
    cf* out;
    uint32_t n_bins, n_int;
    uint32_t Q, N, lim;
    uint32_t* clear_tickets;
    const uint16_t* order;
};
typedef void (*EdgeLaunch)(hipStream_t, const EdgeArgs&);
EdgeLaunch find_edge_mix_fft(int n);
EdgeLaunch find_edge_comp_fwd_sub(int nb);
EdgeLaunch find_edge_long_fwd_sub(int nb);
void launch_edge_reduce(hipStream_t, const uint32_t* full, uint32_t* met, uint32_t* choice, const uint32_t* worker_list,
                        uint32_t n_workers, uint32_t P, uint32_t H, uint32_t D);

struct DecideArgs;
struct PlanOps {
    int n;
    int threads;
    int tw_total;
    int lds_bytes;
    int split_slab;
    int code_paired;
    void (*fill_tw)(cf* tw, bool inverse);
    int (*fill_order)(uint16_t* order);
    void (*mix_fft)(hipStream_t, const void* samples, int fmt, const cf* tables, const cf* tw_fwd,
                    cf* spectra, int n_bins, int n_int, uint32_t* clear_tickets, const uint16_t* order, const DecideArgs* dec);
    void (*corr)(hipStream_t, const cf* spectra, const cf* code_fft, const cf* tw_inv, float* mmax,
                 uint32_t* margmax, float* msum, const uint32_t* worker_list, int n_workers, int n_bins,
                 int n_int, float* split_scratch, int split_planes, uint32_t* split_counter, int strict_sum, int tickets_cleared,
                 int ref_mul);
    void (*code_fft)(hipStream_t, const int8_t* code_samples, const cf* tw_fwd, cf* code_fft, int n_codes);
    void (*pair_codes)(hipStream_t, const cf* natural, cf* paired, int n_codes);
    void (*fft_batch)(hipStream_t, cf* data, const cf* tw, int inverse, int batch);
    void (*fine_cols)(hipStream_t, const FineArgs&, int n_sats);
    void (*fine_rows)(hipStream_t, const FineArgs&, int n_sats);
    int fine_rows_per_wg;
    void (*big_cols)(hipStream_t, const cf* x, cf* B, const cf* tw, uint32_t n2, int inverse);
    void (*big_rows)(hipStream_t, const cf* B, cf* X, const cf* tw, uint32_t n1, int inverse);
    int tw_total_mix;
    void (*fill_tw_mix)(cf* tw, bool inverse);
    int tw_total_corr;
    void (*fill_tw_corr)(cf* tw);
    void (*mix_fft_coh)(hipStream_t, const CohArgs&);
};
void launch_fine_mean(hipStream_t, const void* samples, int fmt, uint32_t n, float* d_mean);
void launch_fine_final(hipStream_t, const float* rowmax, const uint32_t* rowarg, uint32_t n_rows, int n_sats,
                       float* peak_pow, uint32_t* peak_idx);
constexpr int GM_CORR_SPLIT_MAX_K = 16;
constexpr int GM_CORR_SPLIT_MAX_SLABS = 8 * 320;
constexpr int GM_CORR_SPLIT_MAX_ITEMS = 8 * 80;
int diag_int(const char* name, int dflt);
const PlanOps* find_plan(int n);
int list_plans(uint32_t* sizes, int cap);

void set_corr_stamps(long long* d_ptr);
bool corr_stamps_built();

struct CompOps {
    int nb, q;
    void (*fwd_sub)(hipStream_t, const void* samples, int fmt, const cf* tables, const int8_t* code_samples,
                    const cf* tw_fwd, cf* A, uint32_t n_items, uint32_t n_int, const uint16_t* order);
    void (*fwd_post)(hipStream_t, const cf* A, cf* X, uint32_t n_items, int paired, const uint16_t* order);
    void (*corr)(hipStream_t, const cf* spectra, const cf* code_paired, const cf* twn, const cf* tw_inv, float* mmax,
                 uint32_t* margmax, float* msum, const uint32_t* worker_list, int n_workers, int n_bins, int n_int, float* planes);
    void (*fill_twn)(cf* out);
    void (*comb)(hipStream_t, const cf* code_paired, const cf* twn, cf* comb, uint32_t n_codes);
    int (*fill_order)(uint16_t* order);
    void (*relayout)(hipStream_t, const cf* natural, cf* stored, int n_blocks);
    void (*fold_post)(hipStream_t, const cf* comb, const uint16_t* order, cf* comb2, uint32_t n_codes);
    void (*fwd_sub_coh)(hipStream_t, const CohArgs&);
};
const CompOps* find_comp(uint32_t n);
void launch_plane_strict_sum(hipStream_t, const float* planes, float* msum, const uint32_t* worker_list, int n_workers, int n_bins, uint32_t N);

struct LongOps {
    int nb;
    void (*fwd_sub)(hipStream_t, const void* samples, int fmt, const cf* tables, const int8_t* code_samples, const cf* tw_fwd,
                    cf* A, uint32_t n_items, uint32_t Q, uint32_t N, uint32_t lim, uint32_t n_int);
    void (*corr_inv)(hipStream_t, const cf* Z, const cf* tw_inv, float* pmax, uint32_t* parg, float* psum, float* planes,
                     const uint32_t* worker_list, uint32_t n_workers, uint32_t n_bins, uint32_t item0, uint32_t n_slab, uint32_t Q,
                     uint32_t N, uint32_t n_int, float scale);
    void (*fwd_sub_coh)(hipStream_t, const CohArgs&);
};
const LongOps* long_bases(int* n);
void launch_long_fwd_post(hipStream_t, cf* X, uint32_t n_items, uint32_t Q, uint32_t Nb);
struct LongCorrArgs {
    const cf* spectra;
    const cf* code_fft;
    const cf* tw_inv;
    cf* Z;
    float *pmax, *psum; uint32_t* parg;
    float *mmax, *msum; uint32_t* margmax;
    float* planes;
    const uint32_t* worker_list;
    uint32_t n_workers, n_bins, n_int, Q, Nb, N, slab_items;
    float scale;
};
void launch_long_corr(hipStream_t, const LongOps*, const LongCorrArgs&);

void launch_apply_doppler(hipStream_t, const cf* s, const cf* t, cf* out, size_t n);
void launch_power(hipStream_t, const cf* x, float* p, size_t n);

struct DecideArgs {
    const float* mmax; const uint32_t* margmax; const float* msum;
    const float* table_freq;
    const uint8_t* prn_ids;
    uint64_t mask_lo;
    int n_prn, n_bins, fft_size;
    float fs, threshold, code_rate;
    int best_bin_mode;
    uint64_t local_tail;
    gm_acq_result* results; uint8_t* found;
};
void launch_decide(hipStream_t, const DecideArgs&);

struct TrkDevCfg {
    float fs;
    int n_channels, n_arms;
    float el_space, vel_space;
    int code_index_mode, boc11;
    int code_len;
    float code_len_f;
    int gps_ca;
    int n_codes;
    float lock_threshold; uint32_t max_lost_epochs;
    float pll_tau1, pll_tau2, dll_tau1, dll_tau2, pll_dt, dll_dt;
    float nominal_code_rate;
    float inv_fs, inv_len, inv_2pi;
    float pll_dt_tau1, pll_tau2_tau1, dll_dt_tau1, dll_tau2_tau1;
    int div_fs_ok;
    int strict_libm;
    int strict_sum_order;
};
inline void fill_trk_derived(TrkDevCfg& d) {
    d.inv_fs = 1.0f / d.fs; d.inv_len = 1.0f / d.code_len_f; d.inv_2pi = 1.0f / (2.0f * 3.14159265358979323846f);
    d.pll_dt_tau1 = d.pll_dt / d.pll_tau1; d.pll_tau2_tau1 = d.pll_tau2 / d.pll_tau1;
    d.dll_dt_tau1 = d.dll_dt / d.dll_tau1; d.dll_tau2_tau1 = d.dll_tau2 / d.dll_tau1;
    uint32_t bits; __builtin_memcpy(&bits, &d.fs, 4);
    d.div_fs_ok = ((bits & 0x7fffffu) != 0x7fffffu && d.fs > 1.0f && d.fs < 1.0e12f) ? 1 : 0;
}
enum { TRK_MODE_CORRELATE = 0, TRK_MODE_DO_WORK = 1 };
struct TrkSrc {
    const cf* base; uint64_t mask; uint64_t head; int linear;
    int only_channel;
};
void launch_trk_epoch(hipStream_t, const TrkDevCfg&, const int8_t* d_codes, gm_trk_state* d_states,
                      const TrkSrc&, int slices, float* d_partials, uint8_t* d_ready, int mode,
                      gm_trk_out* d_outs, uint8_t* d_processed, uint8_t* d_lost, uint8_t* d_lost_prn,
                      float* d_terms = nullptr, size_t terms_cap = 0, int* d_error = nullptr);

#ifndef GM_TRK_THREADS
#define GM_TRK_THREADS 512
#define GM_TRK_WG_PER_CU 2
#endif
constexpr int TRK_PERSIST_THREADS = GM_TRK_THREADS;
constexpr int TRK_PERSIST_WG_PER_CU = GM_TRK_WG_PER_CU;

inline int trk_persistent_slots(int n_channels) { return (n_channels + 7) / 8 * 8; }
int trk_persistent_blocks_per_cu(const TrkDevCfg&);
int trk_persistent_granule_stride(int G);
void launch_trk_results_to_host(hipStream_t, const void* d_src, void* h_dst_pinned, size_t bytes, const void* d_src2 = nullptr, void* h_dst2_pinned = nullptr,
                                size_t bytes2 = 0);
void launch_trk_persistent(hipStream_t, const TrkDevCfg&, const int8_t* d_codes, gm_trk_state* d_states,
                           const cf* ring, uint64_t mask, uint64_t head, int G, int packed, int epochs, uint32_t tag_base,
                           unsigned long long* d_xchg, gm_trk_out* d_outs, uint8_t* d_processed, uint8_t* d_lost,
                           uint8_t* d_lost_prn, int* d_error, int* d_error_dev, long long* d_stamps);

struct FeState { float phase_accumulator; float bias_re[8]; float bias_im[8]; };
struct FrontendArgs {
    struct Stream {
        const void* in;
        void* out;
        uint64_t out_start, out_mask;
        size_t n_samples;
        FeState* state;
        float phase_step;
        int fast_fmod;
        const float* ph_table;
        uint32_t tab_len;
        uint32_t tab_lambda;
        uint32_t tab_pos;
        uint32_t tab_pos_end;
        float tab_scale;
    };
    const Stream* streams;
    Stream one;
    const float* lut;
    float alpha, con;
    int spec_k = 0, spec_poison = 0, spec_warm = 0;
    float* spec_buf = nullptr;
    unsigned int* spec_repairs = nullptr;
};
void launch_frontend_spec(hipStream_t, const FrontendArgs&, int fmt);
void launch_frontend(hipStream_t, const FrontendArgs&, int n_streams, int fmt);
void launch_frontend_fast(hipStream_t, const FrontendArgs&, int n_streams, int fmt);
constexpr int FE_SPEC_K_MAX = 64;
// ... 4 lines not shown
```

include/gnss_mi355x.h:

```cpp
#ifndef GNSS_MI355X_H
#define GNSS_MI355X_H

#include <stddef.h>
#include <stdint.h>

#ifdef __cplusplus
extern "C" {
#endif

#define GM_ABI_VERSION 9

typedef enum {
    GM_OK = 0,
    GM_ERR_INVALID_ARG = -1,
    GM_ERR_UNSUPPORTED_N = -2,
    GM_ERR_NO_DEVICE = -3,
    GM_ERR_HIP = -4,
    GM_ERR_OUT_OF_RANGE = -5,
    GM_ERR_ALIGNMENT = -6,
    GM_ERR_NOMEM = -7,
    GM_ERR_UNSUPPORTED = -8
} gm_status;

typedef struct { float re, im; } gm_c32;

int gm_abi_version(void);
int gm_init(int device);
int gm_device_count(int *count);
const char *gm_last_error(void);
const char *gm_status_string(int status);

int gm_ca_code_row(int row, int8_t out_chips[1023]);
int gm_b1i_code(uint32_t prn, int8_t *out_chips, uint32_t n_chips);
int gm_generate_ca_code_samples(uint8_t prn, float code_rate, float f_sampling, int8_t *out, size_t cap,
                                size_t *n_out);

int gm_doppler_table_new(float f_if, float doppler_freq_hz, float fs, size_t num_samples,
                         float *doppler_freq_hz_out, gm_c32 *table_out);
int gm_apply_doppler_shift(const gm_c32 *samples, const gm_c32 *table, gm_c32 *output, size_t n);

int gm_fft_c2c_f32(size_t n, int dir, gm_c32 *inout, size_t batch);
int gm_fft_power_spectrum_f32(size_t n, gm_c32 *inout, float *power);
int gm_rfft_f32(size_t n, const float *in, gm_c32 *out);
int gm_fft_supported_sizes(uint32_t *sizes, int cap);

typedef struct {
    uint8_t prn;
    uint64_t code_phase_samples;
    float code_phase_chips;
    float carrier_freq;
    float fs;
    float mag_relative;
    uint64_t sample_global_index;
    int32_t doppler_bin;
} gm_acq_result;

typedef enum { GM_FMT_C32 = 0, GM_FMT_I8_IQ = 1, GM_FMT_I8_REAL = 2 } gm_sample_format;

typedef struct {
    float fs;
    float f_if;
    uint32_t fft_size;
    uint32_t n_integrations;
    uint32_t n_bins;
    const float *doppler_hz;
    const gm_c32 *tables;
    const float *table_freq;
    uint32_t n_prn;
    const uint8_t *prn_ids;
    const int8_t *codes;
    uint32_t code_len;
    float code_rate;
    float threshold;
    int32_t decision_mode;
    int32_t strict_sum_order;
    int32_t reference_products;
    int32_t any_length;
    uint32_t coherent_periods;
} gm_acq_cfg;
typedef enum { GM_DECIDE_REFERENCE = 0, GM_DECIDE_BEST_BIN = 1 } gm_decision_mode;

typedef struct gm_acq gm_acq;

typedef enum {
    GM_ACQ_FORM_LDS = 0,
    GM_ACQ_FORM_COMPOSITE = 1,
    GM_ACQ_FORM_LONG = 2,
    GM_ACQ_FORM_LONG_PADDED = 3
} gm_acq_form;
typedef struct {
    int32_t form;
    uint32_t base;
    uint32_t q;
    uint32_t transform_len;
} gm_acq_plan;
int gm_acq_plan_info(uint32_t fft_size, int32_t any_length, gm_acq_plan *out);

int gm_acq_create(const gm_acq_cfg *cfg, gm_acq **out);
int gm_acq_destroy(gm_acq *a);

int gm_acq_search(gm_acq *a, const void *samples, size_t n_samples, int fmt, uint64_t local_tail,
                  uint64_t prn_mask, gm_acq_result *results, uint8_t *found);
int gm_acq_search_c32(gm_acq *a, const gm_c32 *samples, size_t n_samples, uint64_t local_tail,
                      uint64_t prn_mask, gm_acq_result *results, uint8_t *found);
int gm_acq_search_i8(gm_acq *a, const int8_t *iq_interleaved, size_t n_samples, uint64_t local_tail,
                     uint64_t prn_mask, gm_acq_result *results, uint8_t *found);

typedef struct gm_ring gm_ring;
int gm_acq_search_ring(gm_acq *a, gm_ring *ring, uint64_t prn_mask, gm_acq_result *results, uint8_t *found,
                       uint64_t *local_tail_out);

int gm_acq_finer_doppler(gm_acq *a, const gm_acq_result *results, const uint8_t *found, uint32_t n_prn,
                         float *fine_freq_hz, uint64_t *peak_index, float *peak_mag, uint64_t *fft_size);

int gm_acq_search_dev(gm_acq *a, const void *d_samples, int fmt, void *d_metrics);
int gm_acq_set_prn_mask(gm_acq *a, uint64_t prn_mask);
#define GM_COMM_ID_BYTES 128
typedef struct gm_comm gm_comm;
int gm_comm_get_unique_id(uint8_t id[GM_COMM_ID_BYTES]);
int gm_comm_init(int nranks, int rank, const uint8_t id[GM_COMM_ID_BYTES], gm_comm **out);
int gm_comm_destroy(gm_comm *c);
int gm_comm_info(gm_comm *c, int *nranks, int *rank);
int gm_acq_allgather_metrics(gm_acq *a, gm_comm *c, const void *d_local, void *d_all);
int gm_acq_allgather_metrics_async(gm_acq *a, gm_comm *c, const void *d_local, void *d_all);
int gm_comm_wait(gm_comm *c, void *hip_stream);
int gm_comm_allgather_words(gm_comm *c, const void *d_local, void *d_all, size_t words, void *hip_stream);
int gm_grid_assemble_dev(const void *d_gathered, uint32_t nranks, uint32_t p_max, uint32_t n_bins,
                         const uint32_t *d_row_map, uint32_t n_rows, void *d_out, void *hip_stream);
int gm_acq_decide_planes_dev(const float *d_max, const uint32_t *d_argmax, const float *d_sum, uint32_t n_prn,
                             uint32_t n_bins, const uint8_t *d_prn_ids, const float *d_table_freq, uint32_t fft_size,
                             float fs, float code_rate, float threshold, int decision_mode, uint64_t local_tail,
                             gm_acq_result *d_results, uint8_t *d_found, void *hip_stream);

int gm_acq_decide_dev(gm_acq *a, const void *d_metrics, uint32_t n_prn, const uint8_t *prn_ids,
                      uint64_t local_tail);
int gm_acq_fetch_results(gm_acq *a, uint32_t n_prn, gm_acq_result *results, uint8_t *found);
int gm_acq_decide_host(const float *max, const uint32_t *argmax, const float *sum, const float *table_freq,
                       uint32_t n_prn, uint32_t n_bins, const uint8_t *prn_ids, uint32_t fft_size, float fs,
                       float code_rate, float threshold, uint64_t local_tail, gm_acq_result *results,
                       uint8_t *found);
int gm_acq_synchronize(gm_acq *a);
int gm_acq_set_deferred_decision(gm_acq *a, int on);
int gm_acq_prepare_dev(gm_acq *a, const void *d_samples, int fmt, void *ready_stream, uint64_t *token);
int gm_acq_search_prepared_dev(gm_acq *a, uint64_t token, void *d_metrics);
int gm_acq_drop_prepared(gm_acq *a);
int gm_acq_set_stream(gm_acq *a, void *hip_stream);

int gm_acq_metrics(gm_acq *a, float *max, uint32_t *argmax, float *sum);
int gm_acq_code_fft(gm_acq *a, uint32_t worker, gm_c32 *out);
int gm_acq_tables(gm_acq *a, gm_c32 *tables, float *table_freq);
int gm_acq_coherent_phasors(gm_acq *a, gm_c32 *out);
int gm_acq_edge_dwell_periods(uint32_t coherent_periods, uint32_t n_integrations, uint32_t n_offsets,
                              const uint32_t *offsets, const int8_t *secondary, uint64_t *dwell_periods);
int gm_acq_set_edge_search(gm_acq *a, uint32_t n_offsets, const uint32_t *offsets, const int8_t *secondary);
int gm_acq_edge_metrics(gm_acq *a, float *max, uint32_t *argmax, float *sum);
int gm_acq_edge_choice(gm_acq *a, uint32_t *hypothesis);
int gm_acq_result_offsets(gm_acq *a, const gm_acq_result *results, const uint8_t *found, uint32_t n_prn,
                          uint32_t *offset_periods);
int gm_acq_enable_timing(gm_acq *a, int on);
int gm_acq_last_timing(gm_acq *a, float *ms_mix_fft, float *ms_corr, float *ms_decide);
int gm_acq_timing_summary(gm_acq *a, uint32_t *launches, float *avg_ms_mix_fft, float *avg_ms_corr);

int gm_acq_debug_stamps(gm_acq *a, long long *out);

int gm_acq_manager_mode_for(size_t tracked_count);
int gm_acq_manager_pacing_and_list(int mode, uint32_t active_prn_mask, uint64_t *interval_ms, uint32_t *mask);

int gm_ring_create(size_t buf_size, gm_ring **out);
int gm_ring_destroy(gm_ring *r);
int gm_ring_write_samples(gm_ring *r, const gm_c32 *samples, size_t n);
int gm_ring_get_head(gm_ring *r, uint64_t *head);
int gm_ring_copy_to_slice(gm_ring *r, uint64_t start, gm_c32 *dest, size_t n);
int gm_ring_write_samples_async(gm_ring *r, const gm_c32 *samples, size_t n);
int gm_ring_flush(gm_ring *r);
int gm_ring_get_enqueued_head(gm_ring *r, uint64_t *head);
int gm_ring_wait_head(gm_ring *r, uint64_t required_idx, uint32_t timeout_ms, int *reached);

typedef struct gm_frontend gm_frontend;
int gm_frontend_create(float f_if, float fs_in, float fs_out, gm_frontend **out);
int gm_frontend_destroy(gm_frontend *f);
int gm_frontend_lut(gm_frontend *f, float lut_re[2048], float lut_im[2048], float *phase_step);
int gm_frontend_get_state(gm_frontend *f, float *phase_accumulator, float bias_re[8], float bias_im[8]);
int gm_frontend_set_state(gm_frontend *f, float phase_accumulator, const float bias_re[8], const float bias_im[8]);
int gm_frontend_process_block(gm_frontend *f, float *raw_floats, size_t n_floats);
int gm_frontend_process_dev(gm_frontend *f, const void *d_in, int fmt, void *d_out, size_t n_samples, void *stream);
int gm_frontend_process_dev_batch(gm_frontend *const *fes, uint32_t n_streams, const void *const *d_in, int fmt,
                                  void *const *d_out, size_t n_samples, void *stream);
int gm_frontend_synchronize(gm_frontend *f);
int gm_frontend_write_ring(gm_frontend *f, gm_ring *ring, const void *samples, size_t n_samples, int fmt);
int gm_frontend_debug_repairs(gm_frontend *f, uint32_t *runs);

typedef struct {
    uint8_t prn;
    uint8_t active;
    uint8_t reserved[2];
    uint32_t lost_counter;
    uint64_t next_sample_index;
    uint64_t num_samples_per_code;
    float carrier_freq, carrier_phase, carrier_error, carrier_nco;
    float code_phase, code_error, code_nco, code_rate;
    float i_prompt, q_prompt;
} gm_trk_state;

typedef struct {
    float ip, qp, ie, qe, il, ql, ive, qve, ivl, qvl;
} gm_trk_out;

typedef enum { GM_CODE_INDEX_FAITHFUL = 0, GM_CODE_INDEX_FIXED = 1 } gm_code_index_mode;

typedef struct {
    float fs;
    uint32_t n_channels;
    uint32_t n_arms;
    float early_late_space;
    float very_early_late_space;
    int32_t code_index_mode;
    int32_t boc11;
    const int8_t *codes;
    uint32_t n_codes, code_len;
    float nominal_code_rate;
    float pll_bw, pll_zeta, pll_gain, dll_bw, dll_zeta, dll_gain, pll_dt, dll_dt;
    float lock_threshold;
    uint32_t max_lost_epochs;
    int32_t strict_libm;
    int32_t strict_sum_order;
    int32_t share_device;
} gm_trk_cfg;

typedef struct gm_trk gm_trk;

int gm_trk_create(const gm_trk_cfg *cfg, gm_trk **out);
int gm_trk_destroy(gm_trk *t);
int gm_trk_start(gm_trk *t, uint32_t ch, const gm_acq_result *r);
int gm_trk_reset(gm_trk *t, uint32_t ch);
int gm_trk_get_state(gm_trk *t, uint32_t ch, gm_trk_state *out);
int gm_trk_set_state(gm_trk *t, uint32_t ch, const gm_trk_state *in);
int gm_trk_get_states(gm_trk *t, gm_trk_state *out);
int gm_trk_set_states(gm_trk *t, const gm_trk_state *in, const uint8_t *which);
int gm_trk_get_ca_chip(gm_trk *t, uint32_t ch, float phase, float *chip);
int gm_loop_filter_new(float noise_bw, float damping, float gain, float *tau1, float *tau2);
float gm_loop_filter_update(float tau1, float tau2, float d_err, float err, float dt);

int gm_trk_correlate(gm_trk *t, uint32_t ch, const gm_c32 *samples, size_t n, gm_trk_out *out);
int gm_trk_do_work(gm_trk *t, uint32_t ch, const gm_c32 *samples, size_t n, gm_trk_out *out, uint8_t *lost,
                   uint8_t *lost_prn);
int gm_trk_update_all(gm_trk *t, gm_ring *ring, uint32_t max_epochs, gm_trk_out *outs, uint8_t *processed,
                      uint8_t *lost, uint32_t *epochs_done);
int gm_trk_update_all_dev(gm_trk *t, gm_ring *ring, uint32_t epochs);
int gm_trk_update_all_async(gm_trk *t, gm_ring *ring, uint32_t max_epochs, uint64_t *ticket);
int gm_trk_collect(gm_trk *t, uint64_t ticket, int wait, gm_trk_out *outs, uint8_t *processed, uint8_t *lost, gm_trk_state *states,
                   uint32_t *epochs_done, int *ready);
int gm_trk_synchronize(gm_trk *t);
int gm_trk_set_stream(gm_trk *t, void *hip_stream);
int gm_trk_debug_stamps(gm_trk *t, uint32_t cap, long long *out);
int gm_trk_enable_timing(gm_trk *t, int on);
int gm_trk_last_timing(gm_trk *t, float *ms_correlate_total, uint32_t *launches);

enum { GM_NAV_FAITHFUL = 0, GM_NAV_FIXED = 1 };
typedef struct gm_nav_sync gm_nav_sync;
typedef struct {
    uint8_t flag_bit_sync, flag_frame_sync, sync_sw;
    int8_t bit;
    int8_t polarity;
    uint32_t frame_sync_ind;
    uint64_t n_frame_bits;
    float i_p;
    uint64_t sf_cnt, sf_start_biti, tow_expected_ind;
} gm_nav_status;
int gm_nav_sync_create(int mode, gm_nav_sync **out);
int gm_nav_sync_destroy(gm_nav_sync *s);
int gm_nav_sync_update(gm_nav_sync *s, float old_i_prompt, float i_prompt, uint64_t cnt, uint64_t buff_loc,
                       gm_nav_status *out);
int gm_nav_sync_update_many(gm_nav_sync *s, float old_i_prompt0, const float *i_prompt, size_t stride, size_t n, uint64_t cnt0,
                            uint64_t buff_loc, gm_nav_status *out, int64_t *first_bit_sync, int64_t *first_frame_sync);
int gm_nav_sync_frame_bits(gm_nav_sync *s, int8_t *bits, size_t cap, size_t *n);
int gm_nav_sync_histogram(gm_nav_sync *s, uint64_t hist[20]);
int gm_nav_parity_check(const int8_t bits[32], int *ok, int *ref_sum_zero);

#ifdef __cplusplus
}
#endif
#endif
```

Before: 62.37 billion.

## Add persistent-block task schedule for correlation with head/tail integration splits

Introduces a host-built task table that makes each correlation workgroup loop over a list of tasks (whole items, or head/tail halves of the non-coherent integration range). The goal is to balance the last wave of correlation work across all XCD slots. A tail task polls a per-block flag and resumes from the head's partial accumulator in scratch. If the flag is not set after a few polls, it recomputes from m=0 instead. The path is gated on plan traits, LDS occupancy and a slack heuristic, and the table is rebuilt with a stream sync when the grid shape changes.

Result: slower. 57.67 billion (-7.5%).

```diff
diff --git a/gnss-sdr-rs_amd/_lib.py b/gnss-sdr-rs_amd/_lib.py
--- a/gnss-sdr-rs_amd/_lib.py
+++ b/gnss-sdr-rs_amd/_lib.py
@@ -125,6 +125,7 @@
     "gm_acq_set_edge_search": (_i, [_vp, _u32, _vp, _vp]),
     "gm_acq_edge_metrics": (_i, [_vp, _vp, _vp, _vp]),
     "gm_acq_edge_choice": (_i, [_vp, _vp]),
+    "gm_debug_corr_schedule": (_i, [_u32, _u32, _u32, _u32, _u32, _vp, _u32, C.POINTER(_u32)]),
     "gm_acq_result_offsets": (_i, [_vp, _vp, _vp, _u32, _vp]),
     "gm_acq_enable_timing": (_i, [_vp, _i]),
     "gm_acq_last_timing": (_i, [_vp, C.POINTER(_f), C.POINTER(_f), C.POINTER(_f)]),
diff --git a/gnss-sdr-rs_amd/build.py b/gnss-sdr-rs_amd/build.py
--- a/gnss-sdr-rs_amd/build.py
+++ b/gnss-sdr-rs_amd/build.py
@@ -7,8 +7,8 @@
 CSRC = os.path.join(HERE, "csrc")
 LIBDIR = os.path.join(HERE, "lib")
 LIB = os.path.join(LIBDIR, "libgnss_mi355x.so")
-SOURCES = ["acq_kernels.hip", "acq_composite.hip", "acq_long.hip", "acq_coherent.hip", "acq_edge.hip", "trk_kernels.hip", "fe_kernels.hip", "nav_host.hip", "gm_api.hip"]
-HEADERS = ["fft_core.h", "fft_plans.h", "acq_corr_plans.h", "gm_internal.h", "gm_libm.h", "acq_device.h", "acq_corr_ws31.h", "ws31_core.h", "acq_comp_ws.h", os.path.join("..", "..", "include", "gnss_mi355x.h")]
+SOURCES = ["acq_kernels.hip", "corr_sched.hip", "acq_composite.hip", "acq_long.hip", "acq_coherent.hip", "acq_edge.hip", "trk_kernels.hip", "fe_kernels.hip", "nav_host.hip", "gm_api.hip"]
+HEADERS = ["fft_core.h", "fft_plans.h", "acq_corr_plans.h", "gm_internal.h", "gm_libm.h", "acq_device.h", "acq_corr_ws31.h", "ws31_core.h", "acq_comp_ws.h", "corr_sched.h", os.path.join("..", "..", "include", "gnss_mi355x.h")]
 FLAGS = ["--offload-arch=gfx950", "-O3", "-std=c++17", "-ffp-contract=off", "-fno-slp-vectorize", "-fhip-fp32-correctly-rounded-divide-sqrt", "-fPIC",
          "-Wall", "-Wno-unused-function"]
 
diff --git a/gnss-sdr-rs_amd/csrc/acq_kernels.hip b/gnss-sdr-rs_amd/csrc/acq_kernels.hip
--- a/gnss-sdr-rs_amd/csrc/acq_kernels.hip
+++ b/gnss-sdr-rs_amd/csrc/acq_kernels.hip
@@ -1,4 +1,5 @@
 #include "acq_device.h"
+#include "corr_sched.h"
 
 namespace gm {
 
@@ -170,16 +171,38 @@
 void set_corr_stamps(long long*) {}
 #endif
 
-template <class PLX, bool KEEP_CODE, bool STAMPS, bool REF_MUL>
+template <class PLX, bool KEEP_CODE, bool STAMPS, bool REF_MUL, bool SCHED = false>
 __global__ __launch_bounds__(CorrPlanOf<PLX>::type::T, CorrPlanOf<PLX>::type::WAVES_PER_EU) void acq_corr_kernel(
     const cf* __restrict__ spectra, const cf* __restrict__ code_fft, const cf* __restrict__ tw_inv,
     float* __restrict__ mmax, uint32_t* __restrict__ margmax, float* __restrict__ msum,
     const uint32_t* __restrict__ worker_list, int n_workers, int n_bins, int n_int, int map_mode,
     int split_from, int split_k, int split_items, float* __restrict__ split_scratch, uint32_t* __restrict__ split_counter,
-    int strict_sum) {
+    int strict_sum, const uint32_t* __restrict__ sched, int sched_flags) {
     const int xcd = blockIdx.x & 7, wslot = blockIdx.x >> 3;
+    using PL = typename CorrPlanOf<PLX>::type;
+    constexpr bool PFA = CorrMode<PL>::PFA, HYB = CorrMode<PL>::HYBRID;
+    __shared__ cf lds[PL::LDS_ELEMS + ((PFA || HYB) ? 0 : PL::TW_TOTAL)];
+    __shared__ int s_last;
+    cf* tw = lds + PL::LDS_ELEMS;
+    const int tid0 = threadIdx.x;
+    if constexpr (SCHED && !PFA && !HYB) load_twiddles<PL>(tw, tw_inv, tid0);
+    constexpr int RL4 = (PL::RL + 3) / 4;
+    constexpr int SLAB = PL::ITL * RL4 * 4 * PL::T;
+    uint32_t t_at = 0, t_end = 1;
+    if constexpr (SCHED) { t_at = sched[blockIdx.x]; t_end = sched[blockIdx.x + 1]; }
+    do {
+    int tid = tid0;
+    if constexpr (SCHED) asm volatile("" : "+v"(tid));
     int slot = wslot, part = 0, parts = 1;
-    if (wslot >= split_from) {
+    uint32_t kind = CORR_TASK_WHOLE;
+    int task_m_begin = 0, task_m_end = n_int;
+    if constexpr (SCHED) {
+        const uint32_t task = sched[t_at];
+        slot = int(corr_task_item(task));
+        task_m_begin = int(corr_task_m_begin(task));
+        task_m_end = int(corr_task_m_end(task));
+        kind = corr_task_kind(task);
+    } else if (wslot >= split_from) {
         const int h = wslot - split_from;
         slot = split_from + h / split_k;
         part = h % split_k;
@@ -220,12 +243,7 @@
         }
     }
 
-    using PL = typename CorrPlanOf<PLX>::type;
-    constexpr bool PFA = CorrMode<PL>::PFA, HYB = CorrMode<PL>::HYBRID;
-    __shared__ cf lds[PL::LDS_ELEMS + ((PFA || HYB) ? 0 : PL::TW_TOTAL)];
-    cf* tw = lds + PL::LDS_ELEMS;
-    const int tid = threadIdx.x;
-    if constexpr (!PFA && !HYB) load_twiddles<PL>(tw, tw_inv, tid);
+    if constexpr (!SCHED && !PFA && !HYB) load_twiddles<PL>(tw, tw_inv, tid);
     constexpr int NB0 = PL::NB(0), NBL = PL::NB(PL::NP - 1);
     auto last_active = [&](int it) { if constexpr (HYB) return PL::last_active(tid); else return tid + it * PL::T < NBL; };
     auto out_index = [&](int it, int r) {
@@ -256,17 +274,50 @@
         }
     }
     float acc[PL::ITL][PL::RL];
-#pragma unroll
-    for (int it = 0; it < PL::ITL; ++it)
-#pragma unroll
-        for (int r = 0; r < PL::RL; ++r) acc[it][r] = 0.0f;
+    const int m_per = n_int / parts;
+    int m_begin = part * m_per, m_end = m_begin + m_per;
+    if constexpr (!SCHED) {
+#pragma unroll
+        for (int it = 0; it < PL::ITL; ++it)
+#pragma unroll
+            for (int r = 0; r < PL::RL; ++r) acc[it][r] = 0.0f;
+    } else {
+        constexpr int POLLS = 8;
+        int have = 0;
+        if (kind == CORR_TASK_TAIL) {
+            if (tid == 0) {
+                int ok = 0;
+                if (!(sched_flags & 1)) {
+                    for (int i = 0; i < POLLS && !ok; ++i) {
+                        ok = __hip_atomic_load(split_counter + (blockIdx.x - 8), __ATOMIC_RELAXED, __HIP_MEMORY_SCOPE_AGENT) != 0u;
+                        if (!ok) __builtin_amdgcn_s_sleep(8);
+                    }
+                }
+                s_last = ok;
+            }
+            __syncthreads();
+            have = __builtin_amdgcn_readfirstlane(s_last);
+        }
+        m_begin = (kind == CORR_TASK_TAIL && !have) ? 0 : task_m_begin;
+        m_end = task_m_end;
+        const size_t plane = have ? size_t(blockIdx.x - 8) : 0;
+        const __amdgpu_buffer_rsrc_t prs = make_rsrc(split_scratch + plane * SLAB, have ? unsigned(SLAB) * 4u : 0u);
+#pragma unroll
+        for (int it = 0; it < PL::ITL; ++it)
+#pragma unroll
+            for (int r4 = 0; r4 < RL4; ++r4) {
+                const u32x4 v = __builtin_amdgcn_raw_buffer_load_b128(prs, tid * 16 + (it * RL4 + r4) * PL::T * 16, 0, 16);
+                if (4 * r4 + 0 < PL::RL) acc[it][4 * r4 + 0] = __uint_as_float(v.x);
+                if (4 * r4 + 1 < PL::RL) acc[it][4 * r4 + 1 < PL::RL ? 4 * r4 + 1 : 0] = __uint_as_float(v.y);
+                if (4 * r4 + 2 < PL::RL) acc[it][4 * r4 + 2 < PL::RL ? 4 * r4 + 2 : 0] = __uint_as_float(v.z);
+                if (4 * r4 + 3 < PL::RL) acc[it][4 * r4 + 3 < PL::RL ? 4 * r4 + 3 : 0] = __uint_as_float(v.w);
+            }
+    }
 
     long long* stbase = nullptr;
     if constexpr (STAMPS) stbase = (blockIdx.x == 0 && (tid & 63) == 0 && PL::T / 64 <= 8) ? g_corr_stamps : nullptr;
     const int wv = tid >> 6;
-    const int m_per = n_int / parts, m_begin = part * m_per, m_end = m_begin + m_per;
     constexpr bool CAN_SPLIT = !STAMPS;
-    constexpr int RL4 = (PL::RL + 3) / 4;
     auto acc_or_zero = [&](int it, int r) { return r < PL::RL ? acc[it][r < PL::RL ? r : 0] : 0.0f; };
 #ifndef GM_CORR_PREFETCH_PAIRS
 #define GM_CORR_PREFETCH_PAIRS 4
@@ -329,25 +380,32 @@
         }
     }
 
-    if constexpr (CAN_SPLIT) {
+    auto store_plane = [&](const __amdgpu_buffer_rsrc_t& srs, int voff) {
+#pragma unroll
+        for (int it = 0; it < PL::ITL; ++it)
+#pragma unroll
+            for (int r4 = 0; r4 < RL4; ++r4) {
+                u32x4 v;
+                v.x = __float_as_uint(acc_or_zero(it, 4 * r4 + 0)); v.y = __float_as_uint(acc_or_zero(it, 4 * r4 + 1));
+                v.z = __float_as_uint(acc_or_zero(it, 4 * r4 + 2)); v.w = __float_as_uint(acc_or_zero(it, 4 * r4 + 3));
+                __builtin_amdgcn_raw_buffer_store_b128(v, srs, voff + (it * RL4 + r4) * PL::T * 16, 0, 16);
+                asm volatile("s_nop 1" ::: "memory");
+            }
+        asm volatile("s_waitcnt vmcnt(0)" ::: "memory");
+        __syncthreads();
+    };
+    if constexpr (SCHED) {
+        if (kind == CORR_TASK_HEAD) {
+            store_plane(make_rsrc(split_scratch + size_t(blockIdx.x) * SLAB, unsigned(SLAB) * 4u), tid * 16);
+            if (tid == 0) __hip_atomic_store(split_counter + blockIdx.x, 1u, __ATOMIC_RELAXED, __HIP_MEMORY_SCOPE_AGENT);
+            continue;
+        }
+    }
+    if constexpr (CAN_SPLIT && !SCHED) {
         if (parts > 1) {
-            constexpr int SLAB = PL::ITL * RL4 * 4 * PL::T;
             const size_t item_plane0 = (size_t(xcd) * split_items + (slot - split_from)) * size_t(n_int);
             const __amdgpu_buffer_rsrc_t srs = make_rsrc(split_scratch + item_plane0 * SLAB, unsigned(n_int) * SLAB * 4u);
-            const int voff = tid * 16 + part * SLAB * 4;
-#pragma unroll
-            for (int it = 0; it < PL::ITL; ++it)
-#pragma unroll
-                for (int r4 = 0; r4 < RL4; ++r4) {
-                    u32x4 v;
-                    v.x = __float_as_uint(acc_or_zero(it, 4 * r4 + 0)); v.y = __float_as_uint(acc_or_zero(it, 4 * r4 + 1));
-                    v.z = __float_as_uint(acc_or_zero(it, 4 * r4 + 2)); v.w = __float_as_uint(acc_or_zero(it, 4 * r4 + 3));
-                    __builtin_amdgcn_raw_buffer_store_b128(v, srs, voff + (it * RL4 + r4) * PL::T * 16, 0, 16);
-                    asm volatile("s_nop 1" ::: "memory");
-                }
-            asm volatile("s_waitcnt vmcnt(0)" ::: "memory");
-            __syncthreads();
-            __shared__ int s_last;
+            store_plane(srs, tid * 16 + part * SLAB * 4);
             if (tid == 0) {
                 uint32_t* cnt = split_counter + size_t(xcd) * split_items + (slot - split_from);
                 const uint32_t old = __hip_atomic_fetch_add(cnt, 1u, __ATOMIC_RELAXED, __HIP_MEMORY_SCOPE_AGENT);
@@ -474,6 +532,8 @@
         const size_t o = size_t(p) * n_bins + d;
         mmax[o] = fv; margmax[o] = fi; msum[o] = strict_sum ? strict_total : fs;
     }
+    if constexpr (SCHED) __syncthreads();
+    } while (SCHED && ++t_at < t_end);
 }
 
 }
@@ -718,21 +778,37 @@
         else return generic;
     }
     static constexpr int SPLIT_SLAB = slab();
+    static constexpr bool SCHED_OK = !WS31 && CP::WG_PER_CU == 2 && SPLIT_SLAB > 0 && PL::N != 8192;
     static void corr(hipStream_t st, const cf* spectra, const cf* code_fft, const cf* tw_inv, float* mmax,
                      uint32_t* margmax, float* msum, const uint32_t* worker_list, int n_workers, int n_bins,
                      int n_int, float* split_scratch, int split_planes, uint32_t* split_counter, int strict_sum, int tickets_cleared,
-                     int ref_mul) {
+                     int ref_mul, const uint32_t* sched, int sched_flags) {
         if (n_workers <= 0) return;
         static const int forced = diag_int("GM_CORR_MAP", -1);
-        const int per_xcd_bins = ((n_bins + 7) / 8) * n_workers, per_xcd_even = (n_bins * n_workers + 7) / 8;
+        const int per_xcd_even = (n_bins * n_workers + 7) / 8;
         const int slots = 32 * CP::WG_PER_CU;
-        const int q = n_bins / 8, left = (n_bins - 8 * q) * n_workers;
-        const int per_xcd_mixed = q * n_workers + (left + 7) / 8;
-        int map_mode = ((per_xcd_bins + slots - 1) / slots > (per_xcd_even + slots - 1) / slots) ? 0 : 1;
-        if (map_mode == 1 && per_xcd_mixed < per_xcd_bins) map_mode = 2;
-        if (forced >= 0) map_mode = forced;
+        int share_of_map = 0;
+        int map_mode = corr_map_mode(n_workers, n_bins, slots, &share_of_map);
         static const int cb_env = diag_int("GM_CORR_CB", -1);
         int cb = cb_env >= 0 ? cb_env : 0;
+        if constexpr (SCHED_OK) {
+            if (sched && forced < 0 && cb == 0 && !g_corr_stamps_armed && !strict_sum && split_scratch && split_counter &&
+                split_planes >= 8 * slots && 8 * slots <= GM_CORR_SPLIT_MAX_ITEMS) {
+                if (!tickets_cleared) (void)hipMemsetAsync(split_counter, 0, size_t(GM_CORR_SPLIT_MAX_ITEMS) * sizeof(uint32_t), st);
+                if (ref_mul)
+                    hipLaunchKernelGGL((acq_corr_kernel<PL, CP::KEEP_CODE, false, true, true>), dim3(8 * slots), dim3(PL::T), 0, st,
+                                       spectra, code_fft, tw_inv, mmax, margmax, msum, worker_list, n_workers, n_bins, n_int, map_mode,
+                                       share_of_map, 1, 0, split_scratch, split_counter, 0, sched, sched_flags);
+                else
+                    hipLaunchKernelGGL((acq_corr_kernel<PL, CP::KEEP_CODE, false, false, true>), dim3(8 * slots), dim3(PL::T), 0, st,
+                                       spectra, code_fft, tw_inv, mmax, margmax, msum, worker_list, n_workers, n_bins, n_int, map_mode,
+                                       share_of_map, 1, 0, split_scratch, split_counter, 0, sched, sched_flags);
+                return;
+            }
+        }
+        if (forced >= 0) map_mode = forced;
+        const int per_xcd_bins = ((n_bins + 7) / 8) * n_workers;
+        const int per_xcd_mixed = (n_bins / 8) * n_workers + ((n_bins - 8 * (n_bins / 8)) * n_workers + 7) / 8;
         int share = map_mode == 0 ? per_xcd_even : (map_mode == 1 ? per_xcd_bins : per_xcd_mixed);
         if (cb > 0) {
             const int rows_max = (per_xcd_even + n_workers - 2) / n_workers + 1;
@@ -776,7 +852,7 @@
         if (g_corr_stamps_armed) {
             hipLaunchKernelGGL((acq_corr_kernel<PL, CP::KEEP_CODE, true, false>), dim3(grid), dim3(PL::T), 0, st,
                                spectra, code_fft, tw_inv, mmax, margmax, msum, worker_list, n_workers, n_bins, n_int, map_mode,
-                               split_from, split_k, split_items, split_scratch, split_counter, strict_sum);
+                               split_from, split_k, split_items, split_scratch, split_counter, strict_sum, nullptr, 0);
             return;
         }
 #endif
@@ -789,11 +865,11 @@
             if (ref_mul)
                 hipLaunchKernelGGL((acq_corr_kernel<PL, CP::KEEP_CODE, false, true>), dim3(grid), dim3(PL::T), 0, st,
                                    spectra, code_fft, tw_inv, mmax, margmax, msum, worker_list, n_workers, n_bins, n_int, map_mode,
-                                   split_from, split_k, split_items, split_scratch, split_counter, strict_sum);
+                                   split_from, split_k, split_items, split_scratch, split_counter, strict_sum, nullptr, 0);
             else
                 hipLaunchKernelGGL((acq_corr_kernel<PL, CP::KEEP_CODE, false, false>), dim3(grid), dim3(PL::T), 0, st,
                                    spectra, code_fft, tw_inv, mmax, margmax, msum, worker_list, n_workers, n_bins, n_int, map_mode,
-                                   split_from, split_k, split_items, split_scratch, split_counter, strict_sum);
+                                   split_from, split_k, split_items, split_scratch, split_counter, strict_sum, nullptr, 0);
         }
     }
     static void code_fft(hipStream_t st, const int8_t* code_samples, const cf* tw_fwd, cf* out, int n_codes) {
@@ -831,7 +907,7 @@
                        &fill_tw, &fill_order, &mix_fft, &corr, &code_fft, &pair_codes, &fft_batch,
                        POW2 ? &fine_cols : nullptr, POW2 ? &fine_rows : nullptr, FineRows<PL>::RT,
                        POW2 ? &big_cols : nullptr, POW2 ? &big_rows : nullptr, MP::TW_TOTAL, &fill_tw_mix, corr_tw_total(), &fill_tw_corr,
-                       &launch_mix_fft_coh<PL>};
+                       &launch_mix_fft_coh<PL>, SCHED_OK ? 32 * CP::WG_PER_CU : 0};
     }
 };
 
diff --git a/gnss-sdr-rs_amd/csrc/corr_sched.h b/gnss-sdr-rs_amd/csrc/corr_sched.h
--- /dev/null
+++ b/gnss-sdr-rs_amd/csrc/corr_sched.h
@@ -0,0 +1,24 @@
+#pragma once
+#include <cstdint>
+#include <vector>
+
+namespace gm {
+
+enum : uint32_t { CORR_TASK_WHOLE = 0, CORR_TASK_HEAD = 1, CORR_TASK_TAIL = 2 };
+constexpr uint32_t CORR_TASK_ITEM_MAX = 0xffffu;
+constexpr uint32_t corr_task_pack(uint32_t item, uint32_t m_begin, uint32_t m_end, uint32_t kind) {
+    return item | (m_begin << 16) | (m_end << 21) | (kind << 26);
+}
+constexpr uint32_t corr_task_item(uint32_t t) { return t & 0xffffu; }
+constexpr uint32_t corr_task_m_begin(uint32_t t) { return (t >> 16) & 31u; }
+constexpr uint32_t corr_task_m_end(uint32_t t) { return (t >> 21) & 31u; }
+constexpr uint32_t corr_task_kind(uint32_t t) { return (t >> 26) & 3u; }
+
+int corr_map_mode(int n_workers, int n_bins, int slots, int* share);
+int corr_xcd_items(int map_mode, int n_workers, int n_bins, int xcd);
+
+bool corr_sched_build(const int items_per_xcd[8], int slots, int n_int, std::vector<uint32_t>& table);
+bool corr_sched_build_grid(int n_workers, int n_bins, int slots, int n_int, std::vector<uint32_t>& table);
+long corr_sched_slack_times_slots(int n_workers, int n_bins, int slots, int n_int);
+
+}
diff --git a/gnss-sdr-rs_amd/csrc/corr_sched.hip b/gnss-sdr-rs_amd/csrc/corr_sched.hip
--- /dev/null
+++ b/gnss-sdr-rs_amd/csrc/corr_sched.hip
@@ -0,0 +1,86 @@
+#include "corr_sched.h"
+
+namespace gm {
+
+int corr_map_mode(int n_workers, int n_bins, int slots, int* share) {
+    const int per_xcd_bins = ((n_bins + 7) / 8) * n_workers, per_xcd_even = (n_bins * n_workers + 7) / 8;
+    const int q = n_bins / 8, left = (n_bins - 8 * q) * n_workers;
+    const int per_xcd_mixed = q * n_workers + (left + 7) / 8;
+    int map_mode = ((per_xcd_bins + slots - 1) / slots > (per_xcd_even + slots - 1) / slots) ? 0 : 1;
+    if (map_mode == 1 && per_xcd_mixed < per_xcd_bins) map_mode = 2;
+    if (share) *share = map_mode == 0 ? per_xcd_even : (map_mode == 1 ? per_xcd_bins : per_xcd_mixed);
+    return map_mode;
+}
+
+static int clampi(int v, int lo, int hi) { return v < lo ? lo : (v > hi ? hi : v); }
+
+int corr_xcd_items(int map_mode, int n_workers, int n_bins, int xcd) {
+    if (n_workers <= 0 || n_bins <= 0 || xcd < 0 || xcd > 7) return 0;
+    if (map_mode == 0) {
+        const int items = n_bins * n_workers, share = (items + 7) >> 3;
+        return clampi(items - xcd * share, 0, share);
+    }
+    if (map_mode == 1) return ((n_bins + 7 - xcd) / 8) * n_workers;
+    if (map_mode == 2) {
+        const int q = n_bins >> 3, left = (n_bins - 8 * q) * n_workers, each = (left + 7) >> 3;
+        return q * n_workers + clampi(left - xcd * each, 0, each);
+    }
+    return 0;
+}
+
+bool corr_sched_build(const int items_per_xcd[8], int slots, int n_int, std::vector<uint32_t>& table) {
+    table.clear();
+    const int L = slots, M = n_int;
+    if (L <= 0 || M < 2 || M > 16) return false;
+    for (int x = 0; x < 8; ++x)
+        if (items_per_xcd[x] < L || uint32_t(items_per_xcd[x] - 1) > CORR_TASK_ITEM_MAX) return false;
+    std::vector<std::vector<uint32_t>> lists(size_t(8) * L);
+    for (int x = 0; x < 8; ++x) {
+        const int S = items_per_xcd[x], R = S / L - 1, first = R * L;
+        const long T = long(S - first) * M;
+        for (int s = 0; s < L; ++s) {
+            std::vector<uint32_t>& out = lists[size_t(s) * 8 + x];
+            for (int r = 0; r < R; ++r) out.push_back(corr_task_pack(uint32_t(r * L + s), 0, uint32_t(M), CORR_TASK_WHOLE));
+            const long a = s * T / L, b = (s + 1) * T / L;
+            const int i0 = int(a / M), ma = int(a % M), i1 = int(b / M), mb = int(b % M);
+            if (mb) out.push_back(corr_task_pack(uint32_t(first + i1), 0, uint32_t(mb), CORR_TASK_HEAD));
+            for (int i = ma ? i0 + 1 : i0; i < i1; ++i) out.push_back(corr_task_pack(uint32_t(first + i), 0, uint32_t(M), CORR_TASK_WHOLE));
+            if (ma) out.push_back(corr_task_pack(uint32_t(first + i0), uint32_t(ma), uint32_t(M), CORR_TASK_TAIL));
+        }
+    }
+    const size_t n_wg = size_t(8) * L;
+    size_t total = n_wg + 1;
+    for (const auto& l : lists) total += l.size();
+    table.resize(total);
+    uint32_t at = uint32_t(n_wg + 1);
+    for (size_t b = 0; b < n_wg; ++b) {
+        table[b] = at;
+        for (uint32_t t : lists[b]) table[at++] = t;
+    }
+    table[n_wg] = at;
+    return true;
+}
+
+bool corr_sched_build_grid(int n_workers, int n_bins, int slots, int n_int, std::vector<uint32_t>& table) {
+    table.clear();
+    if (n_workers <= 0 || n_bins <= 0 || slots <= 0) return false;
+    const int mode = corr_map_mode(n_workers, n_bins, slots, nullptr);
+    int S[8];
+    for (int x = 0; x < 8; ++x) S[x] = corr_xcd_items(mode, n_workers, n_bins, x);
+    return corr_sched_build(S, slots, n_int, table);
+}
+
+long corr_sched_slack_times_slots(int n_workers, int n_bins, int slots, int n_int) {
+    if (n_workers <= 0 || n_bins <= 0 || slots <= 0) return -1;
+    const int mode = corr_map_mode(n_workers, n_bins, slots, nullptr);
+    long least = -1;
+    for (int x = 0; x < 8; ++x) {
+        const int S = corr_xcd_items(mode, n_workers, n_bins, x);
+        if (S < slots) return -1;
+        const long slack = long(S - (S / slots - 1) * slots) * n_int - long(slots) * n_int;
+        if (least < 0 || slack < least) least = slack;
+    }
+    return least;
+}
+
+}
diff --git a/gnss-sdr-rs_amd/csrc/gm_api.hip b/gnss-sdr-rs_amd/csrc/gm_api.hip
--- a/gnss-sdr-rs_amd/csrc/gm_api.hip
+++ b/gnss-sdr-rs_amd/csrc/gm_api.hip
@@ -13,6 +13,7 @@
 #include <vector>
 
 #include "gm_internal.h"
+#include "corr_sched.h"
 
 using gm::cf;
 
@@ -294,6 +295,13 @@
     float* d_split_scratch = nullptr;
     int split_planes = 0;
     uint32_t* d_split_counter = nullptr;
+    struct CorrSched {
+        uint32_t n_workers = 0, n_bins = 0, n_int = 0;
+        bool valid = false, scheduled = false;
+        std::vector<uint32_t> host;
+        uint32_t* d_table = nullptr;
+        size_t cap_words = 0;
+    } csched;
     uint32_t Q = 1, Nb = 0;
     const gm::CompOps* comp = nullptr;
     cf* d_comp_tmp = nullptr;
@@ -630,7 +638,7 @@
     hipFree(a->d_planes);
     if (a->d_long_code != a->d_code_fft) hipFree(a->d_long_code);
     hipFree(a->d_long_z); hipFree(a->d_long_part);
-    hipFree(a->d_comp_tmp); hipFree(a->d_comp_twn); hipFree(a->d_code_comb); hipFree(a->d_split_scratch); hipFree(a->d_split_counter);
+    hipFree(a->d_comp_tmp); hipFree(a->d_comp_twn); hipFree(a->d_code_comb); hipFree(a->d_split_scratch); hipFree(a->d_split_counter); hipFree(a->csched.d_table);
     hipFree(a->fine.d_chips); hipFree(a->fine.d_tw1); hipFree(a->fine.d_tw2); hipFree(a->fine.d_B); hipFree(a->fine.d_mean);
     hipFree(a->fine.d_rowmax); hipFree(a->fine.d_rowarg); hipFree(a->fine.d_sat_worker); hipFree(a->fine.d_sat_cp);
     hipFree(a->fine.d_peak_pow); hipFree(a->fine.d_peak_idx);
@@ -915,6 +923,38 @@
     c.n_bins = a->D; c.n_int = a->M; c.Q = a->Q; c.N = a->N; c.lim = a->long_lim; c.clear_tickets = clear_tickets;
     c.order = a->lng ? nullptr : a->d_order;
     return c;
+}
+
+constexpr long GM_CORR_SCHED_MIN_SLACK = 2;
+static int acq_corr_sched(gm_acq* a, uint32_t n_bins, const uint32_t** sched, int* sched_flags) {
+    *sched = nullptr; *sched_flags = 0;
+    const int slots = a->plan->corr_sched_slots;
+    static const int env = gm::diag_int("GM_CORR_SCHED", -1);
+    static const bool reshaped = gm::diag_int("GM_CORR_MAP", -1) >= 0 || gm::diag_int("GM_CORR_CB", -1) >= 0 ||
+                                 gm::diag_int("GM_CORR_SPLIT", -1) >= 0 || gm::diag_int("GM_CORR_SPLIT_ITEMS", -1) >= 0;
+    if (!slots || env == 0 || (reshaped && env < 0) || a->cfg.strict_sum_order || !a->n_workers || a->M < 2 || a->M > uint32_t(gm::GM_CORR_SPLIT_MAX_K) ||
+        !a->d_split_scratch || !a->d_split_counter || a->split_planes < 8 * slots || 8 * slots > gm::GM_CORR_SPLIT_MAX_ITEMS)
+        return GM_OK;
+    gm_acq::CorrSched& cs = a->csched;
+    if (!cs.valid || cs.n_workers != a->n_workers || cs.n_bins != n_bins || cs.n_int != a->M) {
+        HIPC(hipStreamSynchronize(a->stream));
+        cs.valid = false;
+        const long slack = gm::corr_sched_slack_times_slots(int(a->n_workers), int(n_bins), slots, int(a->M));
+        const bool two_fill_the_cu = 3 * a->plan->lds_bytes > 160 * 1024;
+        cs.scheduled = slack >= 0 && (env >= 1 || (two_fill_the_cu && slack >= GM_CORR_SCHED_MIN_SLACK * slots)) &&
+                       gm::corr_sched_build_grid(int(a->n_workers), int(n_bins), slots, int(a->M), cs.host);
+        if (cs.scheduled) {
+            if (cs.host.size() > cs.cap_words) {
+                hipFree(cs.d_table); cs.d_table = nullptr; cs.cap_words = 0;
+                HIPC(hipMalloc(&cs.d_table, cs.host.size() * sizeof(uint32_t)));
+                cs.cap_words = cs.host.size();
+            }
+            HIPC(hipMemcpyAsync(cs.d_table, cs.host.data(), cs.host.size() * sizeof(uint32_t), hipMemcpyHostToDevice, a->stream));
+        }
+        cs.n_workers = a->n_workers; cs.n_bins = n_bins; cs.n_int = a->M; cs.valid = true;
+    }
+    if (cs.scheduled) { *sched = cs.d_table; *sched_flags = env == 2 ? 1 : 0; }
+    return GM_OK;
 }
 
 static int acq_search_common(gm_acq* a, const void* d_samples, int fmt, void* d_metrics, bool prepared) {
@@ -1004,10 +1044,13 @@
                 gm::launch_plane_strict_sum(a->stream, planes, reinterpret_cast<float*>(met + 2 * PD), a->d_worker_list, int(a->n_workers), int(Dv), uint32_t(a->N));
         }
     } else if (a->Q == 1) {
+        const uint32_t* sched = nullptr;
+        int sched_flags = 0;
+        if (int rc = acq_corr_sched(a, Dv, &sched, &sched_flags)) return rc;
         a->plan->corr(a->stream, spectra, a->plan->code_paired ? a->d_code_fft_paired : a->d_code_fft, a->d_tw_inv, reinterpret_cast<float*>(met), met + PD,
                       reinterpret_cast<float*>(met + 2 * PD), a->d_worker_list, int(a->n_workers), int(Dv), int(a->M),
                       a->d_split_scratch, a->split_planes, a->d_split_counter, a->cfg.strict_sum_order ? 1 : 0, tickets_cleared ? 1 : 0,
-                      a->cfg.reference_products ? 1 : 0);
+                      a->cfg.reference_products ? 1 : 0, sched, sched_flags);
     } else if (a->n_workers) {
         a->comp->corr(a->stream, spectra, a->d_code_comb, a->d_comp_twn, a->d_tw_inv, reinterpret_cast<float*>(met),
                       met + PD, reinterpret_cast<float*>(met + 2 * PD), a->d_worker_list, int(a->n_workers), int(Dv), int(a->M), planes);
@@ -1450,6 +1493,24 @@
     if (int rc = ensure_device(a->device)) return rc;
     HIPC(hipStreamSynchronize(a->stream));
     HIPC(hipMemcpy(hypothesis, a->edge.d_choice, size_t(a->P) * a->D * 4, hipMemcpyDeviceToHost));
+    return GM_OK;
+}
+
+int gm_debug_corr_schedule(uint32_t items, uint32_t n_workers, uint32_t n_bins, uint32_t n_integrations, uint32_t slots,
+                           uint32_t* table, uint32_t cap_words, uint32_t* n_words) {
+    if (!n_words) return set_err(GM_ERR_INVALID_ARG, "null n_words");
+    *n_words = 0;
+    if (!n_workers || !n_bins || n_workers > 65535u || n_bins > 65535u || uint64_t(n_workers) * n_bins != items || items > (1u << 24) ||
+        !slots || slots > 1024u)
+        return set_err(GM_ERR_INVALID_ARG, "items must be n_workers * n_bins (at most 2^24), slots in 1 .. 1024");
+    std::vector<uint32_t> t;
+    if (!gm::corr_sched_build_grid(int(n_workers), int(n_bins), int(slots), int(n_integrations), t))
+        return set_err(GM_ERR_UNSUPPORTED, "this grid cannot be scheduled (an XCD with fewer items than slots, or n_integrations outside 2 .. 16)");
+    *n_words = uint32_t(t.size());
+    if (table) {
+        if (cap_words < t.size()) return set_err(GM_ERR_OUT_OF_RANGE, "table capacity below n_words");
+        memcpy(table, t.data(), t.size() * sizeof(uint32_t));
+    }
     return GM_OK;
 }
 
diff --git a/gnss-sdr-rs_amd/csrc/gm_internal.h b/gnss-sdr-rs_amd/csrc/gm_internal.h
--- a/gnss-sdr-rs_amd/csrc/gm_internal.h
+++ b/gnss-sdr-rs_amd/csrc/gm_internal.h
@@ -69,7 +69,7 @@
     void (*corr)(hipStream_t, const cf* spectra, const cf* code_fft, const cf* tw_inv, float* mmax,
                  uint32_t* margmax, float* msum, const uint32_t* worker_list, int n_workers, int n_bins,
                  int n_int, float* split_scratch, int split_planes, uint32_t* split_counter, int strict_sum, int tickets_cleared,
-                 int ref_mul);
+                 int ref_mul, const uint32_t* sched, int sched_flags);
     void (*code_fft)(hipStream_t, const int8_t* code_samples, const cf* tw_fwd, cf* code_fft, int n_codes);
     void (*pair_codes)(hipStream_t, const cf* natural, cf* paired, int n_codes);
     void (*fft_batch)(hipStream_t, cf* data, const cf* tw, int inverse, int batch);
@@ -83,6 +83,7 @@
     int tw_total_corr;
     void (*fill_tw_corr)(cf* tw);
     void (*mix_fft_coh)(hipStream_t, const CohArgs&);
+    int corr_sched_slots;
 };
 void launch_fine_mean(hipStream_t, const void* samples, int fmt, uint32_t n, float* d_mean);
 void launch_fine_final(hipStream_t, const float* rowmax, const uint32_t* rowarg, uint32_t n_rows, int n_sats,
diff --git a/include/gnss_mi355x.h b/include/gnss_mi355x.h
--- a/include/gnss_mi355x.h
+++ b/include/gnss_mi355x.h
@@ -155,6 +155,8 @@
 int gm_acq_set_edge_search(gm_acq *a, uint32_t n_offsets, const uint32_t *offsets, const int8_t *secondary);
 int gm_acq_edge_metrics(gm_acq *a, float *max, uint32_t *argmax, float *sum);
 int gm_acq_edge_choice(gm_acq *a, uint32_t *hypothesis);
+int gm_debug_corr_schedule(uint32_t items, uint32_t n_workers, uint32_t n_bins, uint32_t n_integrations, uint32_t slots,
+                           uint32_t *table, uint32_t cap_words, uint32_t *n_words);
 int gm_acq_result_offsets(gm_acq *a, const gm_acq_result *results, const uint8_t *found, uint32_t n_prn,
                           uint32_t *offset_periods);
 int gm_acq_enable_timing(gm_acq *a, int on);
```
